# seungju-k1m/Distributed_RL

Hardware: AMD Instinct MI355X
Metric: learner frames/sec (whole node), Ape-X DQN Atari CNN (higher is better)
Workload: dtype bf16; 1 GPU; model=ape_x net (ape_x.json), global_batch=512, seq_len=4, parallelism=dp1, actors=0, replay=gpu sum-tree PER, graph=True

## Files before the change

distributed_rl_amd/algos/ape_x.py:

```python

from __future__ import annotations

import time
from collections import deque
from typing import Any, Dict, List, Optional

import numpy as np
import torch

from .. import ops
from ..config import Config
from ..models import BaseAgent
from ..replay import make_apex_schema, make_per
from .common import LearnerBase

PUBLISH_EVERY = 50
ACTOR_PULL_EVERY = 100


class ApexLearner(LearnerBase):
    ALG = "APE_X"

    def __init__(self, cfg: Config, device: Optional[str] = None, rank: int = 0,
                 world_size: int = 1, transport=None,
                 batch_size: Optional[int] = None,
                 replay_capacity: Optional[int] = None,
                 replay_device: Optional[str] = None,
                 replay_state_dtype: Optional[torch.dtype] = None,
                 replay=None, enable_tb: bool = True, run_root: str = "."):
        super().__init__(cfg, device, rank, world_size, run_root=run_root,
                         enable_tb=enable_tb)
        self.batch_size = batch_size or cfg.batch_size
        self.model = self.build_model()
        self.mp = None
        if self.device.type == "cuda":
            from ..parallel.precision import MixedPrecisionTrainer

            self.model.to(memory_format=torch.channels_last)
            order = self._dueling_param_order()
            self.mp = MixedPrecisionTrainer(self.model, param_order=order)
            self.net = self.mp.compute
            import copy as _copy

            self.target = _copy.deepcopy(self.mp.compute)
            for p in self.target.parameters():
                p.requires_grad_(False)
            from ..parallel.precision import _to_flat, _view_like

            tnamed = dict(self.target.named_parameters())
            tp = [tnamed[n] for n in self.mp._name_order]
            self.flat_tparam = torch.empty(
                sum(p.numel() for p in tp), dtype=torch.bfloat16,
                device=self.device,
            )
            off = 0
            with torch.no_grad():
                for p in tp:
                    n = p.numel()
                    self.flat_tparam[off : off + n].copy_(_to_flat(p))
                    p.data = _view_like(self.flat_tparam[off : off + n], p)
                    off += n
            self._build_fast_forward(order)
        else:
            self.net = self.model
            self.target = self.build_model()
            self.target.updateParameter(self.model, 1.0)
            for p in self.target.parameters():
                p.requires_grad_(False)
        self.optim = self.build_optim(self.model)
        cap = replay_capacity or cfg.replay_memory_len
        rdev = replay_device or (
            str(self.device) if self.device.type == "cuda" else "cpu"
        )
        self._nhwc = self.device.type == "cuda"
        self.state_dtype = replay_state_dtype or torch.uint8
        if replay is not None:
            self.replay = replay
            self._nhwc = False
        else:
            schema = (
                make_apex_schema(frame_shape=(84, 84, 4),
                                 state_dtype=self.state_dtype)
                if self._nhwc else make_apex_schema(state_dtype=self.state_dtype)
            )
            self.replay = make_per(cap, schema, device=rdev)
        self.transport = transport
        self.gamma = cfg.gamma
        self.n_step = cfg.unroll_step
        self.alpha = cfg.alpha
        self.beta = cfg.beta
        self.reducer = None
        self._ingest_stream = (
            torch.cuda.Stream(self.device) if self.device.type == "cuda" else None
        )
        self._staging = None

    def _dueling_param_order(self) -> List[str]:
        d = getattr(self.model, "_dueling", {})
        if len(d) != 1:
            return []
        (a_node, v_node), = d.values()
        if a_node not in self.model.nodes or v_node not in self.model.nodes:
            return []
        a_mod = self.model.nodes[a_node]
        v_mod = self.model.nodes[v_node]
        try:
            ok = (a_mod.body[0].in_features == v_mod.body[0].in_features
                  and a_mod.body[0].out_features == v_mod.body[0].out_features
                  and len(a_mod.body) == 4)
        except (AttributeError, IndexError, TypeError):
            ok = False
        if not ok:
            return []
        self._fast_nodes = (a_node, v_node)
        return [
            f"nodes.{a_node}.body.0.weight", f"nodes.{v_node}.body.0.weight",
            f"nodes.{a_node}.body.0.bias", f"nodes.{v_node}.body.0.bias",
        ]

    def _build_fast_forward(self, order: List[str]):
        self._fast_fwd = None
        self._fast_heads = None
        if not order:
            return
        import torch.nn.functional as F

        a_node, v_node = self._fast_nodes
        a_mod = self.net.nodes[a_node]
        hidden = a_mod.body[0].out_features
        in_f = a_mod.body[0].in_features
        w1 = self.mp.flat_view(order[:2]).view(2 * hidden, in_f
                                               ).detach().requires_grad_(True)
        w1.grad = self.mp.flat_view(order[:2], "grad").view_as(w1)
        b1 = self.mp.flat_view(order[2:]).detach().requires_grad_(True)
        b1.grad = self.mp.flat_view(order[2:], "grad").view_as(b1)
        a_head = self.net.nodes[a_node].body[2]
        v_head = self.net.nodes[v_node].body[2]
        cnn_node = next(
            n for n, c in self.cfg.model_info.items()
            if str(c.get("netCat", "")).upper() == "CNN2D"
        )
        cnn = self.net.nodes[cnn_node]

        import os as _os

        own_lin = (ops.linear_relu_supported(in_f, 2 * hidden)
                   and _os.environ.get("DRL_OWN_LINEAR", "0") == "1")

        def hidden_of(feat):
            if own_lin and feat.dtype == torch.bfloat16:
                return ops.fused_linear_relu(feat, w1, b1)
            return F.relu(F.linear(feat.to(w1.dtype), w1, b1))

        def fast_fwd(x):
            h = hidden_of(cnn(x))
            adv = a_head(h[:, :hidden])
            val = v_head(h[:, hidden:])
            return ops.dueling_head(adv.float(), val.float())

        self._fast_fwd = fast_fwd

        def fast_heads(x):
            h = hidden_of(cnn(x))
            return a_head(h[:, :hidden]), v_head(h[:, hidden:])

        self._fast_heads = fast_heads

        def fast_hidden(x):
            return hidden_of(cnn(x))

        self._fast_hidden = fast_hidden
        self._direct_list = [w1, b1] + list(self.mp.groups[0].c_params[4:])
        self._head_params = (a_head.weight, a_head.bias, v_head.weight,
                             v_head.bias)
        self._use_q_loss = ops.has_dueling_q_loss(hidden, self.cfg.action_size)
        t_cnn = self.target.nodes[cnn_node]
        ta_head = self.target.nodes[a_node].body[2]
        tv_head = self.target.nodes[v_node].body[2]
        w1t = self.flat_tparam[: 2 * hidden * in_f].view(2 * hidden, in_f)
        b1t = self.flat_tparam[2 * hidden * in_f : 2 * hidden * (in_f + 1)]

        def t_hidden_of(feat):
            if own_lin and feat.dtype == torch.bfloat16:
                return ops.fused_linear_relu(feat, w1t, b1t)
            return F.relu(F.linear(feat.to(w1t.dtype), w1t, b1t))

        def target_heads(x):
            h = t_hidden_of(t_cnn(x))
            return ta_head(h[:, :hidden]), tv_head(h[:, hidden:])

        self._target_heads = target_heads

        def target_hidden(x):
            return t_hidden_of(t_cnn(x))

        self._target_hidden = target_hidden
        self._thead_params = (ta_head.weight, ta_head.bias, tv_head.weight,
                              tv_head.bias)

    def _online_q(self, x):
        if getattr(self, "_fast_fwd", None) is not None:
            return self._fast_fwd(x)
        return self.net.forward([x])[0]

    _STAGE_ROWS = 4096

    def _staging_buffers(self):
        if self._staging is None:
            from ..replay import make_apex_schema

            wire = make_apex_schema()
            self._wire_names = list(wire)
            self._staging = {
                name: torch.empty((self._STAGE_ROWS, *shape), dtype=dtype
                                  ).pin_memory()
                for name, (shape, dtype) in wire.items()
            }
            self._staging["__prio__"] = torch.empty(
                self._STAGE_ROWS, dtype=torch.float32).pin_memory()
            self._stage_evt = torch.cuda.Event()
            self._stage_busy = False
        return self._staging

    def ingest(self) -> int:
        if self.transport is None:
            return 0
        if self._ingest_stream is not None and \
                hasattr(self.transport, "drain_views"):
            return self._ingest_views()
        got = self.transport.drain()
        if got is None:
            return 0
        cols_np, prio_np = got
        n = len(prio_np)
        if self._ingest_stream is None:
            cols = {k: torch.from_numpy(np.ascontiguousarray(v))
                    for k, v in cols_np.items()}
            self.replay.push(cols, torch.from_numpy(
                np.ascontiguousarray(prio_np)))
            self.ingested_total += n
            return n
        stage = self._staging_buffers()
        done = 0
        while done < n:
            k = min(self._STAGE_ROWS, n - done)
            if self._stage_busy:
                self._stage_evt.synchronize()
            for name, arr in cols_np.items():
                stage[name][:k].numpy()[:] = arr[done : done + k]
            stage["__prio__"][:k].numpy()[:] = prio_np[done : done + k]
            with torch.cuda.stream(self._ingest_stream):
                dev_cols = {
                    name: stage[name][:k].to(self.device, non_blocking=True)
                    for name in cols_np
                }
                if self._nhwc:
                    for kk in ("state", "next_state"):
                        dev_cols[kk] = dev_cols[kk].permute(0, 2, 3, 1
                                                            ).contiguous()
                if self.state_dtype != torch.uint8:
                    for kk in ("state", "next_state"):
                        dev_cols[kk] = dev_cols[kk].to(self.state_dtype) / 255.0
                prio_dev = stage["__prio__"][:k].to(self.device,
                                                    non_blocking=True)
            self._ingest_stream.wait_stream(
                torch.cuda.current_stream(self.device))
            with torch.cuda.stream(self._ingest_stream):
                self.replay.push(dev_cols, prio_dev)
            self._stage_evt.record(self._ingest_stream)
            self._stage_busy = True
            torch.cuda.current_stream(self.device).wait_stream(
                self._ingest_stream)
            done += k
        self.ingested_total += n
        return n

    def _ingest_views(self) -> int:
        stage = self._staging_buffers()
        np_dtype = self.transport.record_dtype
# ... 46 lines not shown
        for views, n, advance in self.transport.drain_views(
                max_per_ring=self._STAGE_ROWS):
            if stop_evt is not None and stop_evt.is_set():
                break
            for v in views:
                nrows = v.shape[0]
                i = 0
                while i < nrows:
                    if cursor == 0 and self._stage_busy:
                        self._stage_evt.synchronize()
                        self._stage_busy = False
                    k = min(self._STAGE_ROWS - cursor, nrows - i)
                    if has_pack:
                        src = torch.from_numpy(
                            np.ascontiguousarray(v[i : i + k]).reshape(-1))
                        ext.pack_rows(src, rec_size, offs, sizes, dsts, cursor)
                    else:
                        sl = v[i : i + k].reshape(-1).view(np_dtype)
                        for name in names:
                            stage[name][cursor : cursor + k].numpy()[:] = \
                                sl[name]
                        stage["__prio__"][cursor : cursor + k].numpy()[:] = \
                            sl["priority"]
                    cursor += k
                    i += k
                    total += k
                    self.ingested_total += k
                    if cursor == self._STAGE_ROWS:
                        flush()
            advance(n)
        flush()
        return total

    def push_experience(self, cols: Dict[str, torch.Tensor], prio: torch.Tensor):
        cols = dict(cols)
        for k in ("state", "next_state"):
            v = cols[k]
            if self._nhwc:
                v = v.permute(0, 2, 3, 1)
            if self.state_dtype != torch.uint8 and v.dtype == torch.uint8:
                v = v.to(self.state_dtype) / 255.0
            cols[k] = v.contiguous()
        self.replay.push(cols, prio)

    def train_step(self, data, idx, weights) -> Dict[str, torch.Tensor]:
        stats, prio = self._fwd_bwd(data, weights)
        if self.mp is not None:
            self.mp.allreduce_grads()
            self._optimize_mp()
        else:
            if self.reducer is not None:
                self.reducer.all_reduce()
            self.optim.step()
        self.replay.update(idx, prio)
        return stats

    def _fwd_bwd(self, data, weights):
        cuda = self.device.type == "cuda"
        if cuda:
            def to_cl(t):
                if t.shape[-1] == 4:
                    return t.to(self.device, non_blocking=True).permute(0, 3, 1, 2)
                return t.to(self.device, non_blocking=True).contiguous(
                    memory_format=torch.channels_last
                )

            s = to_cl(data["state"])
            sp = to_cl(data["next_state"])
            if s.dtype == torch.float16:
                s = s.to(torch.bfloat16)
                sp = sp.to(torch.bfloat16)
        elif data["state"].dtype == torch.uint8:
            s = ops.dequant_frames(data["state"], torch.float32)
            sp = ops.dequant_frames(data["next_state"], torch.float32)
        else:
            s = data["state"].float()
            sp = data["next_state"].float()
        actions = data["action"].to(self.device).long()
        rewards = data["reward"].to(self.device)
        dones = data["done"].to(self.device)
        weights = weights.to(self.device)

        if cuda and getattr(self, "_use_q_loss", False):
            h_s = self._fast_hidden(s)
            with torch.no_grad():
                h_on = self._fast_hidden(sp)
                h_tg = self._target_hidden(sp)
            wa, ba, wv, bv = self._head_params
            wat, bat, wvt, bvt = self._thead_params
            loss, prio, qmean = ops.dueling_q_head_loss(
                h_s, wa, ba, wv, bv, h_on, h_tg, wat, bat, wvt, bvt,
                actions, rewards, dones, weights, self.gamma, self.n_step,
                self.alpha,
            )
        elif cuda and getattr(self, "_fast_heads", None) is not None:
            adv_s, val_s = self._fast_heads(s)
            with torch.no_grad():
                adv_on, val_on = self._fast_heads(sp)
                adv_tg, val_tg = self._target_heads(sp)
            loss, prio, qmean = ops.dueling_nstep_dqn_loss(
                adv_s, val_s, adv_on, val_on, adv_tg, val_tg, actions,
                rewards, dones, weights, self.gamma, self.n_step, self.alpha,
            )
        else:
            q_s = self._online_q(s) if cuda else self.net.forward([s])[0]
            with torch.no_grad():
                q_sp_on = (self._online_q(sp) if cuda
                           else self.net.forward([sp])[0])
                q_sp_tg = self.target.forward([sp])[0]
            loss, prio, qmean = ops.nstep_dqn_loss(
                q_s, q_sp_on, q_sp_tg, actions, rewards,
                dones, weights, self.gamma, self.n_step, self.alpha,
                with_value_stat=True,
            )
        if self.mp is not None:
            self.mp.direct_grads(loss, getattr(self, "_direct_list", None))
        else:
            self.optim.zero_grad(set_to_none=False)
            loss.backward()
        return {"loss": loss.detach(), "value": qmean}, prio

    def _optimize_mp(self):
        self.mp.upcast_grads()
        self.optim.step()
        self.mp.sync_compute_params()

    def sync_target(self):
        if self.mp is not None:
            self.flat_tparam.copy_(self.mp.flat_cparam)
        else:
            self.target.updateParameter(self.model, 1.0)

    def _inner_step(self) -> Dict[str, torch.Tensor]:
        data, idx, w = self.replay.sample(self.batch_size, self.beta)
        return self.train_step(data, idx, w)

    def _cadence(self):
        self.step_count += 1
        if self.step_count % self.cfg.target_frequency == 0:
            self.sync_target()
            self.publish_weights(include_target=True)
        elif self.step_count % PUBLISH_EVERY == 0:
            self.publish_weights()

    def step(self) -> Dict[str, torch.Tensor]:
        stats = self.maybe_profile_first_step(self._inner_step)
        self._cadence()
        return stats

    def make_graphed_step(self, warmup_iters: int = 3):
        assert self.device.type == "cuda", "graph capture needs a GPU"
        for g in self.optim.param_groups:
            g["capturable"] = True
        split = self.mp is not None and self.mp.world > 1
        side = torch.cuda.Stream(self.device)
        side.wait_stream(torch.cuda.current_stream(self.device))
        with torch.cuda.stream(side):
            for _ in range(warmup_iters):
                self._inner_step()
        torch.cuda.current_stream(self.device).wait_stream(side)

        if not split:
            graph = torch.cuda.CUDAGraph()
            with torch.cuda.graph(graph):
                static_out = self._inner_step()
            self._graph = graph

            def stepper():
                graph.replay()
                self._cadence()
                return static_out

            return stepper

        mp = self.mp
        idx_save = torch.empty(self.batch_size, dtype=torch.int64,
                               device=self.device)
        g_s = torch.cuda.CUDAGraph()
        with torch.cuda.graph(g_s):
            s_data, s_idx, s_w = self.replay.sample(self.batch_size, self.beta)
        g_fb = torch.cuda.CUDAGraph()
        with torch.cuda.graph(g_fb, pool=g_s.pool()):
            static_out, prio = self._fwd_bwd(s_data, s_w)
            idx_save.copy_(s_idx)
        g_upd = torch.cuda.CUDAGraph()
        with torch.cuda.graph(g_upd, pool=g_s.pool()):
            self.replay.update(idx_save, prio)
        g_opt = torch.cuda.CUDAGraph()
        with torch.cuda.graph(g_opt, pool=g_s.pool()):
            self._optimize_mp()
        self._graph = (g_s, g_fb, g_upd, g_opt)
        comm = torch.cuda.Stream(self.device)
        g_s.replay()

        def stepper():
            cur = torch.cuda.current_stream(self.device)
            g_fb.replay()
            comm.wait_stream(cur)
            with torch.cuda.stream(comm):
                mp.allreduce_grads()
            g_upd.replay()
            g_s.replay()
            cur.wait_stream(comm)
            g_opt.replay()
            self._cadence()
# ... 366 lines not shown
```

distributed_rl_amd/models/base_agent.py:

```python

from __future__ import annotations

from typing import Any, Dict, List, Optional, Sequence, Tuple

import torch
import torch.nn as nn

_ACTS = {
    "relu": nn.ReLU,
    "leakyrelu": nn.LeakyReLU,
    "tanh": nn.Tanh,
    "sigmoid": nn.Sigmoid,
    "elu": nn.ELU,
    "linear": nn.Identity,
    "identity": nn.Identity,
}


def _act(name: str) -> nn.Module:
    return _ACTS[name.lower()]()


class CNN2D(nn.Module):

    def __init__(self, cfg: Dict[str, Any]):
        super().__init__()
        in_ch = int(cfg["iSize"])
        n_layer = int(cfg["nLayer"])
        f_size = list(cfg["fSize"])
        n_unit = list(cfg["nUnit"])
        stride = list(cfg.get("stride", [1] * len(n_unit)))
        padding = list(cfg.get("padding", [0] * len(n_unit)))
        acts = list(cfg.get("act", ["relu"] * len(n_unit)))
        bn = list(cfg.get("BN", [False] * n_layer))
        self.flatten = bool(cfg.get("linear", False)) or (f_size and f_size[-1] == -1)

        layers: List[nn.Module] = []
        n_conv = len(n_unit)
        ch = in_ch
        self._convs: List[nn.Conv2d] = []
        for i in range(n_conv):
            conv = nn.Conv2d(ch, n_unit[i], kernel_size=f_size[i],
                             stride=stride[i], padding=padding[i])
            self._convs.append(conv)
            layers.append(conv)
            if i < len(bn) and bn[i]:
                layers.append(nn.BatchNorm2d(n_unit[i]))
            layers.append(_act(acts[i]))
            ch = n_unit[i]
        self.body = nn.Sequential(*layers)
        self._fusable_static = (
            all(a.lower() == "relu" for a in acts[:n_conv])
            and not any(bn[:n_conv])
            and all(p == 0 for p in padding[:n_conv])
        )
        self._fused_checked: dict = {}

    def _fused_ok(self, x: torch.Tensor) -> bool:
        if not (self._fusable_static and x.is_cuda):
            return False
        if x.dtype not in (torch.uint8, torch.bfloat16):
            return False
        key = (tuple(x.shape[1:]), x.dtype)
        hit = self._fused_checked.get(key)
        if hit is not None:
            return hit
        from .. import ops as _ops

        ok = self._convs[0].weight.dtype == torch.bfloat16 and x.is_contiguous(
            memory_format=torch.channels_last
        )
        if ok:
            C, H, W = x.shape[1:]
            u8 = x.dtype == torch.uint8
            for conv in self._convs:
                COUT, _, KH, KW = conv.weight.shape
                S = conv.stride[0]
                if not _ops.conv_supported(H, W, C, KH, KW, S, COUT, u8):
                    ok = False
                    break
                H = (H - KH) // S + 1
                W = (W - KW) // S + 1
                C = COUT
                u8 = False
        self._fused_checked[key] = ok
        return ok

    def forward(self, x: torch.Tensor) -> torch.Tensor:
        if self._fused_ok(x):
            from .. import ops as _ops

            y = x
            last = len(self._convs) - 1
            for i, conv in enumerate(self._convs):
                if i == last and self.flatten and _ops.conv_chw_supported(
                        y.shape[2], y.shape[3], y.shape[1],
                        conv.weight.shape[2], conv.weight.shape[3],
                        conv.stride[0], conv.weight.shape[0]):
                    return _ops.fused_conv_relu(y, conv.weight, conv.bias,
                                                conv.stride[0], chw_out=True)
                y = _ops.fused_conv_relu(y, conv.weight, conv.bias,
                                         conv.stride[0])
        else:
            y = self.body(x)
        if self.flatten:
            y = torch.flatten(y, 1)
        return y


class MLP(nn.Module):
    def __init__(self, cfg: Dict[str, Any]):
        super().__init__()
        in_f = int(cfg["iSize"])
        f_size = list(cfg["fSize"])
        acts = list(cfg.get("act", ["relu"] * len(f_size)))
        bn = list(cfg.get("BN", [False] * len(f_size)))
        layers: List[nn.Module] = []
        f = in_f
        for i, out_f in enumerate(f_size):
            layers.append(nn.Linear(f, out_f))
            if i < len(bn) and bn[i]:
                layers.append(nn.BatchNorm1d(out_f))
            layers.append(_act(acts[i]))
            f = out_f
        self.body = nn.Sequential(*layers)

    def forward(self, x: torch.Tensor) -> torch.Tensor:
        return self.body(x)


class ViewV2(nn.Module):

    def forward(self, x: torch.Tensor, shape_hint: torch.Tensor) -> torch.Tensor:
        shape = [int(v) for v in shape_hint.flatten().tolist()]
        return x.reshape(shape)


class LSTMNET(nn.Module):

    def __init__(self, cfg: Dict[str, Any]):
        super().__init__()
        self.hidden_size = int(cfg["hiddenSize"])
        self.input_size = int(cfg["iSize"])
        self.num_layers = int(cfg.get("nLayer", 1))
        self.flatten_mode = bool(cfg.get("FlattenMode", True))
        self.return_hidden = bool(cfg.get("return_hidden", False))
        self.lstm = nn.LSTM(self.input_size, self.hidden_size, self.num_layers)
        self._state: Optional[Tuple[torch.Tensor, torch.Tensor]] = None

    def get_cell_state(self):
        return self._state

    def set_cell_state(self, state) -> None:
        self._state = state

    def zero_cell_state(self, batch: int = 1) -> None:
        p = next(self.lstm.parameters())
        z = torch.zeros(
            self.num_layers, batch, self.hidden_size, device=p.device, dtype=p.dtype
        )
        self._state = (z, z.clone())

    def detach_cell_state(self) -> None:
        if self._state is not None:
            self._state = (self._state[0].detach(), self._state[1].detach())

    def forward(self, x: torch.Tensor) -> torch.Tensor:
        p = next(self.lstm.parameters())
        import os as _os

        bf16_in = (
            x.dtype == torch.bfloat16 and x.is_cuda and self.num_layers == 1
            and _os.environ.get("DRL_LSTM_BF16_IN", "1") == "1"
        )
        if x.dtype != p.dtype and not bf16_in:
            x = x.to(p.dtype)
        if x.dim() == 2:
            x = x.unsqueeze(0)
        seq, batch, _ = x.shape
        if self._state is None or self._state[0].shape[1] != batch:
            self.zero_cell_state(batch)
        st = self._state
        if st[0].dtype != p.dtype or st[0].device != x.device:
            st = (st[0].to(x.device, p.dtype), st[1].to(x.device, p.dtype))
        if x.is_cuda and self.num_layers == 1:
            from .manual_lstm import manual_lstm_seq

            out, new_state = manual_lstm_seq(x, st, self.lstm)
        else:
            out, new_state = self.lstm(x, st)
# ... 292 lines not shown
```

distributed_rl_amd/ops/__init__.py:

```python

from __future__ import annotations

import os
from typing import Optional

import torch

from . import torch_ref

_EXT = None
_EXT_TRIED = False


def hip_ext(required: bool = True):
    global _EXT, _EXT_TRIED
    if _EXT is None and not _EXT_TRIED:
        _EXT_TRIED = True
        from . import build as _build

        _EXT = _build.load_prebuilt()
        if _EXT is None and torch.cuda.is_available():
            try:
                _EXT = _build.build()
            except Exception as e:
# ... 2 lines not shown
                        "gfx950 HIP extension missing and build failed: %s" % e
                    )
    if _EXT is None and required and not _allow_eager():
        raise RuntimeError(
            "device tensor reached a fused op but the _drl_hip extension is "
            "not built; run `python -m distributed_rl_amd.ops.build` "
            "(or set DRL_ALLOW_EAGER=1 to debug with eager torch)"
        )
    return _EXT


def _allow_eager() -> bool:
    return os.environ.get("DRL_ALLOW_EAGER", "0") == "1"


def _use_hip(t: torch.Tensor) -> bool:
    if not t.is_cuda:
        return False
    ext = hip_ext(required=not _allow_eager())
    return ext is not None




def dequant_frames(x_u8: torch.Tensor, dtype: torch.dtype = torch.bfloat16) -> torch.Tensor:
    if _use_hip(x_u8):
        out = torch.empty(x_u8.shape, dtype=dtype, device=x_u8.device)
        hip_ext().dequant(x_u8.contiguous(), out)
        return out
    return torch_ref.dequant_frames(x_u8, dtype)


def dequant_frames_nhwc(x_u8: torch.Tensor) -> torch.Tensor:
    if _use_hip(x_u8):
        out = torch.empty(
            x_u8.shape, dtype=torch.bfloat16, device=x_u8.device,
            memory_format=torch.channels_last,
        )
        hip_ext().dequant_nhwc(x_u8.contiguous(), out)
        return out
    return torch_ref.dequant_frames(x_u8, torch.float32).to(
        memory_format=torch.channels_last
    )




def conv_supported(H, W, C, KH, KW, S, COUT, u8: bool) -> bool:
    ext = hip_ext(required=False)
    if ext is None:
        return False
    return bool(ext.conv_fwd_supported(H, W, C, KH, KW, S, COUT, u8))


class _FusedConvFn(torch.autograd.Function):
    @staticmethod
    def forward(ctx, x, weight, bias, stride, chw_out=False):
        ext = hip_ext()
        N, C, H, W = x.shape
        COUT, _, KH, KW = weight.shape
        P = (H - KH) // stride + 1
        Q = (W - KW) // stride + 1
        b = bias if bias is not None else torch.empty(0, device=x.device)
        if chw_out:
            out = torch.empty(N, COUT * P * Q, dtype=torch.bfloat16,
                              device=x.device)
            ext.conv_fwd_chw(x, weight, b, out, stride)
        else:
            out = torch.empty(
                N, COUT, P, Q, dtype=torch.bfloat16, device=x.device,
                memory_format=torch.channels_last,
            )
            ext.conv_fwd(x, weight, b, out, stride)
        ctx.save_for_backward(x, weight, out)
        ctx.stride = stride
        ctx.has_bias = bias is not None
        ctx.chw = chw_out
        ctx.pq = (P, Q)
        return out

    @staticmethod
    def backward(ctx, gout):
        x, weight, out = ctx.saved_tensors
        stride = ctx.stride
        COUT = weight.shape[0]
        if ctx.chw:
            P, Q = ctx.pq
            N = gout.shape[0]
            masked = torch.empty(N, COUT, P, Q, dtype=torch.bfloat16,
                                 device=gout.device,
                                 memory_format=torch.channels_last)
            hip_ext().relu_mask_bwd_chw(gout.contiguous(), out, masked,
                                        COUT, P * Q)
            gout = masked
        else:
            if not gout.is_contiguous(memory_format=torch.channels_last):
                gout = gout.contiguous(memory_format=torch.channels_last)
            masked = torch.empty_like(gout)
            hip_ext().relu_mask_bwd(gout, out, masked)
            gout = masked
        need_x = ctx.needs_input_grad[0]
        need_w = ctx.needs_input_grad[1]
        need_b = ctx.has_bias and ctx.needs_input_grad[2]
        COUT, C, KH, KW = weight.shape
        ext = hip_ext()
        use_own_wrw = need_w and bool(
            ext.conv_wrw_supported(x.shape[2], x.shape[3], C, KH, KW, stride,
                                   COUT, x.dtype == torch.uint8)
        )
        gw = gb = None
        if use_own_wrw:
            K = KH * KW * C
            flat_ws = torch.empty(COUT * (K + 1), dtype=torch.float32,
                                  device=x.device)
            ws = flat_ws[: COUT * K].view(COUT, K)
            gb_ws = (flat_ws[COUT * K :] if need_b
                     else torch.empty(0, device=x.device))
            ext.conv_wrw(x, gout, ws, gb_ws, stride)
            gw = ws.view(COUT, KH, KW, C).permute(0, 3, 1, 2).to(torch.bfloat16)
            if need_b:
                gb = gb_ws.to(torch.bfloat16)
        gi = None
        use_own_dgrad = (
            os.environ.get("DRL_OWN_DGRAD", "0") == "1"
            and need_x and x.dtype == torch.bfloat16
            and hasattr(ext, "conv_dgrad_supported")
            and bool(ext.conv_dgrad_supported(x.shape[2], x.shape[3], C, KH,
                                              KW, stride, COUT))
        )
        if use_own_dgrad:
            gi = torch.empty_like(x)
            w_t = torch.empty(weight.numel(), dtype=torch.bfloat16,
                              device=x.device)
            ext.conv_dgrad(gout, weight, w_t, gi, stride)
        if (need_x and not use_own_dgrad) or (need_w and not use_own_wrw):
            if x.dtype == torch.uint8:
                xf = dequant_frames(x.permute(0, 2, 3, 1), torch.bfloat16)
                xf = xf.permute(0, 3, 1, 2)
            else:
                xf = x
            gi2, gw2, gb2 = torch.ops.aten.convolution_backward(
                gout, xf, weight,
                [COUT] if ctx.has_bias else None,
                [stride, stride], [0, 0], [1, 1], False, [0, 0], 1,
                [need_x and not use_own_dgrad, need_w and not use_own_wrw,
                 need_b and not use_own_wrw],
            )
            if gi is None:
                gi = gi2
            if gw is None:
                gw, gb = gw2, gb2
        return (gi if need_x else None), gw, gb, None, None


def fused_conv_relu(x, weight, bias, stride: int, chw_out: bool = False):
    return _FusedConvFn.apply(x, weight, bias, stride, chw_out)




def conv3x3_supported(H, W, C, COUT) -> bool:
    ext = hip_ext(required=False)
    return ext is not None and hasattr(ext, "conv3x3p1_supported") and \
        bool(ext.conv3x3p1_supported(H, W, C, COUT))


class _FusedConv3x3Fn(torch.autograd.Function):
    @staticmethod
    def forward(ctx, x, weight, bias, residual, relu_in, relu_out):
        ext = hip_ext()
        N, _, H, W = x.shape
        COUT = weight.shape[0]
        empty = torch.empty(0, device=x.device, dtype=torch.bfloat16)
        out = torch.empty(
            N, COUT, H, W, dtype=torch.bfloat16, device=x.device,
            memory_format=torch.channels_last,
        )
        ext.conv3x3p1_fwd(x, weight, bias if bias is not None else empty,
                          residual if residual is not None else empty, out,
                          relu_in, relu_out)
        ctx.save_for_backward(x, weight, out if relu_out else None)
        ctx.has_bias = bias is not None
        ctx.relu_in = relu_in
        ctx.relu_out = relu_out
        return out

    @staticmethod
    def backward(ctx, gout):
        x, weight, out = ctx.saved_tensors
        ext = hip_ext()
        COUT = weight.shape[0]
        if not gout.is_contiguous(memory_format=torch.channels_last):
            gout = gout.contiguous(memory_format=torch.channels_last)
        if ctx.relu_out:
            masked = torch.empty_like(gout)
            ext.relu_mask_bwd(gout, out, masked)
            gout = masked
        need_x = ctx.needs_input_grad[0]
        need_w = ctx.needs_input_grad[1]
        need_b = ctx.has_bias and ctx.needs_input_grad[2]
        gres = gout if ctx.needs_input_grad[3] else None
        gx = gw = gb = None
        if need_x or need_w or need_b:
            gx, gw, gb = torch.ops.aten.convolution_backward(
                gout, torch.relu(x) if ctx.relu_in else x, weight,
                [COUT] if ctx.has_bias else None,
                [1, 1], [1, 1], [1, 1], False, [0, 0], 1,
                [need_x, need_w, need_b],
            )
            if need_x and ctx.relu_in:
                if not gx.is_contiguous(memory_format=torch.channels_last):
                    gx = gx.contiguous(memory_format=torch.channels_last)
                masked = torch.empty_like(gx)
                ext.relu_mask_bwd(gx, x, masked)
                gx = masked
        return (gx if need_x else None), gw, gb, gres, None, None


def fused_conv3x3(x, weight, bias, *, relu_in: bool = False,
                  relu_out: bool = False, residual=None):
    if _use_hip(x):
        return _FusedConv3x3Fn.apply(x, weight, bias, residual, bool(relu_in),
                                     bool(relu_out))
    return torch_ref.conv3x3_res(x, weight, bias, relu_in, relu_out, residual)


def conv_chw_supported(H, W, C, KH, KW, S, COUT) -> bool:
    ext = hip_ext(required=False)
    return ext is not None and hasattr(ext, "conv_fwd_chw_supported") and \
        bool(ext.conv_fwd_chw_supported(H, W, C, KH, KW, S, COUT))


def linear_relu_supported(K, N) -> bool:
    ext = hip_ext(required=False)
    return ext is not None and hasattr(ext, "linear_relu_supported") and \
        bool(ext.linear_relu_supported(K, N))


class _LinearReluFn(torch.autograd.Function):
# ... 104 lines not shown
                   with_value_stat: bool = False):
    if _use_hip(q_s):
        loss, prio, qmean = _DQNLossFn.apply(
            q_s, q_sp_on, q_sp_tg, actions.long(),
            rewards.float(), dones.float(), weights.float(),
            gamma ** n_step, alpha,
        )
        return (loss, prio, qmean) if with_value_stat else (loss, prio)
    loss, prio = torch_ref.nstep_dqn_loss(
        q_s.float(), q_sp_on.float(), q_sp_tg.float(), actions, rewards.float(),
        dones.float(), weights.float(), gamma, n_step, alpha
    )
    if with_value_stat:
        return loss, prio, q_s.detach().float().max(1).values.mean()
    return loss, prio




class _DuelingDQNLossFn(torch.autograd.Function):
    @staticmethod
    def forward(ctx, adv_s, val_s, adv_on, val_on, adv_tg, val_tg, actions,
                rewards, dones, weights, gamma_n, alpha):
        ext = hip_ext()
        B, A = adv_s.shape
        dev = adv_s.device
        acc2 = torch.zeros(2, dtype=torch.float32, device=dev)
        prio = torch.empty(B, dtype=torch.float32, device=dev)
        coef = torch.empty(B, dtype=torch.float32, device=dev)
        ext.dueling_dqn_loss_fwd(
            adv_s.contiguous(), val_s.reshape(B).contiguous(),
            adv_on.contiguous(), val_on.reshape(B).contiguous(),
            adv_tg.contiguous(), val_tg.reshape(B).contiguous(),
            actions.contiguous(), rewards.contiguous(), dones.contiguous(),
            weights.contiguous(), float(gamma_n), float(alpha),
            acc2[0:1], prio, coef, acc2[1:2],
        )
        ctx.save_for_backward(coef, actions)
        ctx.shape = (B, A)
        ctx.in_dtype = adv_s.dtype
        loss_out, qmean = acc2[0], acc2[1]
        ctx.mark_non_differentiable(prio, qmean)
        return loss_out, prio, qmean

    @staticmethod
    def backward(ctx, gout, _gprio, _gqm):
        coef, actions = ctx.saved_tensors
        B, A = ctx.shape
        g_adv = torch.empty(B, A, dtype=ctx.in_dtype, device=coef.device)
        g_val = torch.empty(B, 1, dtype=ctx.in_dtype, device=coef.device)
        hip_ext().dueling_dqn_loss_bwd(coef, actions,
                                       gout.reshape(1).contiguous(), g_adv,
                                       g_val)
        return (g_adv, g_val) + (None,) * 10


def dueling_nstep_dqn_loss(adv_s, val_s, adv_on, val_on, adv_tg, val_tg,
                           actions, rewards, dones, weights, gamma: float,
                           n_step: int, alpha: float):
    if _use_hip(adv_s):
        return _DuelingDQNLossFn.apply(
            adv_s, val_s, adv_on, val_on, adv_tg, val_tg, actions.long(),
            rewards.float(), dones.float(), weights.float(),
            gamma ** n_step, alpha,
        )
    q_s = dueling_head(adv_s.float(), val_s.float())
    q_on = dueling_head(adv_on.float(), val_on.float())
    q_tg = dueling_head(adv_tg.float(), val_tg.float())
    return nstep_dqn_loss(q_s, q_on, q_tg, actions, rewards, dones, weights,
                          gamma, n_step, alpha, with_value_stat=True)




def has_dueling_q_loss(hidden: int, actions: int) -> bool:
    ext = hip_ext(required=False)
    return (ext is not None and hasattr(ext, "dueling_q_loss_fwd")
            and hidden == 512 and actions == 6)


class _DuelingQLossFn(torch.autograd.Function):
    @staticmethod
    def forward(ctx, h_s, wa, ba, wv, bv, h_on, h_tg, wa_t, ba_t, wv_t, bv_t,
                actions, rewards, dones, weights, gamma_n, alpha):
        ext = hip_ext()
        B = h_s.shape[0]
        dev = h_s.device
        acc2 = torch.zeros(2, dtype=torch.float32, device=dev)
        prio = torch.empty(B, dtype=torch.float32, device=dev)
        coef = torch.empty(B, dtype=torch.float32, device=dev)
        ext.dueling_q_loss_fwd(
            h_s.contiguous(), h_on.contiguous(), h_tg.contiguous(),
            wa.contiguous(), ba.contiguous(), wv.reshape(-1).contiguous(),
            bv.contiguous(), wa_t.contiguous(), ba_t.contiguous(),
            wv_t.reshape(-1).contiguous(), bv_t.contiguous(),
            actions.contiguous(), rewards.contiguous(), dones.contiguous(),
            weights.contiguous(), float(gamma_n), float(alpha),
            acc2[0:1], prio, coef, acc2[1:2],
        )
        ctx.save_for_backward(coef, actions, wa, wv, h_s)
        loss_out, qmean = acc2[0], acc2[1]
        ctx.mark_non_differentiable(prio, qmean)
        return loss_out, prio, qmean

    @staticmethod
    def backward(ctx, gout, _gprio, _gqm):
        coef, actions, wa, wv, h_s = ctx.saved_tensors
        ext = hip_ext()
        B = h_s.shape[0]
        dev = h_s.device
        dh = torch.empty(B, 1024, dtype=torch.bfloat16, device=dev)
        dwa = torch.empty(6, 512, dtype=torch.bfloat16, device=dev)
        dba = torch.empty(6, dtype=torch.bfloat16, device=dev)
        dwv = torch.empty(1, 512, dtype=torch.bfloat16, device=dev)
        dbv = torch.empty(1, dtype=torch.bfloat16, device=dev)
        ext.dueling_q_loss_bwd(coef, actions, gout.reshape(1).contiguous(),
                               wa.contiguous(), wv.reshape(-1).contiguous(),
                               h_s.contiguous(), dh, dwa, dba, dwv, dbv)
        return (dh, dwa, dba, dwv, dbv) + (None,) * 12


def has_r2d2_seq_loss() -> bool:
    ext = hip_ext(required=False)
    return ext is not None and hasattr(ext, "r2d2_loss_fwd")


class _R2D2SeqLossFn(torch.autograd.Function):
    @staticmethod
    def forward(ctx, q_train, q_tgt, actions, rewards, done, weights,
                burn_in, n_step, gamma, alpha, eta, use_rescaling):
        ext = hip_ext()
        T, B, A = q_tgt.shape
        W = T - 1 - burn_in
        dev = q_tgt.device
        td = torch.empty(W, B, dtype=torch.float32, device=dev)
        stats = torch.zeros(3, dtype=torch.float32, device=dev)
        ext.r2d2_loss_fwd(q_train, q_tgt, actions, rewards, done, weights,
                          burn_in, n_step, float(gamma), bool(use_rescaling),
                          td, stats)
        prio = torch.empty(B, dtype=torch.float32, device=dev)
        ext.r2d2_prio(td, float(alpha), float(eta), prio)
        ctx.save_for_backward(td, actions, weights)
        ctx.meta = (T, burn_in, tuple(q_train.shape))
        loss_out, value, td_abs = stats[0], stats[1], stats[2]
        ctx.mark_non_differentiable(prio, value, td_abs)
        return loss_out, prio, value, td_abs

    @staticmethod
    def backward(ctx, gout, _gp, _gv, _gt):
        td, actions, weights = ctx.saved_tensors
        T, m, qshape = ctx.meta
        dq = torch.empty(qshape, dtype=torch.float32, device=td.device)
        hip_ext().r2d2_loss_bwd(td, actions, weights,
                                gout.reshape(1).contiguous(), T, m, dq)
        return (dq,) + (None,) * 11


def r2d2_sequence_loss(q_train, q_tgt, actions, rewards, done, weights,
                       burn_in: int, n_step: int, gamma: float, alpha: float,
                       eta: float, use_rescaling: bool):
    return _R2D2SeqLossFn.apply(
        q_train.contiguous(), q_tgt.contiguous(),
        actions.to(torch.int32).contiguous(), rewards.float().contiguous(),
        done.float().contiguous(), weights.float().contiguous(),
        burn_in, n_step, gamma, alpha, eta, use_rescaling,
    )


def dueling_q_head_loss(h_s, wa, ba, wv, bv, h_on, h_tg, wa_t, ba_t, wv_t,
                        bv_t, actions, rewards, dones, weights, gamma: float,
                        n_step: int, alpha: float):
    if _use_hip(h_s):
        return _DuelingQLossFn.apply(
            h_s, wa, ba, wv, bv, h_on, h_tg, wa_t, ba_t, wv_t, bv_t,
            actions.long(), rewards.float(), dones.float(), weights.float(),
            gamma ** n_step, alpha,
        )
    import torch.nn.functional as F

    def heads(h, wa_, ba_, wv_, bv_):
        return (F.linear(h[:, :512].float(), wa_.float(), ba_.float()),
                F.linear(h[:, 512:].float(), wv_.float(), bv_.float()))

    adv_s, val_s = heads(h_s, wa, ba, wv, bv)
    adv_on, val_on = heads(h_on, wa, ba, wv, bv)
    adv_tg, val_tg = heads(h_tg, wa_t, ba_t, wv_t, bv_t)
    return dueling_nstep_dqn_loss(adv_s, val_s, adv_on, val_on, adv_tg,
                                  val_tg, actions, rewards, dones, weights,
                                  gamma, n_step, alpha)




def value_rescale(x: torch.Tensor, eps: float = 1e-3) -> torch.Tensor:
    if _use_hip(x) and not x.requires_grad:
        y = torch.empty_like(x, dtype=torch.float32)
        hip_ext().value_rescale(x.float().contiguous(), y, eps)
        return y
    return torch_ref.value_rescale(x, eps)


def inv_value_rescale(x: torch.Tensor, eps: float = 1e-3) -> torch.Tensor:
    if _use_hip(x) and not x.requires_grad:
        y = torch.empty_like(x, dtype=torch.float32)
        hip_ext().inv_value_rescale(x.float().contiguous(), y, eps)
        return y
    return torch_ref.inv_value_rescale(x, eps)


def sequence_priority(td_abs: torch.Tensor, alpha: float, eta: float = 0.9) -> torch.Tensor:
    if _use_hip(td_abs):
        T, B = td_abs.shape
        out = torch.empty(B, dtype=torch.float32, device=td_abs.device)
        hip_ext().seq_priority(td_abs.float().contiguous(), eta, alpha, out)
        return out
    return torch_ref.sequence_priority(td_abs, alpha, eta)




def vtrace(behavior_log_prob, target_log_prob, rewards, values, bootstrap_value,
           not_done, gamma, rho_bar=1.0, c_bar=1.0, lam=1.0):
    if _use_hip(rewards):
        T, B = rewards.shape
        dev = rewards.device
        vs = torch.empty(T, B, dtype=torch.float32, device=dev)
        pg_adv = torch.empty_like(vs)
        rho_c = torch.empty_like(vs)
        hip_ext().vtrace(
            behavior_log_prob.float().contiguous(),
            target_log_prob.float().contiguous(), rewards.float().contiguous(),
            values.float().contiguous(), bootstrap_value.float().contiguous(),
            not_done.float().contiguous(), gamma, rho_bar, c_bar, lam,
            vs, pg_adv, rho_c,
        )
        return vs, pg_adv, rho_c
    return torch_ref.vtrace(
        behavior_log_prob, target_log_prob, rewards, values, bootstrap_value,
        not_done, gamma, rho_bar, c_bar, lam
    )


def vtrace_bt(mu_probs, target_log_prob, rewards, values, bootstrap_value,
              not_done, gamma, rho_bar=1.0, c_bar=1.0, lam=1.0):
    if _use_hip(rewards):
        B, T = rewards.shape
        dev = rewards.device
        vs = torch.empty(B, T, dtype=torch.float32, device=dev)
        pg_adv = torch.empty_like(vs)
        hip_ext().vtrace_bt(
            mu_probs.float().contiguous(), target_log_prob.float().contiguous(),
            rewards.float().contiguous(), values.float().contiguous(),
            bootstrap_value.float().contiguous(), not_done.float().contiguous(),
            gamma, rho_bar, c_bar, lam, vs, pg_adv,
        )
        return vs, pg_adv
    vs_T, pg_T, _ = torch_ref.vtrace(
        mu_probs.log().t().contiguous(), target_log_prob.t().contiguous(),
        rewards.t().contiguous(), values.t().contiguous(), bootstrap_value,
        not_done, gamma, rho_bar, c_bar, lam
    )
# ... 116 lines not shown
```

distributed_rl_amd/ops/hip/conv_mfma.hip:

```cpp

#include <hip/hip_runtime.h>
#include <hip/hip_bf16.h>
#include <torch/extension.h>
#include <ATen/cuda/CUDAContext.h>

namespace {

using bf16x8 = __attribute__((ext_vector_type(8))) __bf16;
using f32x4 = __attribute__((ext_vector_type(4))) float;

constexpr int kPad = 32;

template <int H, int W, int C, int KH, int KW, int S, int COUT, bool U8IN>
struct ConvGeom {
  static constexpr int P = (H - KH) / S + 1;
  static constexpr int Q = (W - KW) / S + 1;
  static constexpr int K = KH * KW * C;
  static constexpr int KCHUNKS = K / 32;
  static_assert(K % 32 == 0, "K must be a multiple of 32");
  static_assert((KW * C) % 32 == 0, "patch row must tile by 32");
  static constexpr int ROWC = KW * C;
  static constexpr int LDS_ROW = K + kPad;
  static constexpr int LDS_ELEMS = COUT * LDS_ROW;
};

template <int H, int W, int C, int KH, int KW, int S, int COUT, bool U8IN,
          int WAVES, int RPW, bool CHW_OUT = false>
__global__ __launch_bounds__(WAVES * 64) void conv_fwd_kernel(
    const void* __restrict__ in_v,
    const __bf16* __restrict__ weight,
    const __bf16* __restrict__ bias,
    __bf16* __restrict__ out,
    int batch) {
  using G = ConvGeom<H, W, C, KH, KW, S, COUT, U8IN>;
  extern __shared__ __attribute__((aligned(16))) char smem[];
  __bf16* wlds = reinterpret_cast<__bf16*>(smem);

  const int tid = threadIdx.x;
  const int lane = tid & 63;
  const int wave = tid >> 6;

  constexpr int WELEMS = COUT * G::K;
  for (int base = tid * 8; base < WELEMS; base += WAVES * 64 * 8) {
    int co = base / G::K;
    int k = base - co * G::K;
    bf16x8 v = *reinterpret_cast<const bf16x8*>(weight + co * G::K + k);
    *reinterpret_cast<bf16x8*>(wlds + co * G::LDS_ROW + k) = v;
  }
  __syncthreads();

  const int M = batch * G::P * G::Q;
  const int row0 = (blockIdx.x * WAVES + wave) * RPW;
  if (row0 >= M) return;
  constexpr int RFRAG = RPW / 16;
  constexpr int NFRAG = COUT / 16;
  int64_t in_row0[RFRAG];
#pragma unroll
  for (int rf = 0; rf < RFRAG; ++rf) {
    int arow = row0 + rf * 16 + (lane & 15);
    if (arow >= M) arow = M - 1;
    const int n = arow / (G::P * G::Q);
    const int rem = arow - n * (G::P * G::Q);
    const int p = rem / G::Q;
    const int q = rem - p * G::Q;
    in_row0[rf] = ((int64_t)n * H + p * S) * (W * C) + q * S * C;
  }
  const int kpart = (lane >> 4) * 8;

  f32x4 acc[RFRAG][NFRAG];
#pragma unroll
  for (int rf = 0; rf < RFRAG; ++rf)
#pragma unroll
    for (int f = 0; f < NFRAG; ++f) acc[rf][f] = {0.f, 0.f, 0.f, 0.f};

#pragma unroll
  for (int kc = 0; kc < G::KCHUNKS; ++kc) {
    const int kelem = kc * 32 + kpart;
    const int dy = kelem / G::ROWC;
    const int dx = kelem - dy * G::ROWC;
    const int64_t koff = (int64_t)dy * (W * C) + dx;
    bf16x8 a[RFRAG];
#pragma unroll
    for (int rf = 0; rf < RFRAG; ++rf) {
      const int64_t goff = in_row0[rf] + koff;
      if constexpr (U8IN) {
        const uint8_t* src = reinterpret_cast<const uint8_t*>(in_v) + goff;
        uint2 raw = *reinterpret_cast<const uint2*>(src);
        const float inv255 = 1.0f / 255.0f;
#pragma unroll
        for (int j = 0; j < 8; ++j) {
          unsigned byte =
              (j < 4 ? raw.x >> (8 * j) : raw.y >> (8 * (j - 4))) & 0xFF;
          a[rf][j] = (__bf16)(byte * inv255);
        }
      } else {
        a[rf] = *reinterpret_cast<const bf16x8*>(
            reinterpret_cast<const __bf16*>(in_v) + goff);
      }
    }
#pragma unroll
    for (int f = 0; f < NFRAG; ++f) {
      const int col = f * 16 + (lane & 15);
      bf16x8 b = *reinterpret_cast<const bf16x8*>(
          wlds + col * G::LDS_ROW + kc * 32 + kpart);
#pragma unroll
      for (int rf = 0; rf < RFRAG; ++rf)
        acc[rf][f] =
            __builtin_amdgcn_mfma_f32_16x16x32_bf16(a[rf], b, acc[rf][f], 0, 0, 0);
    }
  }

  const int crow_base = (lane >> 4) * 4;
#pragma unroll
  for (int rf = 0; rf < RFRAG; ++rf)
#pragma unroll
    for (int f = 0; f < NFRAG; ++f) {
      const int col = f * 16 + (lane & 15);
      const float bv = bias ? (float)bias[col] : 0.0f;
#pragma unroll
      for (int r = 0; r < 4; ++r) {
        const int orow = row0 + rf * 16 + crow_base + r;
        if (orow < M) {
          float v = acc[rf][f][r] + bv;
          v = v > 0.0f ? v : 0.0f;
          if constexpr (CHW_OUT) {
            const int n = orow / (G::P * G::Q);
            const int pq = orow - n * (G::P * G::Q);
            out[((int64_t)n * COUT + col) * (G::P * G::Q) + pq] = (__bf16)v;
          } else {
            out[(int64_t)orow * COUT + col] = (__bf16)v;
          }
        }
      }
    }
}

struct ConvLaunch {
  int H, W, C, KH, KW, S, COUT;
  bool u8;
  void (*fn)(const void*, const __bf16*, const __bf16*, __bf16*, int);
  int lds_bytes;
  int waves, rpw;
};

template <int H, int W, int C, int KH, int KW, int S, int COUT, bool U8,
          int WAVES = 4, int RPW = 16, bool CHW = false>
ConvLaunch make_launch() {
  using G = ConvGeom<H, W, C, KH, KW, S, COUT, U8>;
  return ConvLaunch{H, W, C, KH, KW, S, COUT, U8,
                    conv_fwd_kernel<H, W, C, KH, KW, S, COUT, U8, WAVES, RPW,
                                    CHW>,
                    (int)(G::LDS_ELEMS * sizeof(__bf16)), WAVES, RPW};
}

static const ConvLaunch kChwLaunches[] = {
    make_launch<9, 9, 64, 3, 3, 1, 64, false, 8, 16, true>(),
    make_launch<20, 20, 16, 4, 4, 2, 32, false, 8, 16, true>(),
};

static const ConvLaunch kLaunches[] = {
    make_launch<84, 84, 4, 8, 8, 4, 32, true, 8, 32>(),
    make_launch<84, 84, 4, 8, 8, 4, 32, false, 8, 32>(),
    make_launch<20, 20, 32, 4, 4, 2, 64, false, 8, 16>(),
    make_launch<9, 9, 64, 3, 3, 1, 64, false, 8, 16>(),
    make_launch<84, 84, 4, 8, 8, 4, 16, true, 8, 16>(),
    make_launch<84, 84, 4, 8, 8, 4, 16, false, 8, 16>(),
    make_launch<20, 20, 16, 4, 4, 2, 32, false, 8, 16>(),
};

static const ConvLaunch kVariants[] = {
    make_launch<84, 84, 4, 8, 8, 4, 32, true, 4, 16>(),
    make_launch<84, 84, 4, 8, 8, 4, 32, true, 8, 16>(),
    make_launch<84, 84, 4, 8, 8, 4, 32, true, 4, 32>(),
    make_launch<84, 84, 4, 8, 8, 4, 32, true, 8, 32>(),
    make_launch<20, 20, 32, 4, 4, 2, 64, false, 4, 16>(),
    make_launch<20, 20, 32, 4, 4, 2, 64, false, 8, 16>(),
    make_launch<20, 20, 32, 4, 4, 2, 64, false, 4, 32>(),
    make_launch<20, 20, 32, 4, 4, 2, 64, false, 8, 32>(),
    make_launch<9, 9, 64, 3, 3, 1, 64, false, 4, 16>(),
    make_launch<9, 9, 64, 3, 3, 1, 64, false, 8, 16>(),
    make_launch<9, 9, 64, 3, 3, 1, 64, false, 4, 32>(),
    make_launch<9, 9, 64, 3, 3, 1, 64, false, 8, 32>(),
};

__global__ void mfma_probe_kernel(const __bf16* __restrict__ A,
                                  const __bf16* __restrict__ B,
                                  float* __restrict__ C) {
  int lane = threadIdx.x & 63;
  bf16x8 a, b;
  int kpart = (lane >> 4) * 8;
#pragma unroll
  for (int j = 0; j < 8; ++j) {
    a[j] = A[(lane & 15) * 32 + kpart + j];
    b[j] = B[(kpart + j) * 16 + (lane & 15)];
  }
  f32x4 acc = {0.f, 0.f, 0.f, 0.f};
  acc = __builtin_amdgcn_mfma_f32_16x16x32_bf16(a, b, acc, 0, 0, 0);
#pragma unroll
  for (int r = 0; r < 4; ++r)
    C[((lane >> 4) * 4 + r) * 16 + (lane & 15)] = acc[r];
}

}

void mfma_probe(torch::Tensor A, torch::Tensor B, torch::Tensor C) {
  hipLaunchKernelGGL(mfma_probe_kernel, dim3(1), dim3(64), 0,
                     (hipStream_t)at::cuda::getCurrentCUDAStream().stream(),
                     (const __bf16*)A.data_ptr(), (const __bf16*)B.data_ptr(),
                     C.data_ptr<float>());
}

bool conv_fwd_supported(int64_t H, int64_t W, int64_t C, int64_t KH, int64_t KW,
                        int64_t S, int64_t COUT, bool u8) {
  for (const auto& l : kLaunches)
    if (l.H == H && l.W == W && l.C == C && l.KH == KH && l.KW == KW &&
        l.S == S && l.COUT == COUT && l.u8 == u8)
      return true;
  return false;
}

void conv_fwd(torch::Tensor in, torch::Tensor weight, torch::Tensor bias,
              torch::Tensor out, int64_t stride) {
  TORCH_CHECK(in.is_cuda() && out.is_cuda());
  TORCH_CHECK(in.is_contiguous(at::MemoryFormat::ChannelsLast),
              "conv_fwd input must be channels_last");
  TORCH_CHECK(out.is_contiguous(at::MemoryFormat::ChannelsLast));
  TORCH_CHECK(weight.is_contiguous(at::MemoryFormat::ChannelsLast));
  const int N = (int)in.size(0), C = (int)in.size(1), H = (int)in.size(2),
            W = (int)in.size(3);
  const int COUT = (int)weight.size(0), KH = (int)weight.size(2),
            KW = (int)weight.size(3);
  const bool u8 = in.scalar_type() == torch::kUInt8;
  if (!u8) TORCH_CHECK(in.scalar_type() == torch::kBFloat16);
  TORCH_CHECK(weight.scalar_type() == torch::kBFloat16);
  TORCH_CHECK(out.scalar_type() == torch::kBFloat16);
  const ConvLaunch* L = nullptr;
  for (const auto& l : kLaunches)
    if (l.H == H && l.W == W && l.C == C && l.KH == KH && l.KW == KW &&
        l.S == (int)stride && l.COUT == COUT && l.u8 == u8) {
      L = &l;
      break;
    }
  TORCH_CHECK(L, "no fused conv kernel for this geometry: ", H, "x", W, "x", C,
              " k", KH, "x", KW, " s", stride, " -> ", COUT, " u8=", u8);
  const int P = (H - KH) / (int)stride + 1, Q = (W - KW) / (int)stride + 1;
  const int M = N * P * Q;
  const int rows_per_block = L->waves * L->rpw;
  const int blocks = (M + rows_per_block - 1) / rows_per_block;
  const __bf16* bias_ptr = nullptr;
  if (bias.defined() && bias.numel() > 0) {
    TORCH_CHECK(bias.scalar_type() == torch::kBFloat16);
    bias_ptr = (const __bf16*)bias.data_ptr();
  }
  hipLaunchKernelGGL(L->fn, dim3(blocks), dim3(L->waves * 64), L->lds_bytes,
                     (hipStream_t)at::cuda::getCurrentCUDAStream().stream(),
                     (const void*)in.data_ptr(),
                     (const __bf16*)weight.data_ptr(), bias_ptr,
                     (__bf16*)out.data_ptr(), N);
}

bool conv_fwd_variant(torch::Tensor in, torch::Tensor weight,
                      torch::Tensor bias, torch::Tensor out, int64_t stride,
                      int64_t variant) {
  const int N = (int)in.size(0), C = (int)in.size(1), H = (int)in.size(2),
            W = (int)in.size(3);
  const int COUT = (int)weight.size(0), KH = (int)weight.size(2),
            KW = (int)weight.size(3);
  const bool u8 = in.scalar_type() == torch::kUInt8;
  if (variant < 0 || variant >= (int64_t)(sizeof(kVariants) / sizeof(ConvLaunch)))
    return false;
  const ConvLaunch* L = &kVariants[variant];
  if (!(L->H == H && L->W == W && L->C == C && L->KH == KH && L->KW == KW &&
        L->S == (int)stride && L->COUT == COUT && L->u8 == u8))
    return false;
  const int P = (H - KH) / (int)stride + 1, Q = (W - KW) / (int)stride + 1;
  const int M = N * P * Q;
  const int rows_per_block = L->waves * L->rpw;
  const int blocks = (M + rows_per_block - 1) / rows_per_block;
  const __bf16* bias_ptr = nullptr;
  if (bias.defined() && bias.numel() > 0)
    bias_ptr = (const __bf16*)bias.data_ptr();
  hipLaunchKernelGGL(L->fn, dim3(blocks), dim3(L->waves * 64), L->lds_bytes,
                     (hipStream_t)at::cuda::getCurrentCUDAStream().stream(),
                     (const void*)in.data_ptr(),
                     (const __bf16*)weight.data_ptr(), bias_ptr,
                     (__bf16*)out.data_ptr(), N);
  return true;
}

void conv_wrw(torch::Tensor in, torch::Tensor gout, torch::Tensor gw_ws,
              torch::Tensor gb_ws, int64_t stride);
bool conv_wrw_supported(int64_t H, int64_t W, int64_t C, int64_t KH,
                        int64_t KW, int64_t S, int64_t COUT, bool u8);
void conv_dgrad(torch::Tensor gout, torch::Tensor weight, torch::Tensor w_t,
                torch::Tensor dx, int64_t stride);
bool conv_dgrad_supported(int64_t H, int64_t W, int64_t C, int64_t KH,
                          int64_t KW, int64_t S, int64_t COUT);
void conv_fwd_chw(torch::Tensor in, torch::Tensor weight, torch::Tensor bias,
                  torch::Tensor out2d, int64_t stride);
bool conv_fwd_chw_supported(int64_t H, int64_t W, int64_t C, int64_t KH,
                            int64_t KW, int64_t S, int64_t COUT);
void relu_mask_bwd_chw(torch::Tensor gout2d, torch::Tensor out2d,
                       torch::Tensor dst_nhwc, int64_t C, int64_t PQ);
void linear_relu(torch::Tensor x, torch::Tensor w, torch::Tensor b,
                 torch::Tensor out);
bool linear_relu_supported(int64_t K, int64_t N);
void tr16_probe(torch::Tensor out, int64_t mode);
void conv3x3p1_fwd(torch::Tensor in, torch::Tensor weight, torch::Tensor bias,
                   torch::Tensor residual, torch::Tensor out, bool relu_in,
                   bool relu_out);
bool conv3x3p1_supported(int64_t H, int64_t W, int64_t C, int64_t COUT);

void register_conv(pybind11::module_& m) {
  m.def("conv_fwd", &conv_fwd,
        "fused NHWC bf16 MFMA conv fwd (+dequant on u8 input, bias, ReLU)");
  m.def("conv_fwd_supported", &conv_fwd_supported);
  m.def("mfma_probe", &mfma_probe, "16x16x32 bf16 MFMA fragment-map probe");
  m.def("conv_fwd_variant", &conv_fwd_variant, "tuning-variant conv fwd");
  m.def("conv_wrw", &conv_wrw, "MFMA conv weight-grad (fp32 workspace)");
  m.def("conv_wrw_supported", &conv_wrw_supported);
  m.def("conv_dgrad", &conv_dgrad,
        "MFMA conv data-grad (masked-tap gather, pre-transposed weights)");
  m.def("conv_dgrad_supported", &conv_dgrad_supported);
  m.def("conv_fwd_chw", &conv_fwd_chw,
        "conv fwd with flatten fused into the epilogue (2-D CHW out)");
  m.def("conv_fwd_chw_supported", &conv_fwd_chw_supported);
  m.def("relu_mask_bwd_chw", &relu_mask_bwd_chw,
        "relu-mask + CHW->NHWC transpose (backward of the fused flatten)");
  m.def("linear_relu", &linear_relu,
        "fused Linear+bias+ReLU fwd (own MFMA GEMM, LDS-staged W)");
  m.def("linear_relu_supported", &linear_relu_supported);
  m.def("tr16_probe", &tr16_probe);
  m.def("conv3x3p1_fwd", &conv3x3p1_fwd,
        "MFMA 3x3 s1 pad-1 NHWC bf16 conv fwd (+relu_in, bias, residual, "
        "relu_out)");
  m.def("conv3x3p1_supported", &conv3x3p1_supported);
}


namespace {

constexpr int kPadM = 8;
constexpr int kPlanePad = 64;

typedef __bf16 v4bf_w __attribute__((ext_vector_type(4)));

template <int STRIDE>
__device__ __forceinline__ bf16x8 tr_frag(const __bf16* tile, int lane,
                                          int colblk) {
  const int g = lane >> 4, r = lane & 15;
  const __bf16* base =
      tile + (g * 8 + (r >> 2)) * STRIDE + colblk * 16 + 4 * (r & 3);
  auto* p0 = (__attribute__((address_space(3))) v4bf_w*)base;
  auto* p1 = (__attribute__((address_space(3))) v4bf_w*)(base + 4 * STRIDE);
  v4bf_w lo = __builtin_amdgcn_ds_read_tr16_b64_v4bf16(p0);
  v4bf_w hi = __builtin_amdgcn_ds_read_tr16_b64_v4bf16(p1);
  bf16x8 out;
#pragma unroll
  for (int j = 0; j < 4; ++j) { out[j] = lo[j]; out[j + 4] = hi[j]; }
  return out;
}

template <int H, int W, int C, int KH, int KW, int S, int COUT, bool U8IN>
__global__ __launch_bounds__(256) void conv_wrw_kernel(
    const void* __restrict__ in_v,
    const __bf16* __restrict__ gout,
    float* __restrict__ gw_part,
    int batch, int mblocks) {
  using G = ConvGeom<H, W, C, KH, KW, S, COUT, U8IN>;
  extern __shared__ __attribute__((aligned(16))) char smem[];
  constexpr int ASTRIDE = 64 + kPadM;
  constexpr int GSTRIDE = COUT + kPadM;
  __bf16* a_t = reinterpret_cast<__bf16*>(smem);
  __bf16* g_t = a_t + 32 * ASTRIDE;

  const int ktile = blockIdx.x;
  const int mb = blockIdx.y;
  const int tid = threadIdx.x;
  const int lane = tid & 63;
  const int wave = tid >> 6;
  const int M = batch * G::P * G::Q;
  const int n_chunks = (M + 31) / 32;

  constexpr int CBLK = COUT / 16;
  f32x4 acc[CBLK];
#pragma unroll
  for (int cb = 0; cb < CBLK; ++cb) acc[cb] = {0.f, 0.f, 0.f, 0.f};

  static_assert(G::ROWC % 16 == 0, "16-elem staging piece crosses a row");
  const int sm = tid >> 2;
  const int sk16 = (tid & 3) * 16;

  for (int mc = mb; mc < n_chunks; mc += mblocks) {
    const int m0 = mc * 32;
    if (tid < 128) {
      const int m = m0 + sm;
      const int mcl = m < M ? m : M - 1;
      const int n = mcl / (G::P * G::Q);
      const int rem = mcl - n * (G::P * G::Q);
      const int p = rem / G::Q;
      const int q = rem - p * G::Q;
      const int kelem = ktile * 64 + sk16;
      const int dy = kelem / G::ROWC;
      const int dx = kelem - dy * G::ROWC;
      const int64_t goff =
          ((int64_t)n * H + p * S + dy) * (W * C) + q * S * C + dx;
      bf16x8 v0, v1;
      if constexpr (U8IN) {
        const uint8_t* src = reinterpret_cast<const uint8_t*>(in_v) + goff;
        uint4 raw = *reinterpret_cast<const uint4*>(src);
        const float inv255 = 1.0f / 255.0f;
        const unsigned rw[4] = {raw.x, raw.y, raw.z, raw.w};
#pragma unroll
        for (int j = 0; j < 8; ++j) {
          v0[j] = (__bf16)(((rw[j >> 2] >> (8 * (j & 3))) & 0xFF) * inv255);
          v1[j] = (__bf16)(((rw[2 + (j >> 2)] >> (8 * (j & 3))) & 0xFF)
                           * inv255);
        }
      } else {
        const __bf16* src = reinterpret_cast<const __bf16*>(in_v) + goff;
        v0 = *reinterpret_cast<const bf16x8*>(src);
        v1 = *reinterpret_cast<const bf16x8*>(src + 8);
      }
      if (m >= M) {
#pragma unroll
        for (int j = 0; j < 8; ++j) {
          v0[j] = (__bf16)0.0f;
          v1[j] = (__bf16)0.0f;
        }
      }
      *reinterpret_cast<bf16x8*>(a_t + sm * ASTRIDE + sk16) = v0;
      *reinterpret_cast<bf16x8*>(a_t + sm * ASTRIDE + sk16 + 8) = v1;
    } else {
      constexpr int PIECES = COUT / 8;
      for (int piece = tid - 128; piece < 32 * PIECES; piece += 128) {
        const int m = m0 + piece / PIECES;
        const int c0 = (piece % PIECES) * 8;
        bf16x8 v;
        if (m < M) {
          v = *reinterpret_cast<const bf16x8*>(gout + (int64_t)m * COUT + c0);
        } else {
#pragma unroll
          for (int j = 0; j < 8; ++j) v[j] = (__bf16)0.0f;
        }
        *reinterpret_cast<bf16x8*>(g_t + (piece / PIECES) * GSTRIDE + c0) = v;
      }
    }
    __syncthreads();
    bf16x8 bfrag = tr_frag<ASTRIDE>(a_t, lane, wave);
#pragma unroll
    for (int cb = 0; cb < CBLK; ++cb) {
      bf16x8 afrag = tr_frag<GSTRIDE>(g_t, lane, cb);
      acc[cb] = __builtin_amdgcn_mfma_f32_16x16x32_bf16(afrag, bfrag, acc[cb],
                                                        0, 0, 0);
    }
    __syncthreads();
  }

  float* plane = gw_part + (int64_t)mb * (COUT * G::K + kPlanePad);
  const int kout = ktile * 64 + wave * 16 + (lane & 15);
#pragma unroll
  for (int cb = 0; cb < CBLK; ++cb)
#pragma unroll
    for (int r = 0; r < 4; ++r) {
      const int cout = cb * 16 + (lane >> 4) * 4 + r;
      plane[(int64_t)cout * G::K + kout] = acc[cb][r];
    }
}

__global__ __launch_bounds__(256) void wrw_reduce_kernel(
    const float* __restrict__ part, int planes, int n_elem,
    float* __restrict__ out, const float* __restrict__ b_part, int b_planes,
    int cout, float* __restrict__ b_out) {
  __shared__ __attribute__((aligned(16))) float sh4_raw[256 * 4];
  float* sh = sh4_raw;
  const int tid = threadIdx.x;
  const int e_blocks = (n_elem + 63) / 64;
  if ((int)blockIdx.x < e_blocks) {
    const int e4 = blockIdx.x * 64 + (tid & 15) * 4;
    const int g = tid >> 4;
    float4 s = {0.0f, 0.0f, 0.0f, 0.0f};
    const float4 zero = {0.0f, 0.0f, 0.0f, 0.0f};
    for (int p = g; p < planes; p += 64) {
      float4 v[4];
#pragma unroll
      for (int u = 0; u < 4; ++u) {
        const int pu = p + 16 * u;
        v[u] = pu < planes ? *reinterpret_cast<const float4*>(
                                 part + (int64_t)pu * (n_elem + kPlanePad) + e4)
                           : zero;
      }
#pragma unroll
      for (int u = 0; u < 4; ++u) {
        s.x += v[u].x; s.y += v[u].y; s.z += v[u].z; s.w += v[u].w;
      }
    }
    float4* sh4 = reinterpret_cast<float4*>(sh4_raw);
    sh4[tid] = s;
    __syncthreads();
    if (tid < 16) {
      float4 t = sh4[tid];
      for (int k = 1; k < 16; ++k) {
        const float4 v = sh4[k * 16 + tid];
        t.x += v.x; t.y += v.y; t.z += v.z; t.w += v.w;
      }
      *reinterpret_cast<float4*>(out + e4) = t;
    }
  } else {
    const int G = 256 / cout;
    const int c = tid % cout, g = tid / cout;
    float s = 0.0f;
    for (int p = g; p < b_planes; p += G) s += b_part[p * cout + c];
    sh[tid] = s;
    __syncthreads();
    if (tid < cout) {
      float t = 0.0f;
      for (int k = 0; k < G; ++k) t += sh[k * cout + tid];
      b_out[tid] = t;
    }
  }
}

struct WrwLaunch {
  int H, W, C, KH, KW, S, COUT;
  bool u8;
  void (*fn)(const void*, const __bf16*, float*, int, int);
  int lds_bytes;
  int ktiles;
};

template <int H, int W, int C, int KH, int KW, int S, int COUT, bool U8>
WrwLaunch make_wrw() {
  using G = ConvGeom<H, W, C, KH, KW, S, COUT, U8>;
  static_assert(G::K % 64 == 0, "wrw needs K % 64 == 0");
  return WrwLaunch{H, W, C, KH, KW, S, COUT, U8,
                   conv_wrw_kernel<H, W, C, KH, KW, S, COUT, U8>,
                   (int)(32 * (64 + kPadM + COUT + kPadM) * sizeof(__bf16)),
                   G::K / 64};
}

static const WrwLaunch kWrwLaunches[] = {
    make_wrw<84, 84, 4, 8, 8, 4, 32, true>(),
    make_wrw<84, 84, 4, 8, 8, 4, 32, false>(),
    make_wrw<20, 20, 32, 4, 4, 2, 64, false>(),
    make_wrw<9, 9, 64, 3, 3, 1, 64, false>(),
    make_wrw<84, 84, 4, 8, 8, 4, 16, true>(),
    make_wrw<84, 84, 4, 8, 8, 4, 16, false>(),
    make_wrw<20, 20, 16, 4, 4, 2, 32, false>(),
};

template <int COUT>
__global__ __launch_bounds__(256) void colsum_bf16_kernel(
    const __bf16* __restrict__ x, int64_t M, float* __restrict__ out) {
  typedef __bf16 bf8 __attribute__((ext_vector_type(8)));
  __shared__ float sh[256 * 8];
  const int tid = threadIdx.x;
  const int64_t nchunk = M * COUT / 8;
  int64_t i = (int64_t)blockIdx.x * blockDim.x + tid;
  const int64_t stride = (int64_t)gridDim.x * blockDim.x;
  float acc[8] = {0, 0, 0, 0, 0, 0, 0, 0};
  const bf8* __restrict__ x8 = (const bf8*)x;
  for (; i < nchunk; i += stride) {
    bf8 v = x8[i];
#pragma unroll
    for (int j = 0; j < 8; ++j) acc[j] += (float)v[j];
  }
#pragma unroll
  for (int j = 0; j < 8; ++j) sh[tid * 8 + j] = acc[j];
  __syncthreads();
  if (tid < COUT) {
    float s = 0.0f;
    for (int t = tid >> 3; t < 256; t += COUT / 8) s += sh[t * 8 + (tid & 7)];
    out[(int64_t)blockIdx.x * COUT + tid] = s;
  }
}

}

bool conv_wrw_supported(int64_t H, int64_t W, int64_t C, int64_t KH, int64_t KW,
                        int64_t S, int64_t COUT, bool u8) {
  for (const auto& l : kWrwLaunches)
    if (l.H == H && l.W == W && l.C == C && l.KH == KH && l.KW == KW &&
        l.S == S && l.COUT == COUT && l.u8 == u8)
      return true;
  return false;
}

void conv_wrw(torch::Tensor in, torch::Tensor gout, torch::Tensor gw_ws,
              torch::Tensor gb_ws, int64_t stride) {
  TORCH_CHECK(in.is_contiguous(at::MemoryFormat::ChannelsLast));
  TORCH_CHECK(gout.is_contiguous(at::MemoryFormat::ChannelsLast));
  TORCH_CHECK(gw_ws.scalar_type() == torch::kFloat32 && gw_ws.is_contiguous());
  const int N = (int)in.size(0), C = (int)in.size(1), H = (int)in.size(2),
            W = (int)in.size(3);
  const int COUT = (int)gout.size(1);
  const bool u8 = in.scalar_type() == torch::kUInt8;
  const WrwLaunch* L = nullptr;
  for (const auto& l : kWrwLaunches) {
    int KHl = l.KH, KWl = l.KW;
    if (l.H == H && l.W == W && l.C == C && l.S == (int)stride &&
        l.COUT == COUT && l.u8 == u8 &&
        (H - KHl) / (int)stride + 1 == (int)gout.size(2) &&
        (W - KWl) / (int)stride + 1 == (int)gout.size(3)) {
      L = &l;
      break;
    }
  }
  TORCH_CHECK(L, "no wrw kernel for this geometry");
  const int P = (int)gout.size(2), Q = (int)gout.size(3);
  const int M = N * P * Q;
  const int n_chunks = (M + 31) / 32;
  int mb = (n_chunks > 8192 ? 2048 : 512) / L->ktiles;
  if (mb > n_chunks) mb = n_chunks;
  if (mb < 1) mb = 1;
  auto st = (hipStream_t)at::cuda::getCurrentCUDAStream().stream();
  const int n_elem = (int)gw_ws.numel();
  TORCH_CHECK(n_elem == COUT * L->ktiles * 64, "gw_ws shape mismatch");
  auto part = torch::empty({(int64_t)mb, (int64_t)n_elem + kPlanePad},
                           gw_ws.options());
  hipLaunchKernelGGL(L->fn, dim3(L->ktiles, mb), dim3(256), L->lds_bytes, st,
                     (const void*)in.data_ptr(), (const __bf16*)gout.data_ptr(),
                     part.data_ptr<float>(), N, mb);
  const bool bias = gb_ws.defined() && gb_ws.numel() > 0;
  constexpr int kColsumBlocks = 256;
  torch::Tensor b_part;
  if (bias) {
    TORCH_CHECK(gb_ws.numel() == COUT && gb_ws.scalar_type() == torch::kFloat32);
    b_part = torch::empty({(int64_t)kColsumBlocks, (int64_t)COUT},
                          gw_ws.options());
    const int64_t Mrows = (int64_t)N * P * Q;
    switch (COUT) {
      case 16:
        hipLaunchKernelGGL(colsum_bf16_kernel<16>, dim3(kColsumBlocks),
                           dim3(256), 0, st, (const __bf16*)gout.data_ptr(),
                           Mrows, b_part.data_ptr<float>());
        break;
      case 32:
        hipLaunchKernelGGL(colsum_bf16_kernel<32>, dim3(kColsumBlocks),
                           dim3(256), 0, st, (const __bf16*)gout.data_ptr(),
                           Mrows, b_part.data_ptr<float>());
        break;
      case 64:
        hipLaunchKernelGGL(colsum_bf16_kernel<64>, dim3(kColsumBlocks),
                           dim3(256), 0, st, (const __bf16*)gout.data_ptr(),
                           Mrows, b_part.data_ptr<float>());
        break;
      default:
        TORCH_CHECK(false, "no colsum instantiation for COUT=", COUT);
    }
  }
  const int e_blocks = (n_elem + 63) / 64;
  hipLaunchKernelGGL(wrw_reduce_kernel, dim3(e_blocks + (bias ? 1 : 0)),
                     dim3(256), 0, st, (const float*)part.data_ptr<float>(), mb,
                     n_elem, gw_ws.data_ptr<float>(),
                     bias ? (const float*)b_part.data_ptr<float>() : nullptr,
                     kColsumBlocks, COUT, bias ? gb_ws.data_ptr<float>() : nullptr);
}

namespace {
typedef __bf16 v4bf __attribute__((ext_vector_type(4)));
__global__ void tr16_probe_kernel(float* out, int mode) {
  __shared__ __bf16 lds[512];
  int lane = threadIdx.x & 63;
  for (int i = threadIdx.x; i < 512; i += 64) lds[i] = (__bf16)(float)i;
  __syncthreads();
  int off;
  switch (mode) {
    case 0: off = 0; break;
    case 1: off = lane * 4; break;
    case 2: off = (lane >> 4) * 64; break;
    default: off = (lane & 15) * 4; break;
  }
  auto* p = (__attribute__((address_space(3))) v4bf*)(lds + off);
  v4bf v = __builtin_amdgcn_ds_read_tr16_b64_v4bf16(p);
#pragma unroll
  for (int j = 0; j < 4; ++j) out[lane * 4 + j] = (float)v[j];
}
}

void tr16_probe(torch::Tensor out, int64_t mode) {
  hipLaunchKernelGGL(tr16_probe_kernel, dim3(1), dim3(64), 0,
                     (hipStream_t)at::cuda::getCurrentCUDAStream().stream(),
                     out.data_ptr<float>(), (int)mode);
}

namespace {

template <int H, int W, int C, int KH, int KW, int S, int COUT, int WAVES,
          int RPW>
__global__ __launch_bounds__(WAVES * 64) void conv_dgrad_kernel(
    const __bf16* __restrict__ gout,
    const __bf16* __restrict__ w_t,
    __bf16* __restrict__ dx,
    int batch) {
  constexpr int P = (H - KH) / S + 1;
  constexpr int Q = (W - KW) / S + 1;
  constexpr int K = KH * KW * COUT;
  constexpr int KCHUNKS = K / 32;
  constexpr int CPT = COUT / 32;
  static_assert(COUT % 32 == 0, "chunks must not straddle taps");
  constexpr int RFRAG = RPW / 16;
  constexpr int NFRAG = C / 16;

  const int tid = threadIdx.x;
  const int lane = tid & 63;
  const int wave = tid >> 6;
  const int M = batch * H * W;
  const int row0 = (blockIdx.x * WAVES + wave) * RPW;
  if (row0 >= M) return;

  int a_n[RFRAG], a_y[RFRAG], a_x[RFRAG];
#pragma unroll
  for (int rf = 0; rf < RFRAG; ++rf) {
    int arow = row0 + rf * 16 + (lane & 15);
    if (arow >= M) arow = M - 1;
    a_n[rf] = arow / (H * W);
    const int rem = arow - a_n[rf] * (H * W);
    a_y[rf] = rem / W;
    a_x[rf] = rem - a_y[rf] * W;
  }
  const int kpart = (lane >> 4) * 8;

  f32x4 acc[RFRAG][NFRAG];
#pragma unroll
  for (int rf = 0; rf < RFRAG; ++rf)
#pragma unroll
    for (int f = 0; f < NFRAG; ++f) acc[rf][f] = {0.f, 0.f, 0.f, 0.f};

#pragma unroll
  for (int kc = 0; kc < KCHUNKS; ++kc) {
    const int tap = kc / CPT;
    const int kh = tap / KW;
    const int kw = tap - kh * KW;
    const int co = (kc - tap * CPT) * 32 + kpart;
    bf16x8 a[RFRAG];
#pragma unroll
    for (int rf = 0; rf < RFRAG; ++rf) {
      const int py = a_y[rf] - kh;
      const int qx = a_x[rf] - kw;
// ... 64 lines not shown
    make_dgrad<20, 20, 32, 4, 4, 2, 64>(),
    make_dgrad<9, 9, 64, 3, 3, 1, 64>(),
    make_dgrad<20, 20, 16, 4, 4, 2, 32>(),
};
}

bool conv_dgrad_supported(int64_t H, int64_t W, int64_t C, int64_t KH,
                          int64_t KW, int64_t S, int64_t COUT) {
  for (const auto& l : kDgrad)
    if (l.H == H && l.W == W && l.C == C && l.KH == KH && l.KW == KW &&
        l.S == S && l.COUT == COUT)
      return true;
  return false;
}

void conv_dgrad(torch::Tensor gout, torch::Tensor weight, torch::Tensor w_t,
                torch::Tensor dx, int64_t stride) {
  TORCH_CHECK(gout.is_contiguous(at::MemoryFormat::ChannelsLast));
  TORCH_CHECK(dx.is_contiguous(at::MemoryFormat::ChannelsLast));
  TORCH_CHECK(weight.is_contiguous(at::MemoryFormat::ChannelsLast));
  const int N = (int)dx.size(0), C = (int)dx.size(1), H = (int)dx.size(2),
            W = (int)dx.size(3);
  const int COUT = (int)weight.size(0), KH = (int)weight.size(2),
            KW = (int)weight.size(3);
  const DgradLaunch* L = nullptr;
  for (const auto& l : kDgrad)
    if (l.H == H && l.W == W && l.C == C && l.KH == KH && l.KW == KW &&
        l.S == (int)stride && l.COUT == COUT) {
      L = &l;
      break;
    }
  TORCH_CHECK(L, "no dgrad kernel for this geometry");
  auto stream = (hipStream_t)at::cuda::getCurrentCUDAStream().stream();
  const int total = KH * KW * C * COUT;
  hipLaunchKernelGGL(conv_w_transpose_kernel, dim3((total + 255) / 256),
                     dim3(256), 0, stream, (const __bf16*)weight.data_ptr(),
                     (__bf16*)w_t.data_ptr(), KH * KW, C, COUT);
  const int M = N * H * W;
  const int rows_per_block = L->waves * L->rpw;
  const int blocks = (M + rows_per_block - 1) / rows_per_block;
  hipLaunchKernelGGL(L->fn, dim3(blocks), dim3(L->waves * 64), 0, stream,
                     (const __bf16*)gout.data_ptr(),
                     (const __bf16*)w_t.data_ptr(), (__bf16*)dx.data_ptr(), N);
}

bool conv_fwd_chw_supported(int64_t H, int64_t W, int64_t C, int64_t KH,
                            int64_t KW, int64_t S, int64_t COUT) {
  for (const auto& l : kChwLaunches)
    if (l.H == H && l.W == W && l.C == C && l.KH == KH && l.KW == KW &&
        l.S == S && l.COUT == COUT)
      return true;
  return false;
}

void conv_fwd_chw(torch::Tensor in, torch::Tensor weight, torch::Tensor bias,
                  torch::Tensor out2d, int64_t stride) {
  TORCH_CHECK(in.is_contiguous(at::MemoryFormat::ChannelsLast));
  TORCH_CHECK(weight.is_contiguous(at::MemoryFormat::ChannelsLast));
  TORCH_CHECK(out2d.is_contiguous() && out2d.dim() == 2);
  const int N = (int)in.size(0), C = (int)in.size(1), H = (int)in.size(2),
            W = (int)in.size(3);
  const int COUT = (int)weight.size(0), KH = (int)weight.size(2),
            KW = (int)weight.size(3);
  const ConvLaunch* L = nullptr;
  for (const auto& l : kChwLaunches)
    if (l.H == H && l.W == W && l.C == C && l.KH == KH && l.KW == KW &&
        l.S == (int)stride && l.COUT == COUT) {
      L = &l;
      break;
    }
  TORCH_CHECK(L, "no CHW-out conv kernel for this geometry");
  const int P = (H - KH) / (int)stride + 1, Q = (W - KW) / (int)stride + 1;
  const int M = N * P * Q;
  const int rows_per_block = L->waves * L->rpw;
  const int blocks = (M + rows_per_block - 1) / rows_per_block;
  const __bf16* bias_ptr = nullptr;
  if (bias.defined() && bias.numel() > 0)
    bias_ptr = (const __bf16*)bias.data_ptr();
  hipLaunchKernelGGL(L->fn, dim3(blocks), dim3(L->waves * 64), L->lds_bytes,
                     (hipStream_t)at::cuda::getCurrentCUDAStream().stream(),
                     (const void*)in.data_ptr(),
                     (const __bf16*)weight.data_ptr(), bias_ptr,
                     (__bf16*)out2d.data_ptr(), N);
}

namespace {
__global__ void relu_mask_bwd_chw_kernel(const __bf16* __restrict__ gout,
                                         const __bf16* __restrict__ outv,
                                         __bf16* __restrict__ dst, int64_t N,
                                         int C, int PQ) {
  int64_t i = (int64_t)blockIdx.x * blockDim.x + threadIdx.x;
  const int64_t total = N * (int64_t)C * PQ;
  const int64_t stride = (int64_t)gridDim.x * blockDim.x;
  for (; i < total; i += stride) {
    const int c = (int)(i % C);
    const int64_t t = i / C;
    const int pq = (int)(t % PQ);
    const int64_t n = t / PQ;
    const int64_t src = ((int64_t)n * C + c) * PQ + pq;
    dst[i] = ((float)outv[src] > 0.0f) ? gout[src] : (__bf16)0.0f;
  }
}
}

void relu_mask_bwd_chw(torch::Tensor gout2d, torch::Tensor out2d,
                       torch::Tensor dst_nhwc, int64_t C, int64_t PQ) {
  const int64_t N = gout2d.size(0);
  const int64_t total = N * C * PQ;
  int blocks = (int)std::min<int64_t>((total + 255) / 256, 2048);
  hipLaunchKernelGGL(relu_mask_bwd_chw_kernel, dim3(blocks), dim3(256), 0,
                     (hipStream_t)at::cuda::getCurrentCUDAStream().stream(),
                     (const __bf16*)gout2d.data_ptr(),
                     (const __bf16*)out2d.data_ptr(),
                     (__bf16*)dst_nhwc.data_ptr(), N, (int)C, (int)PQ);
}

namespace {

template <int K, int N, int NT >
__global__ __launch_bounds__(256) void linear_relu_kernel(
    const __bf16* __restrict__ x,
    const __bf16* __restrict__ w,
    const __bf16* __restrict__ b,
    __bf16* __restrict__ out,
    int M) {
  constexpr int KB = 64;
  constexpr int LROW = KB + 32;
  __shared__ __bf16 wlds[NT][LROW];
  const int tid = threadIdx.x;
  const int lane = tid & 63;
  const int wave = tid >> 6;
  const int row0 = blockIdx.x * 32 + (wave >> 1) * 16;
  const int col0 = blockIdx.y * NT + (wave & 1) * (NT / 2);
  constexpr int NFRAG = NT / 2 / 16;
  const int arow = row0 + (lane & 15);
  const int arow_c = arow < M ? arow : (M > 0 ? M - 1 : 0);
  const int kpart = (lane >> 4) * 8;

  f32x4 acc[NFRAG];
#pragma unroll
  for (int f = 0; f < NFRAG; ++f) acc[f] = {0.f, 0.f, 0.f, 0.f};

  constexpr int PIECES = NT * KB / (256 * 8);
  bf16x8 wpre[PIECES];
#pragma unroll
  for (int pc = 0; pc < PIECES; ++pc) {
    const int base = (tid + pc * 256) * 8;
    const int r = base / KB;
    wpre[pc] = *reinterpret_cast<const bf16x8*>(
        w + (int64_t)(blockIdx.y * NT + r) * K + (base - r * KB));
  }
  bf16x8 a_cur[2], a_nxt[2];
#pragma unroll
  for (int kc = 0; kc < 2; ++kc)
    a_cur[kc] = *reinterpret_cast<const bf16x8*>(
        x + (int64_t)arow_c * K + kc * 32 + kpart);
  for (int k0 = 0; k0 < K; k0 += KB) {
    __syncthreads();
#pragma unroll
    for (int pc = 0; pc < PIECES; ++pc) {
      const int base = (tid + pc * 256) * 8;
      const int r = base / KB;
      *reinterpret_cast<bf16x8*>(&wlds[r][base - r * KB]) = wpre[pc];
    }
    __syncthreads();
    if (k0 + KB < K) {
// ... 309 lines not shown
```

distributed_rl_amd/ops/hip/drl_kernels.hip:

```cpp

#include <hip/hip_runtime.h>
#include <hip/hip_bf16.h>
#include <torch/extension.h>
#include <ATen/cuda/CUDAContext.h>

#define DRL_CHECK_CUDA(x) TORCH_CHECK(x.is_cuda(), #x " must be a device tensor")
#define DRL_CHECK_CONTIG(x) TORCH_CHECK(x.is_contiguous(), #x " must be contiguous")

namespace {

constexpr int kBlock = 256;

__host__ __device__ inline int64_t ceil_div(int64_t a, int64_t b) { return (a + b - 1) / b; }

inline int grid_for(int64_t work, int per_thread = 1) {
  int64_t blocks = ceil_div(work, (int64_t)kBlock * per_thread);
  if (blocks > 2048) blocks = 2048;
  if (blocks < 1) blocks = 1;
  return (int)blocks;
}


__global__ void dequant_u8_bf16_kernel(const uchar4* __restrict__ in,
                                       ushort2* __restrict__ out,
// ... 516 lines not shown
                     (float)eps);
}

void seq_priority(torch::Tensor td_abs, double eta, double alpha,
                  torch::Tensor out) {
  int T = (int)td_abs.size(0), B = (int)td_abs.size(1);
  hipLaunchKernelGGL(seq_priority_kernel, dim3(ceil_div(B, kBlock)), dim3(kBlock), 0,
                     cur_stream(), td_abs.data_ptr<float>(), T, B, (float)eta,
                     (float)alpha, out.data_ptr<float>());
}

void vtrace(torch::Tensor b_logp, torch::Tensor t_logp, torch::Tensor rew,
            torch::Tensor values, torch::Tensor boot, torch::Tensor not_done,
            double gamma, double rho_bar, double c_bar, double lam,
            torch::Tensor vs, torch::Tensor pg_adv, torch::Tensor rho_out) {
  int T = (int)rew.size(0), B = (int)rew.size(1);
  hipLaunchKernelGGL(vtrace_kernel, dim3(ceil_div(B, kBlock)), dim3(kBlock), 0,
                     cur_stream(), b_logp.data_ptr<float>(),
                     t_logp.data_ptr<float>(), rew.data_ptr<float>(),
                     values.data_ptr<float>(), boot.data_ptr<float>(),
                     not_done.data_ptr<float>(), T, B, (float)gamma,
                     (float)rho_bar, (float)c_bar, (float)lam,
                     vs.data_ptr<float>(), pg_adv.data_ptr<float>(),
                     rho_out.data_ptr<float>());
}

void vtrace_bt(torch::Tensor mu, torch::Tensor t_logp, torch::Tensor rew,
               torch::Tensor values, torch::Tensor boot, torch::Tensor not_done,
               double gamma, double rho_bar, double c_bar, double lam,
               torch::Tensor vs, torch::Tensor pg_adv) {
  int B = (int)rew.size(0), T = (int)rew.size(1);
  for (auto* t : {&mu, &t_logp, &values, &vs, &pg_adv}) {
    DRL_CHECK_CONTIG((*t));
    TORCH_CHECK(t->numel() == (int64_t)B * T, "vtrace_bt shape mismatch");
  }
  TORCH_CHECK(boot.numel() == B && not_done.numel() == B);
  hipLaunchKernelGGL(vtrace_bt_kernel, dim3(ceil_div(B, kBlock)), dim3(kBlock),
                     0, cur_stream(), mu.data_ptr<float>(),
                     t_logp.data_ptr<float>(), rew.data_ptr<float>(),
                     values.data_ptr<float>(), boot.data_ptr<float>(),
                     not_done.data_ptr<float>(), T, B, (float)gamma,
                     (float)rho_bar, (float)c_bar, (float)lam,
                     vs.data_ptr<float>(), pg_adv.data_ptr<float>());
}

void grad_clip(torch::Tensor flat, double max_norm, torch::Tensor sqsum_buf) {
  int64_t n = flat.numel();
  hipLaunchKernelGGL(sq_sum_kernel, dim3(grid_for(n, 8)), dim3(kBlock), 0,
                     cur_stream(), flat.data_ptr<float>(), n,
                     sqsum_buf.data_ptr<float>());
  hipLaunchKernelGGL(clip_scale_kernel, dim3(grid_for(n, 4)), dim3(kBlock), 0,
                     cur_stream(), flat.data_ptr<float>(), n,
                     sqsum_buf.data_ptr<float>(), (float)max_norm);
}

void register_conv(pybind11::module_& m);
void relu_mask_bwd(torch::Tensor gout, torch::Tensor out, torch::Tensor dst);
void dueling_fwd(torch::Tensor adv, torch::Tensor val, torch::Tensor out);
void dueling_bwd(torch::Tensor g, torch::Tensor gadv, torch::Tensor gval);
void lstm_cell_fwd(torch::Tensor gates, torch::Tensor c_prev,
                   torch::Tensor h_out, torch::Tensor c_out,
                   torch::Tensor acts, torch::Tensor tanhc);
void lstm_cell_bwd(torch::Tensor dh, torch::Tensor gout_t, torch::Tensor dc_in,
                   torch::Tensor acts, torch::Tensor tanhc,
                   torch::Tensor c_prev, torch::Tensor dgates,
                   torch::Tensor dc_prev);
void policy_loss_fwd(torch::Tensor logits, torch::Tensor act, torch::Tensor adv,
                     double er, torch::Tensor obj_out, torch::Tensor ent_out,
                     torch::Tensor logpa_out, torch::Tensor pi_save,
                     torch::Tensor H_save);
void policy_loss_bwd(torch::Tensor pi_save, torch::Tensor H_save,
                     torch::Tensor act, torch::Tensor adv, torch::Tensor gout,
                     double er, double gsign, torch::Tensor dlogits);
void impala_loss_fwd(torch::Tensor logpa, torch::Tensor adv,
                     torch::Tensor mean_H, torch::Tensor v, torch::Tensor vs,
                     double er, torch::Tensor loss_out, torch::Tensor obj_out,
                     torch::Tensor critic_out);
void impala_out_bwd(torch::Tensor pi_save, torch::Tensor H_save,
                    torch::Tensor act, torch::Tensor adv, torch::Tensor v,
                    torch::Tensor vs, torch::Tensor gloss, int64_t B,
                    int64_t T, int64_t A, double er, torch::Tensor dout);
void rmsprop_step(torch::Tensor p, torch::Tensor g, torch::Tensor sq,
                  torch::Tensor ga, torch::Tensor mom, double lr, double alpha,
                  double eps, double wd, double mu, bool centered, bool has_mom);
void adam_step(torch::Tensor p, torch::Tensor g, torch::Tensor m,
               torch::Tensor v, torch::Tensor step, double lr, double b1,
               double b2, double eps, double wd);
bool lstm_step_fused(torch::Tensor xp_t, torch::Tensor h_in, torch::Tensor c_in,
                     torch::Tensor w_hh, torch::Tensor h_out,
                     torch::Tensor c_out, torch::Tensor acts,
                     torch::Tensor tanhc);
bool lstm_seq_persistent(torch::Tensor xp, torch::Tensor hs, torch::Tensor cs,
                         torch::Tensor w_hh, torch::Tensor acts,
                         torch::Tensor tanhc, torch::Tensor ctr);
bool lstm_step_fwd_bf16(torch::Tensor xp_t, torch::Tensor h_bf,
                        torch::Tensor c_in, torch::Tensor w_bf,
                        torch::Tensor h_out, torch::Tensor c_out,
                        torch::Tensor h_bf_out, torch::Tensor acts_t,
                        torch::Tensor tanhc_t);
bool lstm_step_bwd_bf16(torch::Tensor dg_prev, torch::Tensor dh_init,
                        torch::Tensor gout_t, torch::Tensor dc_in,
                        torch::Tensor w_t_bf, torch::Tensor acts_t,
                        torch::Tensor tanhc_t, torch::Tensor c_prev,
                        torch::Tensor dgates_t, torch::Tensor dg_bf_t,
                        torch::Tensor dc_out);
void dueling_dqn_loss_fwd(torch::Tensor adv_s, torch::Tensor val_s,
                          torch::Tensor adv_on, torch::Tensor val_on,
                          torch::Tensor adv_tg, torch::Tensor val_tg,
                          torch::Tensor act, torch::Tensor rew,
                          torch::Tensor done, torch::Tensor w, double gamma_n,
                          double alpha, torch::Tensor loss_out,
                          torch::Tensor prio_out, torch::Tensor grad_coef,
                          torch::Tensor qmax_out);
void dueling_dqn_loss_bwd(torch::Tensor grad_coef, torch::Tensor act,
                          torch::Tensor gout, torch::Tensor g_adv,
                          torch::Tensor g_val);
void pack_rows(torch::Tensor src, int64_t rec_size, std::vector<int64_t> offs,
               std::vector<int64_t> sizes, std::vector<torch::Tensor> dsts,
               int64_t dst_row);
bool lstm_seq_fwd_bf16(torch::Tensor xp, torch::Tensor c0, torch::Tensor w_bf,
                       torch::Tensor hs, torch::Tensor cs, torch::Tensor h_bfs,
                       torch::Tensor acts, torch::Tensor tanhc,
                       torch::Tensor ctr);
bool lstm_seq_bwd_bf16(torch::Tensor dh_init, torch::Tensor gout,
                       torch::Tensor dc_T, torch::Tensor w_t_bf,
                       torch::Tensor acts, torch::Tensor tanhc,
                       torch::Tensor cs, torch::Tensor dgates,
                       torch::Tensor dgates_bf, torch::Tensor dc0_out,
                       torch::Tensor ctr);
void dueling_q_loss_fwd(torch::Tensor h_s, torch::Tensor h_on,
                        torch::Tensor h_tg, torch::Tensor wa, torch::Tensor ba,
                        torch::Tensor wv, torch::Tensor bv, torch::Tensor wa_t,
                        torch::Tensor ba_t, torch::Tensor wv_t,
                        torch::Tensor bv_t, torch::Tensor act,
                        torch::Tensor rew, torch::Tensor done, torch::Tensor w,
                        double gamma_n, double alpha, torch::Tensor loss_out,
                        torch::Tensor prio_out, torch::Tensor grad_coef,
                        torch::Tensor qmax_out);
void dueling_q_loss_bwd(torch::Tensor grad_coef, torch::Tensor act,
                        torch::Tensor gout, torch::Tensor wa, torch::Tensor wv,
                        torch::Tensor h_s, torch::Tensor dh, torch::Tensor dwa,
                        torch::Tensor dba, torch::Tensor dwv,
                        torch::Tensor dbv);
void r2d2_loss_fwd(torch::Tensor q_train, torch::Tensor q_tgt,
                   torch::Tensor act, torch::Tensor rew, torch::Tensor done,
                   torch::Tensor w, int64_t m, int64_t n_step, double gamma,
                   bool rescale, torch::Tensor td_out, torch::Tensor stats);
void r2d2_prio(torch::Tensor td, double alpha, double eta, torch::Tensor prio);
void r2d2_loss_bwd(torch::Tensor td, torch::Tensor act, torch::Tensor w,
                   torch::Tensor gout, int64_t T, int64_t m, torch::Tensor dq);
void seq_transpose_rows(torch::Tensor src, torch::Tensor dst);
void gather_rows(torch::Tensor idx, std::vector<torch::Tensor> srcs,
                 std::vector<torch::Tensor> dsts);
void lstm_diag(torch::Tensor h_bfs, torch::Tensor w_bf, torch::Tensor sink,
               torch::Tensor ctr, int64_t B, int64_t T, int64_t mode);

PYBIND11_MODULE(TORCH_EXTENSION_NAME, m) {
  register_conv(m);
  m.def("dequant", &dequant, "u8 -> bf16/f32 /255 (K1)");
  m.def("dequant_nhwc", &dequant_nhwc, "u8 NCHW -> bf16 NHWC /255 (K1)");
  m.def("sumtree_update", &sumtree_update, "sum-tree leaf update + ordered subtree/top rebuild (K10); calls on one "
        "tree must be stream-ordered");
  m.def("sumtree_sample", &sumtree_sample, "stratified sum-tree descent (K10)");
  m.def("leaf_min_pos", &leaf_min_pos, "min positive leaf priority (K10)");
  m.def("per_weights", &per_weights, "PER IS weights (K10)");
  m.def("bump_seed", &bump_seed, "advance device RNG seed (graph-safe)");
  m.def("dqn_loss_fwd", &dqn_loss_fwd, "fused n-step double-DQN loss fwd (K4)");
  m.def("dqn_loss_bwd", &dqn_loss_bwd, "fused n-step double-DQN loss bwd (K4)");
  m.def("value_rescale", &value_rescale, "R2D2 h(x) (K6)");
  m.def("inv_value_rescale", &inv_value_rescale, "R2D2 h^-1(x) (K6)");
  m.def("seq_priority", &seq_priority, "R2D2 eta-mix sequence priority (K7)");
  m.def("vtrace", &vtrace, "IMPALA V-trace reversed scan (K8)");
  m.def("vtrace_bt", &vtrace_bt,
        "V-trace on (B,T) row-major tensors, mu probs raw (K8, no transposes)");
  m.def("grad_clip", &grad_clip, "fused global grad-norm clip (K11)");
  m.def("relu_mask_bwd", &relu_mask_bwd, "dst = gout * (out > 0), bf16");
  m.def("dueling_fwd", &dueling_fwd, "fused (A+V)-mean(A) (K3)");
  m.def("dueling_bwd", &dueling_bwd, "dueling epilogue backward (K3)");
  m.def("lstm_cell_fwd", &lstm_cell_fwd, "fused LSTM cell forward (K5)");
  m.def("lstm_cell_bwd", &lstm_cell_bwd, "fused LSTM cell backward (K5)");
  m.def("policy_loss_fwd", &policy_loss_fwd, "fused IMPALA policy obj fwd (K9)");
  m.def("policy_loss_bwd", &policy_loss_bwd, "fused IMPALA policy obj bwd (K9)");
  m.def("impala_loss_fwd", &impala_loss_fwd,
        "fused IMPALA total loss: pg objective + entropy + critic MSE (K9)");
  m.def("impala_out_bwd", &impala_out_bwd,
        "IMPALA whole-head backward: d loss/d out in one launch (K9)");
  m.def("rmsprop_step", &rmsprop_step, "fused flat centered RMSprop (K12)");
  m.def("adam_step", &adam_step, "fused flat Adam (K12)");
  m.def("lstm_step_fused", &lstm_step_fused,
        "one-kernel LSTM timestep: fp32-MFMA hh GEMM + cell (K5)");
  m.def("lstm_seq_persistent", &lstm_seq_persistent,
        "whole-sequence persistent LSTM: grid-resident, agent-scope step "
        "barriers (K5)");
  m.def("lstm_step_fwd_bf16", &lstm_step_fwd_bf16,
        "one-kernel LSTM timestep fwd: bf16-MFMA hh GEMM + cell (K5 v2)");
  m.def("lstm_step_bwd_bf16", &lstm_step_bwd_bf16,
        "one-kernel LSTM timestep bwd: bf16-MFMA dh GEMM + cell-bwd (K5 v2)");
  m.def("dueling_dqn_loss_fwd", &dueling_dqn_loss_fwd,
        "whole-head dueling + n-step double-DQN loss fwd (K3+K4 fused)");
  m.def("dueling_dqn_loss_bwd", &dueling_dqn_loss_bwd,
        "whole-head dueling loss bwd: closed-form (g_adv, g_val) (K3+K4)");
  m.def("pack_rows", &pack_rows,
        "AoS records -> SoA pinned staging, GIL-free multithreaded (C2)",
        pybind11::call_guard<pybind11::gil_scoped_release>());
  m.def("lstm_seq_fwd_bf16", &lstm_seq_fwd_bf16,
        "persistent whole-sequence LSTM fwd, bf16-MFMA hh + grid barriers "
        "(K5 v3)");
  m.def("lstm_seq_bwd_bf16", &lstm_seq_bwd_bf16,
        "persistent whole-sequence LSTM bwd, bf16-MFMA dh + grid barriers "
        "(K5 v3)");
  m.def("dueling_q_loss_fwd", &dueling_q_loss_fwd,
        "heads+dueling+n-step-DQN loss in one kernel (K3+K4+heads)");
  m.def("dueling_q_loss_bwd", &dueling_q_loss_bwd,
        "closed-form dh + head weight/bias grads (2 kernels)");
  m.def("r2d2_loss_fwd", &r2d2_loss_fwd,
        "R2D2 n-step targets + rescale + IS loss, one kernel (K4/K6 seq)");
  m.def("r2d2_prio", &r2d2_prio, "eta-mix sequence priority (K7)");
  m.def("r2d2_loss_bwd", &r2d2_loss_bwd,
        "R2D2 loss backward: closed-form dq_train scatter");
  m.def("seq_transpose_rows", &seq_transpose_rows,
        "(B,T,row) -> (T,B,row) whole-row block copy");
  m.def("gather_rows", &gather_rows,
        "fused multi-column replay row gather (one launch per sample)");
  m.def("lstm_diag", &lstm_diag,
        "persistent-step cost decomposition (barrier/stage/mfma)");
}
namespace {
__global__ void relu_mask_bwd_kernel(const ushort4* __restrict__ out,
                                     const ushort4* __restrict__ gout,
                                     ushort4* __restrict__ dst, int64_t n4) {
  int64_t stride = (int64_t)gridDim.x * blockDim.x;
  for (int64_t i = (int64_t)blockIdx.x * blockDim.x + threadIdx.x; i < n4;
       i += stride) {
    ushort4 o = out[i];
    ushort4 g = gout[i];
    g.x = (o.x & 0x8000 || o.x == 0) ? 0 : g.x;
    g.y = (o.y & 0x8000 || o.y == 0) ? 0 : g.y;
    g.z = (o.z & 0x8000 || o.z == 0) ? 0 : g.z;
    g.w = (o.w & 0x8000 || o.w == 0) ? 0 : g.w;
    dst[i] = g;
  }
}
}

void relu_mask_bwd(torch::Tensor gout, torch::Tensor out, torch::Tensor dst) {
  TORCH_CHECK(gout.scalar_type() == torch::kBFloat16 &&
              out.scalar_type() == torch::kBFloat16);
  int64_t n = gout.numel();
  TORCH_CHECK(n % 4 == 0);
  hipLaunchKernelGGL(relu_mask_bwd_kernel, dim3(grid_for(n / 4)), dim3(kBlock),
                     0, cur_stream(), (const ushort4*)out.data_ptr(),
                     (const ushort4*)gout.data_ptr(), (ushort4*)dst.data_ptr(),
                     n / 4);
}

namespace {
__global__ void dueling_fwd_kernel(const float* __restrict__ adv,
                                   const float* __restrict__ val, int B, int A,
                                   float* __restrict__ out) {
  int i = blockIdx.x * blockDim.x + threadIdx.x;
  if (i >= B) return;
  const float* a = adv + (int64_t)i * A;
  float mean = 0.0f;
  for (int j = 0; j < A; ++j) mean += a[j];
  mean /= A;
  float v = val[i];
  float* o = out + (int64_t)i * A;
  for (int j = 0; j < A; ++j) o[j] = a[j] + v - mean;
}

// ... 226 lines not shown
  const float n_inv = 1.0f / (float)((int64_t)B * T);
  for (; k < total; k += stride) {
    int64_t r = k / (A + 1);
    int j = (int)(k - r * (A + 1));
    int b = (int)(r / (T + 1));
    int t = (int)(r - (int64_t)b * (T + 1));
    float g = 0.0f;
    if (t < T) {
      int64_t i = (int64_t)b * T + t;
      if (j < A) {
        float p = pi_save[i * A + j];
        float lp = __logf(fmaxf(p, 1e-30f));
        float d = adv[i] * (((int)act[i] == j ? 1.0f : 0.0f) - p)
                  - er * p * (lp + H_save[i]);
        g = -gloss[0] * d * n_inv;
      } else {
        g = gloss[0] * (v[i] - vs[i]) * n_inv;
      }
    }
    dout[k] = g;
  }
}
}

void policy_loss_fwd(torch::Tensor logits, torch::Tensor act, torch::Tensor adv,
                     double er, torch::Tensor obj_out, torch::Tensor ent_out,
                     torch::Tensor logpa_out, torch::Tensor pi_save,
                     torch::Tensor H_save) {
  int N = (int)logits.size(0), A = (int)logits.size(1);
  hipLaunchKernelGGL(policy_loss_fwd_kernel, dim3(ceil_div(N, kBlock)),
                     dim3(kBlock), 0, cur_stream(), logits.data_ptr<float>(),
                     act.data_ptr<int64_t>(), adv.data_ptr<float>(), N, A,
                     (float)er, obj_out.data_ptr<float>(),
                     ent_out.data_ptr<float>(), logpa_out.data_ptr<float>(),
                     pi_save.data_ptr<float>(), H_save.data_ptr<float>());
}

void policy_loss_bwd(torch::Tensor pi_save, torch::Tensor H_save,
                     torch::Tensor act, torch::Tensor adv, torch::Tensor gout,
                     double er, double gsign, torch::Tensor dlogits) {
  int N = (int)pi_save.size(0), A = (int)pi_save.size(1);
  hipLaunchKernelGGL(policy_loss_bwd_kernel,
                     dim3(ceil_div((int64_t)N * A, kBlock)), dim3(kBlock), 0,
                     cur_stream(), pi_save.data_ptr<float>(),
                     H_save.data_ptr<float>(), act.data_ptr<int64_t>(),
                     adv.data_ptr<float>(), gout.data_ptr<float>(), N, A,
                     (float)er, (float)gsign, dlogits.data_ptr<float>());
}

void impala_loss_fwd(torch::Tensor logpa, torch::Tensor adv,
                     torch::Tensor mean_H, torch::Tensor v, torch::Tensor vs,
                     double er, torch::Tensor loss_out, torch::Tensor obj_out,
                     torch::Tensor critic_out) {
  int64_t n = logpa.numel();
  TORCH_CHECK(adv.numel() == n && v.numel() == n && vs.numel() == n,
              "impala_loss_fwd length mismatch");
  for (auto* t : {&logpa, &adv, &v, &vs}) DRL_CHECK_CONTIG((*t));
  hipLaunchKernelGGL(impala_loss_fwd_kernel, dim3(1), dim3(kBlock), 0,
                     cur_stream(), logpa.data_ptr<float>(),
                     adv.data_ptr<float>(), mean_H.data_ptr<float>(),
                     v.data_ptr<float>(), vs.data_ptr<float>(), n, (float)er,
                     loss_out.data_ptr<float>(), obj_out.data_ptr<float>(),
                     critic_out.data_ptr<float>());
}

void impala_out_bwd(torch::Tensor pi_save, torch::Tensor H_save,
                    torch::Tensor act, torch::Tensor adv, torch::Tensor v,
                    torch::Tensor vs, torch::Tensor gloss, int64_t B,
                    int64_t T, int64_t A, double er, torch::Tensor dout) {
  int64_t total = B * (T + 1) * (A + 1);
  TORCH_CHECK(dout.numel() == total && dout.is_contiguous(),
              "impala_out_bwd dout shape mismatch");
  TORCH_CHECK(pi_save.numel() == B * T * A && v.numel() == B * T &&
              vs.numel() == B * T && act.numel() == B * T);
  hipLaunchKernelGGL(impala_out_bwd_kernel, dim3(grid_for(total, 2)),
                     dim3(kBlock), 0, cur_stream(), pi_save.data_ptr<float>(),
                     H_save.data_ptr<float>(), act.data_ptr<int64_t>(),
                     adv.data_ptr<float>(), v.data_ptr<float>(),
                     vs.data_ptr<float>(), gloss.data_ptr<float>(), (int)B,
                     (int)T, (int)A, (float)er, dout.data_ptr<float>());
}

namespace {
__global__ void rmsprop_step_kernel(
    float* __restrict__ p, const float* __restrict__ g,
    float* __restrict__ sq, float* __restrict__ ga, float* __restrict__ mom,
    int64_t n, float lr, float alpha, float eps, float wd, float mu,
    bool centered, bool has_mom) {
  int64_t stride = (int64_t)gridDim.x * blockDim.x;
  for (int64_t i = (int64_t)blockIdx.x * blockDim.x + threadIdx.x; i < n;
       i += stride) {
    float grad = g[i] + wd * p[i];
    float s = alpha * sq[i] + (1.0f - alpha) * grad * grad;
    sq[i] = s;
    float avg;
    if (centered) {
      float a = alpha * ga[i] + (1.0f - alpha) * grad;
      ga[i] = a;
      avg = sqrtf(fmaxf(s - a * a, 0.0f)) + eps;
    } else {
      avg = sqrtf(s) + eps;
    }
    float upd = grad / avg;
    if (has_mom) {
      float m = mu * mom[i] + upd;
      mom[i] = m;
      upd = m;
    }
    p[i] -= lr * upd;
  }
}

__global__ void adam_bump_kernel(float* step) {
  if (threadIdx.x == 0 && blockIdx.x == 0) step[0] += 1.0f;
}

__global__ void adam_step_kernel(
    float* __restrict__ p, const float* __restrict__ g,
    float* __restrict__ m, float* __restrict__ v,
    const float* __restrict__ step, int64_t n, float lr, float b1, float b2,
    float eps, float wd) {
  float t = step[0];
  float bc1 = 1.0f - __powf(b1, t);
  float bc2 = 1.0f - __powf(b2, t);
  int64_t stride = (int64_t)gridDim.x * blockDim.x;
  for (int64_t i = (int64_t)blockIdx.x * blockDim.x + threadIdx.x; i < n;
       i += stride) {
    float grad = g[i] + wd * p[i];
    float mi = b1 * m[i] + (1.0f - b1) * grad;
    float vi = b2 * v[i] + (1.0f - b2) * grad * grad;
    m[i] = mi;
    v[i] = vi;
    p[i] -= lr * (mi / bc1) / (sqrtf(vi / bc2) + eps);
  }
}
}

void rmsprop_step(torch::Tensor p, torch::Tensor g, torch::Tensor sq,
                  torch::Tensor ga, torch::Tensor mom, double lr, double alpha,
                  double eps, double wd, double mu, bool centered,
                  bool has_mom) {
  int64_t n = p.numel();
  hipLaunchKernelGGL(rmsprop_step_kernel, dim3(grid_for(n, 4)), dim3(kBlock), 0,
                     cur_stream(), p.data_ptr<float>(), g.data_ptr<float>(),
                     sq.data_ptr<float>(),
                     centered ? ga.data_ptr<float>() : sq.data_ptr<float>(),
                     has_mom ? mom.data_ptr<float>() : sq.data_ptr<float>(),
                     n, (float)lr, (float)alpha, (float)eps, (float)wd,
                     (float)mu, centered, has_mom);
}

void adam_step(torch::Tensor p, torch::Tensor g, torch::Tensor m,
               torch::Tensor v, torch::Tensor step, double lr, double b1,
               double b2, double eps, double wd) {
  int64_t n = p.numel();
  hipLaunchKernelGGL(adam_bump_kernel, dim3(1), dim3(64), 0, cur_stream(),
                     step.data_ptr<float>());
  hipLaunchKernelGGL(adam_step_kernel, dim3(grid_for(n, 4)), dim3(kBlock), 0,
                     cur_stream(), p.data_ptr<float>(), g.data_ptr<float>(),
                     m.data_ptr<float>(), v.data_ptr<float>(),
                     step.data_ptr<float>(), n, (float)lr, (float)b1,
                     (float)b2, (float)eps, (float)wd);
}

namespace {
constexpr int kLstmMaxB = 32;
using f32x4 = __attribute__((ext_vector_type(4))) float;

template <int H>
__global__ __launch_bounds__(256) void lstm_step_fused_kernel(
    const float* __restrict__ xp_t,
    const float* __restrict__ h_in,
    const float* __restrict__ c_in,
    const float* __restrict__ w_hh,
    float* __restrict__ h_out, float* __restrict__ c_out,
    float* __restrict__ acts,
    float* __restrict__ tanhc,
    int B) {
  constexpr int PAD = 4;
  extern __shared__ __attribute__((aligned(16))) char smem[];
  float* h_lds = reinterpret_cast<float*>(smem);
  float* gbuf = h_lds + 32 * (H + PAD);

  const int tid = threadIdx.x;
  const int lane = tid & 63;
  const int wave = tid >> 6;
  const int s16 = blockIdx.x * 16;

  for (int i = tid * 4; i < 32 * H; i += 256 * 4) {
    int row = i / H;
    int k = i - row * H;
    float4 v = {0.f, 0.f, 0.f, 0.f};
    if (row < B) v = *reinterpret_cast<const float4*>(h_in + row * H + k);
    *reinterpret_cast<float4*>(h_lds + row * (H + PAD) + k) = v;
  }
  __syncthreads();

  const int col = wave * H + s16 + (lane & 15);
  f32x4 acc[2] = {{0.f, 0.f, 0.f, 0.f}, {0.f, 0.f, 0.f, 0.f}};
  const int ksub = (lane >> 4) * 4;
  const float* wrow = w_hh + (int64_t)col * H;
#pragma unroll 4
  for (int kb = 0; kb < H; kb += 16) {
    float4 b4 = *reinterpret_cast<const float4*>(wrow + kb + ksub);
    float4 a0 = *reinterpret_cast<const float4*>(
        h_lds + (lane & 15) * (H + PAD) + kb + ksub);
    float4 a1 = *reinterpret_cast<const float4*>(
        h_lds + (16 + (lane & 15)) * (H + PAD) + kb + ksub);
#pragma unroll
    for (int j = 0; j < 4; ++j) {
      acc[0] = __builtin_amdgcn_mfma_f32_16x16x4f32(a0[j], b4[j], acc[0], 0, 0, 0);
      acc[1] = __builtin_amdgcn_mfma_f32_16x16x4f32(a1[j], b4[j], acc[1], 0, 0, 0);
    }
  }
  const int crow = (lane >> 4) * 4;
#pragma unroll
  for (int rf = 0; rf < 2; ++rf)
#pragma unroll
    for (int r = 0; r < 4; ++r) {
      int row = rf * 16 + crow + r;
      int rclamp = row < B ? row : 0;
      float v = acc[rf][r] + xp_t[(int64_t)rclamp * 4 * H + col];
      gbuf[(wave * 32 + row) * 16 + (lane & 15)] = v;
    }
  __syncthreads();

  for (int e = tid; e < 32 * 16; e += 256) {
    int row = e / 16;
    int hc = e - row * 16;
    if (row >= B) continue;
    float gi = gbuf[(0 * 32 + row) * 16 + hc];
    float gf = gbuf[(1 * 32 + row) * 16 + hc];
// ... 752 lines not shown
      if (row < B) {
        const int64_t base =
            (int64_t)t * B * 4 * H + (int64_t)row * 4 * H + g_ * H + n0;
        float4 lo = *reinterpret_cast<const float4*>(&partial[g_][row][half]);
        float4 hi =
            *reinterpret_cast<const float4*>(&partial[g_][row][half + 4]);
        *reinterpret_cast<float4*>(dgates + base + half) = lo;
        *reinterpret_cast<float4*>(dgates + base + half + 4) = hi;
        bf16x8_k5 bv;
        bv[0] = (__bf16)lo.x; bv[1] = (__bf16)lo.y;
        bv[2] = (__bf16)lo.z; bv[3] = (__bf16)lo.w;
        bv[4] = (__bf16)hi.x; bv[5] = (__bf16)hi.y;
        bv[6] = (__bf16)hi.z; bv[7] = (__bf16)hi.w;
        *reinterpret_cast<bf16x8_k5*>(dgates_bf + base + half) = bv;
      }
    }
    __syncthreads();
    if (tid == 0) {
      __builtin_amdgcn_fence(__ATOMIC_RELEASE, "agent");
      asm volatile("s_waitcnt vmcnt(0)" ::: "memory");
      __hip_atomic_fetch_add((gu32_t*)ctr, 1u, DRL_RLX_AGENT);
      const unsigned target = nblocks * (unsigned)(it + 1);
      unsigned spins = 0;
      while (__hip_atomic_load((gu32_t*)ctr, DRL_RLX_AGENT) < target) {
        __builtin_amdgcn_s_sleep(4);
        if (++spins > 5000000u) break;
      }
      __builtin_amdgcn_fence(__ATOMIC_ACQUIRE, "agent");
    }
    __syncthreads();
  }
#pragma unroll
  for (int u = 0; u < 2; ++u) {
    int e = tid + u * 256;
    int row = e >> 4, hc = e & 15;
    if (row < B) dc0_out[(int64_t)row * H + n0 + hc] = dc_reg[u];
  }
}
}

bool lstm_seq_fwd_bf16(torch::Tensor xp, torch::Tensor c0, torch::Tensor w_bf,
                       torch::Tensor hs, torch::Tensor cs, torch::Tensor h_bfs,
                       torch::Tensor acts, torch::Tensor tanhc,
                       torch::Tensor ctr) {
  int T = (int)xp.size(0), B = (int)xp.size(1), H = (int)c0.size(1);
  if (B > kLstmMaxB || H != 512) return false;
  constexpr int HH = 512;
  hipLaunchKernelGGL(lstm_seq_fwd_bf16_kernel<HH>, dim3(HH / 16), dim3(256), 0,
                     cur_stream(), xp.data_ptr<float>(), c0.data_ptr<float>(),
                     (const __bf16*)w_bf.data_ptr(), hs.data_ptr<float>(),
                     cs.data_ptr<float>(), (__bf16*)h_bfs.data_ptr(),
                     acts.data_ptr<float>(), tanhc.data_ptr<float>(),
                     (unsigned int*)ctr.data_ptr(), B, T);
  return true;
}

bool lstm_seq_bwd_bf16(torch::Tensor dh_init, torch::Tensor gout,
                       torch::Tensor dc_T, torch::Tensor w_t_bf,
                       torch::Tensor acts, torch::Tensor tanhc,
                       torch::Tensor cs, torch::Tensor dgates,
                       torch::Tensor dgates_bf, torch::Tensor dc0_out,
                       torch::Tensor ctr) {
  int T = (int)gout.size(0), B = (int)gout.size(1), H = (int)gout.size(2);
  if (B > kLstmMaxB || H != 512) return false;
  constexpr int HH = 512;
  hipLaunchKernelGGL(lstm_seq_bwd_bf16_kernel<HH>, dim3(HH / 16), dim3(256), 0,
                     cur_stream(), dh_init.data_ptr<float>(),
                     gout.data_ptr<float>(), dc_T.data_ptr<float>(),
                     (const __bf16*)w_t_bf.data_ptr(), acts.data_ptr<float>(),
                     tanhc.data_ptr<float>(), cs.data_ptr<float>(),
                     dgates.data_ptr<float>(), (__bf16*)dgates_bf.data_ptr(),
                     dc0_out.data_ptr<float>(),
                     (unsigned int*)ctr.data_ptr(), B, T);
  return true;
}

namespace {

__device__ __forceinline__ float wave_sum(float v) {
  for (int off = 32; off > 0; off >>= 1) v += __shfl_down(v, off, 64);
  return v;
}

template <int HH, int A>
__global__ __launch_bounds__(256) void dueling_q_loss_fwd_kernel(
    const __bf16* __restrict__ h_s,
    const __bf16* __restrict__ h_on,
    const __bf16* __restrict__ h_tg,
    const __bf16* __restrict__ wa, const __bf16* __restrict__ ba,
    const __bf16* __restrict__ wv, const __bf16* __restrict__ bv,
    const __bf16* __restrict__ wa_t, const __bf16* __restrict__ ba_t,
    const __bf16* __restrict__ wv_t, const __bf16* __restrict__ bv_t,
    const int64_t* __restrict__ act, const float* __restrict__ rew,
    const float* __restrict__ done, const float* __restrict__ w, int B,
    float gamma_n, float alpha, float* __restrict__ loss_out,
    float* __restrict__ prio_out, float* __restrict__ grad_coef,
    float* __restrict__ qmax_out) {
  const int lane = threadIdx.x & 63;
  const int b = blockIdx.x * 4 + (threadIdx.x >> 6);
  if (b >= B) return;
  const int k8 = lane * 8;

  float ha_s[8], hv_s[8], ha_on[8], hv_on[8], ha_tg[8], hv_tg[8];
#pragma unroll
  for (int j = 0; j < 8; ++j) {
    ha_s[j] = (float)h_s[(int64_t)b * 2 * HH + k8 + j];
    hv_s[j] = (float)h_s[(int64_t)b * 2 * HH + HH + k8 + j];
    ha_on[j] = (float)h_on[(int64_t)b * 2 * HH + k8 + j];
    hv_on[j] = (float)h_on[(int64_t)b * 2 * HH + HH + k8 + j];
    ha_tg[j] = (float)h_tg[(int64_t)b * 2 * HH + k8 + j];
    hv_tg[j] = (float)h_tg[(int64_t)b * 2 * HH + HH + k8 + j];
  }
  float q_s[A], q_on[A], q_tg[A];
#pragma unroll
  for (int j = 0; j < A; ++j) {
    float pa_s = 0.f, pa_on = 0.f, pa_tg = 0.f;
#pragma unroll
    for (int u = 0; u < 8; ++u) {
      const float wav = (float)wa[(int64_t)j * HH + k8 + u];
      const float wat = (float)wa_t[(int64_t)j * HH + k8 + u];
      pa_s += ha_s[u] * wav;
      pa_on += ha_on[u] * wav;
      pa_tg += ha_tg[u] * wat;
    }
    q_s[j] = wave_sum(pa_s);
    q_on[j] = wave_sum(pa_on);
    q_tg[j] = wave_sum(pa_tg);
  }
  float pv_s = 0.f, pv_on = 0.f, pv_tg = 0.f;
#pragma unroll
  for (int u = 0; u < 8; ++u) {
    const float wvv = (float)wv[k8 + u];
    const float wvt = (float)wv_t[k8 + u];
    pv_s += hv_s[u] * wvv;
    pv_on += hv_on[u] * wvv;
    pv_tg += hv_tg[u] * wvt;
  }
  const float v_s = wave_sum(pv_s);
  const float v_tg = wave_sum(pv_tg);
  wave_sum(pv_on);

  if (lane == 0) {
    float mean_s = 0.f, mean_tg = 0.f, best = -1e30f;
    int a_star = 0;
#pragma unroll
    for (int j = 0; j < A; ++j) {
      const float adv_on = q_on[j] + (float)ba[j];
      if (adv_on > best) { best = adv_on; a_star = j; }
      q_s[j] += (float)ba[j];
      q_tg[j] += (float)ba_t[j];
      mean_s += q_s[j];
      mean_tg += q_tg[j];
    }
    mean_s /= A;
    mean_tg /= A;
    const float vs_full = v_s + (float)bv[0];
    const float vt_full = v_tg + (float)bv_t[0];
    const float q_tgt = q_tg[a_star] - mean_tg + vt_full;
    const float target = rew[b] + gamma_n * q_tgt * (1.0f - done[b]);
    float smax = q_s[0];
#pragma unroll
    for (int j = 1; j < A; ++j) smax = fmaxf(smax, q_s[j]);
    const float q = q_s[act[b]] - mean_s + vs_full;
    const float raw = target - q;
    const float td = fminf(1.0f, fmaxf(-1.0f, raw));
    prio_out[b] = __powf(fabsf(td) + 1e-7f, alpha);
    const float in_range = (raw > -1.0f && raw < 1.0f) ? 1.0f : 0.0f;
    const float invB = 1.0f / B;
    grad_coef[b] = w[b] * td * in_range * invB;
    atomicAdd(loss_out, 0.5f * w[b] * td * td * invB);
    atomicAdd(qmax_out, (smax - mean_s + vs_full) * invB);
  }
}

template <int HH, int A>
__global__ void dueling_q_loss_bwd_dh_kernel(
    const float* __restrict__ grad_coef, const int64_t* __restrict__ act,
    const float* __restrict__ gout, const __bf16* __restrict__ wa,
    const __bf16* __restrict__ wv, int B, __bf16* __restrict__ dh) {
  const int i = blockIdx.x * blockDim.x + threadIdx.x;
  if (i >= B * 2 * HH) return;
  const int b = i / (2 * HH);
  const int k = i - b * 2 * HH;
  const float c = -grad_coef[b] * gout[0];
  float v;
  if (k < HH) {
    float m = 0.f;
#pragma unroll
    for (int j = 0; j < A; ++j) m += (float)wa[(int64_t)j * HH + k];
    v = c * ((float)wa[(int64_t)act[b] * HH + k] - m / A);
  } else {
    v = c * (float)wv[k - HH];
  }
  dh[i] = (__bf16)v;
}

template <int HH, int A, int BS>
__global__ __launch_bounds__(256) void dueling_q_loss_bwd_dw_kernel(
    const float* __restrict__ grad_coef, const int64_t* __restrict__ act,
    const float* __restrict__ gout, const __bf16* __restrict__ h_s, int B,
    float* __restrict__ ws) {
  const int j = blockIdx.x;
  const int sl = blockIdx.y;
  const int tid = threadIdx.x;
  const float g = gout[0];
  float accw[HH / 256];
#pragma unroll
  for (int u = 0; u < HH / 256; ++u) accw[u] = 0.f;
  float accb = 0.f;
  for (int b = sl; b < B; b += BS) {
    const float c = -grad_coef[b] * g;
    float alpha_jb;
    int64_t hoff;
    if (j < A) {
      alpha_jb = c * (((int)act[b] == j ? 1.0f : 0.0f) - 1.0f / A);
      hoff = (int64_t)b * 2 * HH;
    } else {
      alpha_jb = c;
      hoff = (int64_t)b * 2 * HH + HH;
    }
    accb += alpha_jb;
#pragma unroll
    for (int u = 0; u < HH / 256; ++u) {
      const int k = u * 256 + tid;
      accw[u] += alpha_jb * (float)h_s[hoff + k];
    }
  }
  float* row = ws + ((int64_t)sl * (A + 1) + j) * (HH + 1);
#pragma unroll
  for (int u = 0; u < HH / 256; ++u) row[u * 256 + tid] = accw[u];
  if (tid == 0) row[HH] = accb;
}

template <int HH, int A, int BS>
__global__ void dueling_q_loss_bwd_dw_fold_kernel(
    const float* __restrict__ ws, __bf16* __restrict__ dwa,
    __bf16* __restrict__ dba, __bf16* __restrict__ dwv,
    __bf16* __restrict__ dbv) {
  const int i = blockIdx.x * blockDim.x + threadIdx.x;
  constexpr int ROW = HH + 1;
  if (i >= (A + 1) * ROW) return;
  const int j = i / ROW;
  const int k = i - j * ROW;
  float v = 0.f;
#pragma unroll
  for (int s = 0; s < BS; ++s) v += ws[((int64_t)s * (A + 1) + j) * ROW + k];
  if (k < HH) {
    if (j < A)
      dwa[(int64_t)j * HH + k] = (__bf16)v;
    else
      dwv[k] = (__bf16)v;
  } else {
    if (j < A)
      dba[j] = (__bf16)v;
    else
      dbv[0] = (__bf16)v;
  }
}
}

void dueling_q_loss_fwd(torch::Tensor h_s, torch::Tensor h_on,
                        torch::Tensor h_tg, torch::Tensor wa, torch::Tensor ba,
                        torch::Tensor wv, torch::Tensor bv, torch::Tensor wa_t,
                        torch::Tensor ba_t, torch::Tensor wv_t,
                        torch::Tensor bv_t, torch::Tensor act,
                        torch::Tensor rew, torch::Tensor done, torch::Tensor w,
                        double gamma_n, double alpha, torch::Tensor loss_out,
                        torch::Tensor prio_out, torch::Tensor grad_coef,
                        torch::Tensor qmax_out) {
  int B = (int)h_s.size(0);
  TORCH_CHECK(h_s.size(1) == 1024 && wa.size(0) == 6, "geometry: HH=512 A=6");
  hipLaunchKernelGGL((dueling_q_loss_fwd_kernel<512, 6>),
                     dim3((B + 3) / 4), dim3(256), 0, cur_stream(),
                     (const __bf16*)h_s.data_ptr(),
                     (const __bf16*)h_on.data_ptr(),
                     (const __bf16*)h_tg.data_ptr(),
                     (const __bf16*)wa.data_ptr(), (const __bf16*)ba.data_ptr(),
                     (const __bf16*)wv.data_ptr(), (const __bf16*)bv.data_ptr(),
                     (const __bf16*)wa_t.data_ptr(),
                     (const __bf16*)ba_t.data_ptr(),
                     (const __bf16*)wv_t.data_ptr(),
                     (const __bf16*)bv_t.data_ptr(), act.data_ptr<int64_t>(),
                     rew.data_ptr<float>(), done.data_ptr<float>(),
                     w.data_ptr<float>(), B, (float)gamma_n, (float)alpha,
                     loss_out.data_ptr<float>(), prio_out.data_ptr<float>(),
                     grad_coef.data_ptr<float>(), qmax_out.data_ptr<float>());
}

void dueling_q_loss_bwd(torch::Tensor grad_coef, torch::Tensor act,
                        torch::Tensor gout, torch::Tensor wa, torch::Tensor wv,
                        torch::Tensor h_s, torch::Tensor dh, torch::Tensor dwa,
                        torch::Tensor dba, torch::Tensor dwv,
                        torch::Tensor dbv) {
  int B = (int)h_s.size(0);
  hipLaunchKernelGGL((dueling_q_loss_bwd_dh_kernel<512, 6>),
                     dim3(ceil_div((int64_t)B * 1024, kBlock)), dim3(kBlock),
                     0, cur_stream(), grad_coef.data_ptr<float>(),
                     act.data_ptr<int64_t>(), gout.data_ptr<float>(),
                     (const __bf16*)wa.data_ptr(), (const __bf16*)wv.data_ptr(),
                     B, (__bf16*)dh.data_ptr());
  constexpr int BS = 32;
  auto ws = torch::empty({BS * 7 * 513}, torch::dtype(torch::kFloat32)
                                             .device(h_s.device()));
  hipLaunchKernelGGL((dueling_q_loss_bwd_dw_kernel<512, 6, BS>),
                     dim3(7, BS), dim3(256), 0, cur_stream(),
                     grad_coef.data_ptr<float>(), act.data_ptr<int64_t>(),
                     gout.data_ptr<float>(), (const __bf16*)h_s.data_ptr(), B,
                     ws.data_ptr<float>());
  hipLaunchKernelGGL((dueling_q_loss_bwd_dw_fold_kernel<512, 6, BS>),
                     dim3(ceil_div(7 * 513, kBlock)), dim3(kBlock), 0,
                     cur_stream(), ws.data_ptr<float>(),
                     (__bf16*)dwa.data_ptr(), (__bf16*)dba.data_ptr(),
                     (__bf16*)dwv.data_ptr(), (__bf16*)dbv.data_ptr());
}

namespace {

__device__ __forceinline__ float vrescale(float x) {
  const float s = x >= 0.0f ? 1.0f : -1.0f;
  return s * (sqrtf(fabsf(x) + 1.0f) - 1.0f) + 1e-3f * x;
}

__device__ __forceinline__ float inv_vrescale(float x) {
  const float s = x >= 0.0f ? 1.0f : -1.0f;
  const float e = 1e-3f;
  const float t = 1.0f + 4.0f * e * (fabsf(x) + 1.0f + e);
  const float r = (sqrtf(t) - 1.0f) / (2.0f * e);
  return s * (r * r - 1.0f);
}

__global__ void r2d2_loss_fwd_kernel(
    const float* __restrict__ q_train,
    const float* __restrict__ q_tgt,
    const int* __restrict__ act,
    const float* __restrict__ rew,
    const float* __restrict__ done,
    const float* __restrict__ w,
    int T, int B, int A, int m, int n_step, float gamma, int rescale,
    float* __restrict__ td_out,
    float* __restrict__ stats)
{
  const int W = T - 1 - m;
  const int i = blockIdx.x * blockDim.x + threadIdx.x;
  float lc = 0.f, qc = 0.f, tc = 0.f;
  if (i < W * B) {
    const int ti = i / B;
    const int b = i - ti * B;
    const int t = m + ti;
    const int n = min(n_step, T - 1 - t);
    float ret = 0.f, g = 1.0f;
    for (int k = 0; k < n; ++k) {
      ret += g * rew[(int64_t)(t + k) * B + b];
      g *= gamma;
    }
    const int tn = t + n;
    const float* q_on_row = (tn >= m)
        ? q_train + ((int64_t)(tn - m) * B + b) * A
        : q_tgt + ((int64_t)tn * B + b) * A;
    int a_star = 0;
    float best = q_on_row[0];
    for (int a = 1; a < A; ++a)
      if (q_on_row[a] > best) { best = q_on_row[a]; a_star = a; }
    float q_boot = q_tgt[((int64_t)tn * B + b) * A + a_star];
    if (rescale) q_boot = inv_vrescale(q_boot);
    if (tn == T - 1) q_boot *= (1.0f - done[b]);
    float G = ret + g * q_boot;
    if (rescale) G = vrescale(G);
    const float q_taken =
        q_train[((int64_t)ti * B + b) * A + act[(int64_t)t * B + b]];
    const float td = G - q_taken;
    td_out[(int64_t)ti * B + b] = td;
    const float inv = 1.0f / (B * W);
    lc = 0.5f * w[b] * td * td * inv;
    qc = q_taken * inv;
    tc = fabsf(td) * inv;
  }
  for (int off = 32; off > 0; off >>= 1) {
    lc += __shfl_down(lc, off, 64);
    qc += __shfl_down(qc, off, 64);
    tc += __shfl_down(tc, off, 64);
  }
  if ((threadIdx.x & 63) == 0 && (lc != 0.f || qc != 0.f || tc != 0.f)) {
    atomicAdd(&stats[0], lc);
    atomicAdd(&stats[1], qc);
    atomicAdd(&stats[2], tc);
  }
}
// ... 238 lines not shown
```

distributed_rl_amd/parallel/flat_optim.py:

```python

from __future__ import annotations

from typing import Any, Dict, List

import torch

from ..ops import hip_ext


class _FlatOptimBase:
    def __init__(self):
        self.param_groups: List[Dict[str, Any]] = [{}]

    def zero_grad(self, set_to_none: bool = False):
        for g in self.grads:
            g.zero_()


class FlatRMSprop(_FlatOptimBase):
    def __init__(self, params_flat, grads_flat, lr=1e-2, alpha=0.99, eps=1e-8,
                 weight_decay=0.0, momentum=0.0, centered=False):
        super().__init__()
        self.params = list(params_flat)
        self.grads = list(grads_flat)
        self.lr, self.alpha, self.eps = float(lr), float(alpha), float(eps)
        self.wd, self.mu = float(weight_decay), float(momentum)
        self.centered = bool(centered)
        self.sq = [torch.zeros_like(p) for p in self.params]
        self.ga = [torch.zeros_like(p) if centered else torch.empty(0)
                   for p in self.params]
        self.mom = [torch.zeros_like(p) if momentum > 0 else torch.empty(0)
                    for p in self.params]

    def step(self):
        ext = hip_ext()
        for p, g, sq, ga, mom in zip(self.params, self.grads, self.sq,
                                     self.ga, self.mom):
            ext.rmsprop_step(p, g, sq, ga, mom, self.lr, self.alpha, self.eps,
                             self.wd, self.mu, self.centered, self.mu > 0)

    def state_dict(self):
        return {"kind": "flat_rmsprop", "sq": self.sq, "ga": self.ga,
                "mom": self.mom}

    def load_state_dict(self, sd):
        for dst, src in zip(self.sq, sd["sq"]):
            dst.copy_(src.to(dst.device))
        for dst, src in zip(self.ga, sd["ga"]):
            if dst.numel():
                dst.copy_(src.to(dst.device))
        for dst, src in zip(self.mom, sd["mom"]):
            if dst.numel():
                dst.copy_(src.to(dst.device))


class FlatAdam(_FlatOptimBase):
    def __init__(self, params_flat, grads_flat, lr=1e-3, betas=(0.9, 0.999),
                 eps=1e-8, weight_decay=0.0):
        super().__init__()
        self.params = list(params_flat)
        self.grads = list(grads_flat)
        self.lr, self.eps = float(lr), float(eps)
        self.b1, self.b2 = float(betas[0]), float(betas[1])
        self.wd = float(weight_decay)
        self.m = [torch.zeros_like(p) for p in self.params]
        self.v = [torch.zeros_like(p) for p in self.params]
        dev = self.params[0].device
        self.t = [torch.zeros(1, device=dev) for _ in self.params]

    def step(self):
        ext = hip_ext()
        for p, g, m, v, t in zip(self.params, self.grads, self.m, self.v,
                                 self.t):
            ext.adam_step(p, g, m, v, t, self.lr, self.b1, self.b2, self.eps,
                          self.wd)

    def state_dict(self):
        return {"kind": "flat_adam", "m": self.m, "v": self.v, "t": self.t}

    def load_state_dict(self, sd):
        for name in ("m", "v", "t"):
            for dst, src in zip(getattr(self, name), sd[name]):
                dst.copy_(src.to(dst.device))


def make_flat_optimizer(optim_info: Dict[str, Any], mp):
    name = str(optim_info.get("name", "")).lower()
    params = [g.flat_mparam for g in mp.groups]
    grads = [g.flat_mgrad for g in mp.groups]
    if name == "rmsprop":
        return FlatRMSprop(
            params, grads, lr=float(optim_info.get("lr", 1e-3)),
            alpha=float(optim_info.get("alpha", 0.99)),
            eps=float(optim_info.get("eps", 1e-8)),
            weight_decay=float(optim_info.get("decay", 0.0)),
            momentum=float(optim_info.get("momentum", 0.0)),
            centered=bool(optim_info.get("centered", False)),
        )
    if name == "adam":
        return FlatAdam(
            params, grads, lr=float(optim_info.get("lr", 1e-3)),
            eps=float(optim_info.get("eps", 1e-8)),
            weight_decay=float(optim_info.get("decay", 0.0)),
        )
    return None
```

distributed_rl_amd/parallel/precision.py:

```python

from __future__ import annotations

import copy
from typing import Callable, Optional

import torch
import torch.distributed as dist


def _is_cl(p: torch.Tensor) -> bool:
    return p.dim() == 4 and p.is_contiguous(memory_format=torch.channels_last) \
        and not p.is_contiguous()


def _to_flat(p: torch.Tensor) -> torch.Tensor:
    if _is_cl(p):
        return p.permute(0, 2, 3, 1).reshape(-1)
    return p.reshape(-1)


def _view_like(flat_slice: torch.Tensor, p: torch.Tensor) -> torch.Tensor:
    if _is_cl(p):
        N, C, H, W = p.shape
        return flat_slice.view(N, H, W, C).permute(0, 3, 1, 2)
# ... 76 lines not shown
                assert end - start == sum(offs[n][1] for n in names), (
                    f"params {names} are not adjacent in the flat buffer"
                )
                buf = g.flat_cparam if of == "param" else g.flat_cgrad
                return buf[start:end]
        raise KeyError(f"params {names} not found in one group")

    @property
    def flat_cparam(self):
        assert len(self.groups) == 1
        return self.groups[0].flat_cparam

    @property
    def flat_cgrad(self):
        assert len(self.groups) == 1
        return self.groups[0].flat_cgrad

    @property
    def flat_mgrad(self):
        assert len(self.groups) == 1
        return self.groups[0].flat_mgrad

    @property
    def flat_mparam(self):
        assert len(self.groups) == 1
        return self.groups[0].flat_mparam

    def all_mgrads(self):
        return [g.flat_mgrad for g in self.groups]

    def zero_grads(self):
        for g in self.groups:
            g.flat_cgrad.zero_()

    def direct_grads(self, loss, params_override=None):
        if params_override is not None:
            assert len(self.groups) == 1
            grads = torch.autograd.grad(loss, params_override)
            flats = []
            for p, gr in zip(params_override, grads):
                if gr.dim() == 4 and _is_cl(p) and not _is_cl(gr):
                    gr = gr.contiguous(memory_format=torch.channels_last)
                flats.append(_to_flat(gr))
            torch.cat(flats, out=self.groups[0].flat_cgrad)
            return
        params = [cp for g in self.groups for cp in g.c_params]
        grads = torch.autograd.grad(loss, params)
        i = 0
        for g in self.groups:
            n = len(g.c_params)
            flats = []
            for cp, gr in zip(g.c_params, grads[i : i + n]):
                if gr.dim() == 4 and _is_cl(cp) and not _is_cl(gr):
                    gr = gr.contiguous(memory_format=torch.channels_last)
                flats.append(_to_flat(gr))
            i += n
            torch.cat(flats, out=g.flat_cgrad)

    def allreduce_grads(self):
        if self.world > 1:
            for g in self.groups:
                dist.all_reduce(g.flat_cgrad, group=self.pg)

    def allreduce_grads_async(self):
        if self.world > 1:
            return [dist.all_reduce(g.flat_cgrad, group=self.pg, async_op=True)
                    for g in self.groups]
        return []

    def upcast_grads(self):
        for g in self.groups:
            g.flat_mgrad.copy_(g.flat_cgrad)
            if self.world > 1:
                g.flat_mgrad.mul_(1.0 / self.world)

    def reduce_and_upcast(self):
        self.allreduce_grads()
        self.upcast_grads()

    def sync_compute_params(self):
        for g in self.groups:
            g.flat_cparam.copy_(g.flat_mparam)

    def broadcast_master(self):
        if self.world > 1:
            for g in self.groups:
                dist.broadcast(g.flat_mparam, src=0, group=self.pg)
            self.sync_compute_params()
```

Measured before the change: 908,300 frames/s.

## Group three conv towers, fuse ReLU into Q-loss, fuse optimizer tail

Runs the online-state, online-next-state and target-next-state CNN forwards as one grouped conv launch per layer instead of three separate passes. Moves the hidden-layer ReLU into the dueling Q-loss kernels, which now take pre-activations and mask gradients themselves. Fuses grad upcast, the RMSprop step and the bf16 parameter copy-back into a single kernel reading bf16 grads. Conv weight-gradient output now goes straight to bf16 without a float workspace. These cut kernel launches and memory passes, at the cost of more custom code paths, all enabled by default through environment flags.

```diff
diff --git a/distributed_rl_amd/algos/ape_x.py b/distributed_rl_amd/algos/ape_x.py
--- a/distributed_rl_amd/algos/ape_x.py
+++ b/distributed_rl_amd/algos/ape_x.py
@@ -1,6 +1,7 @@
 
 from __future__ import annotations
 
+import os as _os
 import time
 from collections import deque
 from typing import Any, Dict, List, Optional
@@ -11,6 +12,7 @@
 from .. import ops
 from ..config import Config
 from ..models import BaseAgent
+from ..models.base_agent import CNN2D
 from ..replay import make_apex_schema, make_per
 from .common import LearnerBase
 
@@ -142,8 +144,6 @@
         )
         cnn = self.net.nodes[cnn_node]
 
-        import os as _os
-
         own_lin = (ops.linear_relu_supported(in_f, 2 * hidden)
                    and _os.environ.get("DRL_OWN_LINEAR", "0") == "1")
 
@@ -170,6 +170,14 @@
             return hidden_of(cnn(x))
 
         self._fast_hidden = fast_hidden
+        self._cnn = cnn
+        self._own_lin = own_lin
+
+        def pre_hidden_of(feat):
+            return F.linear(feat.to(w1.dtype), w1, b1)
+
+        self._pre_hidden_of = pre_hidden_of
+        self._hidden_of = hidden_of
         self._direct_list = [w1, b1] + list(self.mp.groups[0].c_params[4:])
         self._head_params = (a_head.weight, a_head.bias, v_head.weight,
                              v_head.bias)
@@ -195,6 +203,10 @@
             return t_hidden_of(t_cnn(x))
 
         self._target_hidden = target_hidden
+        self._t_cnn = t_cnn
+        self._t_hidden_of = t_hidden_of
+        self._t_pre_hidden_of = (
+            lambda feat: F.linear(feat.to(w1t.dtype), w1t, b1t))
         self._thead_params = (ta_head.weight, ta_head.bias, tv_head.weight,
                               tv_head.bias)
 
@@ -407,16 +419,29 @@
         weights = weights.to(self.device)
 
         if cuda and getattr(self, "_use_q_loss", False):
-            h_s = self._fast_hidden(s)
+            pre = (_os.environ.get("DRL_PREACT_LOSS", "1") == "1"
+                   and not self._own_lin)
+            if _os.environ.get("DRL_GROUPED_CONV", "1") == "1":
+                f_s, f_on, f_tg = CNN2D.forward_grouped(
+                    [(s, self._cnn, True), (sp, self._cnn, False),
+                     (sp, self._t_cnn, False)])
+            else:
+                f_s = self._cnn(s)
+                with torch.no_grad():
+                    f_on = self._cnn(sp)
+                    f_tg = self._t_cnn(sp)
+            hid = self._pre_hidden_of if pre else self._hidden_of
+            t_hid = self._t_pre_hidden_of if pre else self._t_hidden_of
+            h_s = hid(f_s)
             with torch.no_grad():
-                h_on = self._fast_hidden(sp)
-                h_tg = self._target_hidden(sp)
+                h_on = hid(f_on)
+                h_tg = t_hid(f_tg)
             wa, ba, wv, bv = self._head_params
             wat, bat, wvt, bvt = self._thead_params
             loss, prio, qmean = ops.dueling_q_head_loss(
                 h_s, wa, ba, wv, bv, h_on, h_tg, wat, bat, wvt, bvt,
                 actions, rewards, dones, weights, self.gamma, self.n_step,
-                self.alpha,
+                self.alpha, pre_act=pre,
             )
         elif cuda and getattr(self, "_fast_heads", None) is not None:
             adv_s, val_s = self._fast_heads(s)
@@ -446,6 +471,9 @@
         return {"loss": loss.detach(), "value": qmean}, prio
 
     def _optimize_mp(self):
+        if (_os.environ.get("DRL_FUSED_OPT_TAIL", "1") == "1"
+                and self.mp.fused_step(self.optim)):
+            return
         self.mp.upcast_grads()
         self.optim.step()
         self.mp.sync_compute_params()
diff --git a/distributed_rl_amd/models/base_agent.py b/distributed_rl_amd/models/base_agent.py
--- a/distributed_rl_amd/models/base_agent.py
+++ b/distributed_rl_amd/models/base_agent.py
@@ -106,6 +106,81 @@
         if self.flatten:
             y = torch.flatten(y, 1)
         return y
+
+    def _grouped_ok(self, x: torch.Tensor) -> bool:
+        if not self._fused_ok(x):
+            return False
+        key = ("grouped", tuple(x.shape[1:]), x.dtype)
+        hit = self._fused_checked.get(key)
+        if hit is not None:
+            return hit
+        from .. import ops as _ops
+
+        ok = True
+        C, H, W = x.shape[1:]
+        u8 = x.dtype == torch.uint8
+        last = len(self._convs) - 1
+        for i, conv in enumerate(self._convs):
+            COUT, _, KH, KW = conv.weight.shape
+            S = conv.stride[0]
+            chw = (i == last and self.flatten
+                   and _ops.conv_chw_supported(H, W, C, KH, KW, S, COUT))
+            if not _ops.conv_grouped_supported(H, W, C, KH, KW, S, COUT, u8,
+                                               chw):
+                ok = False
+                break
+            H = (H - KH) // S + 1
+            W = (W - KW) // S + 1
+            C = COUT
+            u8 = False
+        self._fused_checked[key] = ok
+        return ok
+
+    @staticmethod
+    def forward_grouped(jobs) -> List[torch.Tensor]:
+        from .. import ops as _ops
+
+        xs = [j[0] for j in jobs]
+        mods = [j[1] for j in jobs]
+        m0 = mods[0]
+        same = all(
+            m.flatten == m0.flatten and len(m._convs) == len(m0._convs)
+            and all(a.weight.shape == b.weight.shape and a.stride == b.stride
+                    and (a.bias is None) == (b.bias is None)
+                    for a, b in zip(m._convs, m0._convs))
+            for m in mods)
+        if not (same and 1 <= len(jobs) <= 4
+                and all(x.shape == xs[0].shape and x.dtype == xs[0].dtype
+                        for x in xs)
+                and all(m._grouped_ok(x) for x, m in zip(xs, mods))):
+            outs = []
+            for x, m, needs_grad in jobs:
+                with torch.set_grad_enabled(needs_grad
+                                            and torch.is_grad_enabled()):
+                    outs.append(m(x))
+            return outs
+
+        def par(t, needs_grad):
+            return t if needs_grad or t is None else t.detach()
+
+        ys = [x if g else x.detach() for x, _, g in jobs]
+        last = len(m0._convs) - 1
+        for i in range(len(m0._convs)):
+            convs = [m._convs[i] for m in mods]
+            c0 = convs[0]
+            chw = (i == last and m0.flatten and _ops.conv_chw_supported(
+                ys[0].shape[2], ys[0].shape[3], ys[0].shape[1],
+                c0.weight.shape[2], c0.weight.shape[3], c0.stride[0],
+                c0.weight.shape[0]))
+            ys = list(_ops.fused_conv_relu_grouped(
+                ys, [par(c.weight, j[2]) for c, j in zip(convs, jobs)],
+                [par(c.bias, j[2]) for c, j in zip(convs, jobs)],
+                c0.stride[0], chw_out=chw))
+            if chw:
+                return ys
+        if m0.flatten:
+            ys = [torch.flatten(y, 1) for y in ys]
+        return ys
 
 
 class MLP(nn.Module):
diff --git a/distributed_rl_amd/ops/__init__.py b/distributed_rl_amd/ops/__init__.py
--- a/distributed_rl_amd/ops/__init__.py
+++ b/distributed_rl_amd/ops/__init__.py
@@ -108,79 +108,178 @@
     @staticmethod
     def backward(ctx, gout):
         x, weight, out = ctx.saved_tensors
-        stride = ctx.stride
-        COUT = weight.shape[0]
-        if ctx.chw:
-            P, Q = ctx.pq
-            N = gout.shape[0]
-            masked = torch.empty(N, COUT, P, Q, dtype=torch.bfloat16,
-                                 device=gout.device,
-                                 memory_format=torch.channels_last)
-            hip_ext().relu_mask_bwd_chw(gout.contiguous(), out, masked,
-                                        COUT, P * Q)
-            gout = masked
-        else:
-            if not gout.is_contiguous(memory_format=torch.channels_last):
-                gout = gout.contiguous(memory_format=torch.channels_last)
-            masked = torch.empty_like(gout)
-            hip_ext().relu_mask_bwd(gout, out, masked)
-            gout = masked
         need_x = ctx.needs_input_grad[0]
         need_w = ctx.needs_input_grad[1]
         need_b = ctx.has_bias and ctx.needs_input_grad[2]
-        COUT, C, KH, KW = weight.shape
-        ext = hip_ext()
-        use_own_wrw = need_w and bool(
-            ext.conv_wrw_supported(x.shape[2], x.shape[3], C, KH, KW, stride,
-                                   COUT, x.dtype == torch.uint8)
-        )
-        gw = gb = None
-        if use_own_wrw:
-            K = KH * KW * C
-            flat_ws = torch.empty(COUT * (K + 1), dtype=torch.float32,
-                                  device=x.device)
-            ws = flat_ws[: COUT * K].view(COUT, K)
-            gb_ws = (flat_ws[COUT * K :] if need_b
-                     else torch.empty(0, device=x.device))
-            ext.conv_wrw(x, gout, ws, gb_ws, stride)
-            gw = ws.view(COUT, KH, KW, C).permute(0, 3, 1, 2).to(torch.bfloat16)
-            if need_b:
-                gb = gb_ws.to(torch.bfloat16)
-        gi = None
-        use_own_dgrad = (
-            os.environ.get("DRL_OWN_DGRAD", "0") == "1"
-            and need_x and x.dtype == torch.bfloat16
-            and hasattr(ext, "conv_dgrad_supported")
-            and bool(ext.conv_dgrad_supported(x.shape[2], x.shape[3], C, KH,
-                                              KW, stride, COUT))
-        )
-        if use_own_dgrad:
-            gi = torch.empty_like(x)
-            w_t = torch.empty(weight.numel(), dtype=torch.bfloat16,
+        gi, gw, gb = _fused_conv_backward(
+            x, weight, out, gout, ctx.stride, ctx.has_bias, ctx.chw, ctx.pq,
+            need_x, need_w, need_b)
+        return gi, gw, gb, None, None
+
+
+def _fused_conv_backward(x, weight, out, gout, stride, has_bias, chw, pq,
+                         need_x, need_w, need_b):
+    COUT = weight.shape[0]
+    if chw:
+        P, Q = pq
+        N = gout.shape[0]
+        masked = torch.empty(N, COUT, P, Q, dtype=torch.bfloat16,
+                             device=gout.device,
+                             memory_format=torch.channels_last)
+        hip_ext().relu_mask_bwd_chw(gout.contiguous(), out, masked,
+                                    COUT, P * Q)
+        gout = masked
+    else:
+        if not gout.is_contiguous(memory_format=torch.channels_last):
+            gout = gout.contiguous(memory_format=torch.channels_last)
+        masked = torch.empty_like(gout)
+        hip_ext().relu_mask_bwd(gout, out, masked)
+        gout = masked
+    COUT, C, KH, KW = weight.shape
+    ext = hip_ext()
+    use_own_wrw = need_w and bool(
+        ext.conv_wrw_supported(x.shape[2], x.shape[3], C, KH, KW, stride,
+                               COUT, x.dtype == torch.uint8)
+    )
+    gw = gb = None
+    if use_own_wrw and os.environ.get("DRL_WRW_BF16", "1") == "1":
+        gw = torch.empty(COUT, KH, KW, C, dtype=torch.bfloat16,
+                         device=x.device).permute(0, 3, 1, 2)
+        gb = (torch.empty(COUT, dtype=torch.bfloat16, device=x.device)
+              if need_b else None)
+        ext.conv_wrw(x, gout, gw,
+                     gb if need_b else torch.empty(0, device=x.device),
+                     stride)
+    elif use_own_wrw:
+        K = KH * KW * C
+        flat_ws = torch.empty(COUT * (K + 1), dtype=torch.float32,
                               device=x.device)
-            ext.conv_dgrad(gout, weight, w_t, gi, stride)
-        if (need_x and not use_own_dgrad) or (need_w and not use_own_wrw):
-            if x.dtype == torch.uint8:
-                xf = dequant_frames(x.permute(0, 2, 3, 1), torch.bfloat16)
-                xf = xf.permute(0, 3, 1, 2)
-            else:
-                xf = x
-            gi2, gw2, gb2 = torch.ops.aten.convolution_backward(
-                gout, xf, weight,
-                [COUT] if ctx.has_bias else None,
-                [stride, stride], [0, 0], [1, 1], False, [0, 0], 1,
-                [need_x and not use_own_dgrad, need_w and not use_own_wrw,
-                 need_b and not use_own_wrw],
-            )
-            if gi is None:
-                gi = gi2
-            if gw is None:
-                gw, gb = gw2, gb2
-        return (gi if need_x else None), gw, gb, None, None
+        ws = flat_ws[: COUT * K].view(COUT, K)
+        gb_ws = (flat_ws[COUT * K :] if need_b
+                 else torch.empty(0, device=x.device))
+        ext.conv_wrw(x, gout, ws, gb_ws, stride)
+        gw = ws.view(COUT, KH, KW, C).permute(0, 3, 1, 2).to(torch.bfloat16)
+        if need_b:
+            gb = gb_ws.to(torch.bfloat16)
+    gi = None
+    use_own_dgrad = (
+        os.environ.get("DRL_OWN_DGRAD", "0") == "1"
+        and need_x and x.dtype == torch.bfloat16
+        and hasattr(ext, "conv_dgrad_supported")
+        and bool(ext.conv_dgrad_supported(x.shape[2], x.shape[3], C, KH,
+                                          KW, stride, COUT))
+    )
+    if use_own_dgrad:
+        gi = torch.empty_like(x)
+        w_t = torch.empty(weight.numel(), dtype=torch.bfloat16,
+                          device=x.device)
+        ext.conv_dgrad(gout, weight, w_t, gi, stride)
+    if (need_x and not use_own_dgrad) or (need_w and not use_own_wrw):
+        if x.dtype == torch.uint8:
+            xf = dequant_frames(x.permute(0, 2, 3, 1), torch.bfloat16)
+            xf = xf.permute(0, 3, 1, 2)
+        else:
+            xf = x
+        gi2, gw2, gb2 = torch.ops.aten.convolution_backward(
+            gout, xf, weight,
+            [COUT] if has_bias else None,
+            [stride, stride], [0, 0], [1, 1], False, [0, 0], 1,
+            [need_x and not use_own_dgrad, need_w and not use_own_wrw,
+             need_b and not use_own_wrw],
+        )
+        if gi is None:
+            gi = gi2
+        if gw is None:
+            gw, gb = gw2, gb2
+    return (gi if need_x else None), gw, gb
 
 
 def fused_conv_relu(x, weight, bias, stride: int, chw_out: bool = False):
     return _FusedConvFn.apply(x, weight, bias, stride, chw_out)
+
+
+def conv_grouped_supported(H, W, C, KH, KW, S, COUT, u8: bool,
+                           chw_out: bool = False) -> bool:
+    ext = hip_ext(required=False)
+    return ext is not None and hasattr(ext, "conv_fwd_grouped_supported") and \
+        bool(ext.conv_fwd_grouped_supported(H, W, C, KH, KW, S, COUT, u8,
+                                            chw_out))
+
+
+class _FusedConvGroupedFn(torch.autograd.Function):
+
+    @staticmethod
+    def forward(ctx, stride, chw_out, njobs, *args):
+        ext = hip_ext()
+        xs = list(args[:njobs])
+        ws = list(args[njobs : 2 * njobs])
+        bs = list(args[2 * njobs :])
+        has_bias = bs[0] is not None
+        assert all((b is not None) == has_bias for b in bs), \
+            "grouped conv: biases must be all set or all None"
+        x0, w0 = xs[0], ws[0]
+        N, C, H, W = x0.shape
+        COUT, _, KH, KW = w0.shape
+        P = (H - KH) // stride + 1
+        Q = (W - KW) // stride + 1
+        if chw_out:
+            outs = [torch.empty(N, COUT * P * Q, dtype=torch.bfloat16,
+                                device=x0.device) for _ in range(njobs)]
+        else:
+            outs = [torch.empty(N, COUT, P, Q, dtype=torch.bfloat16,
+                                device=x0.device,
+                                memory_format=torch.channels_last)
+                    for _ in range(njobs)]
+        ext.conv_fwd_grouped(xs, ws, bs if has_bias else [], outs, stride,
+                             chw_out)
+        live = [any(ctx.needs_input_grad[3 + k * njobs + j] for k in range(3))
+                for j in range(njobs)]
+        saved = []
+        for j in range(njobs):
+            if live[j]:
+                saved += [xs[j], ws[j], outs[j]]
+        ctx.save_for_backward(*saved)
+        dead = [outs[j] for j in range(njobs) if not live[j]]
+        if dead:
+            ctx.mark_non_differentiable(*dead)
+        ctx.live = live
+        ctx.njobs = njobs
+        ctx.stride = stride
+        ctx.has_bias = has_bias
+        ctx.chw = chw_out
+        ctx.pq = (P, Q)
+        ctx.set_materialize_grads(False)
+        return tuple(outs)
+
+    @staticmethod
+    def backward(ctx, *gouts):
+        n = ctx.njobs
+        grads = [None] * (3 * n)
+        saved = ctx.saved_tensors
+        k = 0
+        for j in range(n):
+            if not ctx.live[j]:
+                continue
+            x, weight, out = saved[k : k + 3]
+            k += 3
+            if gouts[j] is None:
+                continue
+            need_x = ctx.needs_input_grad[3 + j]
+            need_w = ctx.needs_input_grad[3 + n + j]
+            need_b = ctx.has_bias and ctx.needs_input_grad[3 + 2 * n + j]
+            gi, gw, gb = _fused_conv_backward(
+                x, weight, out, gouts[j], ctx.stride, ctx.has_bias, ctx.chw,
+                ctx.pq, need_x, need_w, need_b)
+            grads[j], grads[n + j], grads[2 * n + j] = gi, gw, gb
+        return (None, None, None, *grads)
+
+
+def fused_conv_relu_grouped(xs, weights, biases, stride: int,
+                            chw_out: bool = False):
+    n = len(xs)
+    assert len(weights) == n and len(biases) == n
+    return _FusedConvGroupedFn.apply(stride, bool(chw_out), n, *xs, *weights,
+                                     *biases)
 
 
 
@@ -451,7 +550,8 @@
 class _DuelingQLossFn(torch.autograd.Function):
     @staticmethod
     def forward(ctx, h_s, wa, ba, wv, bv, h_on, h_tg, wa_t, ba_t, wv_t, bv_t,
-                actions, rewards, dones, weights, gamma_n, alpha):
+                actions, rewards, dones, weights, gamma_n, alpha,
+                pre_act=False):
         ext = hip_ext()
         B = h_s.shape[0]
         dev = h_s.device
@@ -465,8 +565,9 @@
             wv_t.reshape(-1).contiguous(), bv_t.contiguous(),
             actions.contiguous(), rewards.contiguous(), dones.contiguous(),
             weights.contiguous(), float(gamma_n), float(alpha),
-            acc2[0:1], prio, coef, acc2[1:2],
-        )
+            acc2[0:1], prio, coef, acc2[1:2], bool(pre_act),
+        )
+        ctx.pre_act = bool(pre_act)
         ctx.save_for_backward(coef, actions, wa, wv, h_s)
         loss_out, qmean = acc2[0], acc2[1]
         ctx.mark_non_differentiable(prio, qmean)
@@ -485,8 +586,9 @@
         dbv = torch.empty(1, dtype=torch.bfloat16, device=dev)
         ext.dueling_q_loss_bwd(coef, actions, gout.reshape(1).contiguous(),
                                wa.contiguous(), wv.reshape(-1).contiguous(),
-                               h_s.contiguous(), dh, dwa, dba, dwv, dbv)
-        return (dh, dwa, dba, dwv, dbv) + (None,) * 12
+                               h_s.contiguous(), dh, dwa, dba, dwv, dbv,
+                               ctx.pre_act)
+        return (dh, dwa, dba, dwv, dbv) + (None,) * 13
 
 
 def has_r2d2_seq_loss() -> bool:
@@ -538,14 +640,17 @@
 
 def dueling_q_head_loss(h_s, wa, ba, wv, bv, h_on, h_tg, wa_t, ba_t, wv_t,
                         bv_t, actions, rewards, dones, weights, gamma: float,
-                        n_step: int, alpha: float):
+                        n_step: int, alpha: float, pre_act: bool = False):
     if _use_hip(h_s):
         return _DuelingQLossFn.apply(
             h_s, wa, ba, wv, bv, h_on, h_tg, wa_t, ba_t, wv_t, bv_t,
             actions.long(), rewards.float(), dones.float(), weights.float(),
-            gamma ** n_step, alpha,
+            gamma ** n_step, alpha, pre_act,
         )
     import torch.nn.functional as F
+
+    if pre_act:
+        h_s, h_on, h_tg = F.relu(h_s), F.relu(h_on), F.relu(h_tg)
 
     def heads(h, wa_, ba_, wv_, bv_):
         return (F.linear(h[:, :512].float(), wa_.float(), ba_.float()),
diff --git a/distributed_rl_amd/ops/hip/conv_mfma.hip b/distributed_rl_amd/ops/hip/conv_mfma.hip
--- a/distributed_rl_amd/ops/hip/conv_mfma.hip
+++ b/distributed_rl_amd/ops/hip/conv_mfma.hip
@@ -26,15 +26,13 @@
 
 template <int H, int W, int C, int KH, int KW, int S, int COUT, bool U8IN,
           int WAVES, int RPW, bool CHW_OUT = false>
-__global__ __launch_bounds__(WAVES * 64) void conv_fwd_kernel(
+__device__ __forceinline__ void conv_fwd_block(
     const void* __restrict__ in_v,
     const __bf16* __restrict__ weight,
     const __bf16* __restrict__ bias,
     __bf16* __restrict__ out,
-    int batch) {
+    int batch, int tile, __bf16* wlds) {
   using G = ConvGeom<H, W, C, KH, KW, S, COUT, U8IN>;
-  extern __shared__ __attribute__((aligned(16))) char smem[];
-  __bf16* wlds = reinterpret_cast<__bf16*>(smem);
 
   const int tid = threadIdx.x;
   const int lane = tid & 63;
@@ -50,7 +48,7 @@
   __syncthreads();
 
   const int M = batch * G::P * G::Q;
-  const int row0 = (blockIdx.x * WAVES + wave) * RPW;
+  const int row0 = (tile * WAVES + wave) * RPW;
   if (row0 >= M) return;
   constexpr int RFRAG = RPW / 16;
   constexpr int NFRAG = COUT / 16;
@@ -135,34 +133,70 @@
     }
 }
 
+template <int H, int W, int C, int KH, int KW, int S, int COUT, bool U8IN,
+          int WAVES, int RPW, bool CHW_OUT = false>
+__global__ __launch_bounds__(WAVES * 64) void conv_fwd_kernel(
+    const void* __restrict__ in_v, const __bf16* __restrict__ weight,
+    const __bf16* __restrict__ bias, __bf16* __restrict__ out, int batch) {
+  extern __shared__ __attribute__((aligned(16))) char smem[];
+  conv_fwd_block<H, W, C, KH, KW, S, COUT, U8IN, WAVES, RPW, CHW_OUT>(
+      in_v, weight, bias, out, batch, blockIdx.x,
+      reinterpret_cast<__bf16*>(smem));
+}
+
+constexpr int kMaxConvJobs = 4;
+struct ConvJobs {
+  const void* in[kMaxConvJobs];
+  const __bf16* weight[kMaxConvJobs];
+  const __bf16* bias[kMaxConvJobs];
+  __bf16* out[kMaxConvJobs];
+};
+
+template <int H, int W, int C, int KH, int KW, int S, int COUT, bool U8IN,
+          int WAVES, int RPW, bool CHW_OUT = false>
+__global__ __launch_bounds__(WAVES * 64) void conv_fwd_grouped_kernel(
+    const ConvJobs jobs, int njobs, int batch) {
+  extern __shared__ __attribute__((aligned(16))) char smem[];
+  const int tile = blockIdx.x / njobs;
+  const int job = blockIdx.x - tile * njobs;
+  conv_fwd_block<H, W, C, KH, KW, S, COUT, U8IN, WAVES, RPW, CHW_OUT>(
+      jobs.in[job], jobs.weight[job], jobs.bias[job], jobs.out[job], batch,
+      tile, reinterpret_cast<__bf16*>(smem));
+}
+
 struct ConvLaunch {
   int H, W, C, KH, KW, S, COUT;
   bool u8;
   void (*fn)(const void*, const __bf16*, const __bf16*, __bf16*, int);
   int lds_bytes;
   int waves, rpw;
+  void (*grouped)(const ConvJobs, int, int);
 };
 
 template <int H, int W, int C, int KH, int KW, int S, int COUT, bool U8,
-          int WAVES = 4, int RPW = 16, bool CHW = false>
+          int WAVES = 4, int RPW = 16, bool CHW = false, bool GROUPED = false>
 ConvLaunch make_launch() {
   using G = ConvGeom<H, W, C, KH, KW, S, COUT, U8>;
+  void (*grouped)(const ConvJobs, int, int) = nullptr;
+  if constexpr (GROUPED)
+    grouped = conv_fwd_grouped_kernel<H, W, C, KH, KW, S, COUT, U8, WAVES, RPW,
+                                      CHW>;
   return ConvLaunch{H, W, C, KH, KW, S, COUT, U8,
                     conv_fwd_kernel<H, W, C, KH, KW, S, COUT, U8, WAVES, RPW,
                                     CHW>,
-                    (int)(G::LDS_ELEMS * sizeof(__bf16)), WAVES, RPW};
+                    (int)(G::LDS_ELEMS * sizeof(__bf16)), WAVES, RPW, grouped};
 }
 
 static const ConvLaunch kChwLaunches[] = {
-    make_launch<9, 9, 64, 3, 3, 1, 64, false, 8, 16, true>(),
+    make_launch<9, 9, 64, 3, 3, 1, 64, false, 8, 16, true, true>(),
     make_launch<20, 20, 16, 4, 4, 2, 32, false, 8, 16, true>(),
 };
 
 static const ConvLaunch kLaunches[] = {
-    make_launch<84, 84, 4, 8, 8, 4, 32, true, 8, 32>(),
-    make_launch<84, 84, 4, 8, 8, 4, 32, false, 8, 32>(),
-    make_launch<20, 20, 32, 4, 4, 2, 64, false, 8, 16>(),
-    make_launch<9, 9, 64, 3, 3, 1, 64, false, 8, 16>(),
+    make_launch<84, 84, 4, 8, 8, 4, 32, true, 8, 32, false, true>(),
+    make_launch<84, 84, 4, 8, 8, 4, 32, false, 8, 32, false, true>(),
+    make_launch<20, 20, 32, 4, 4, 2, 64, false, 8, 16, false, true>(),
+    make_launch<9, 9, 64, 3, 3, 1, 64, false, 8, 16, false, true>(),
     make_launch<84, 84, 4, 8, 8, 4, 16, true, 8, 16>(),
     make_launch<84, 84, 4, 8, 8, 4, 16, false, 8, 16>(),
     make_launch<20, 20, 16, 4, 4, 2, 32, false, 8, 16>(),
@@ -302,6 +336,14 @@
                             int64_t KW, int64_t S, int64_t COUT);
 void relu_mask_bwd_chw(torch::Tensor gout2d, torch::Tensor out2d,
                        torch::Tensor dst_nhwc, int64_t C, int64_t PQ);
+void conv_fwd_grouped(std::vector<torch::Tensor> ins,
+                      std::vector<torch::Tensor> weights,
+                      std::vector<torch::Tensor> biases,
+                      std::vector<torch::Tensor> outs, int64_t stride,
+                      bool chw_out);
+bool conv_fwd_grouped_supported(int64_t H, int64_t W, int64_t C, int64_t KH,
+                                int64_t KW, int64_t S, int64_t COUT, bool u8,
+                                bool chw_out);
 void linear_relu(torch::Tensor x, torch::Tensor w, torch::Tensor b,
                  torch::Tensor out);
 bool linear_relu_supported(int64_t K, int64_t N);
@@ -317,7 +359,11 @@
   m.def("conv_fwd_supported", &conv_fwd_supported);
   m.def("mfma_probe", &mfma_probe, "16x16x32 bf16 MFMA fragment-map probe");
   m.def("conv_fwd_variant", &conv_fwd_variant, "tuning-variant conv fwd");
-  m.def("conv_wrw", &conv_wrw, "MFMA conv weight-grad (fp32 workspace)");
+  m.def("conv_fwd_grouped", &conv_fwd_grouped,
+        "conv_fwd / conv_fwd_chw for up to 4 same-geometry jobs in one launch");
+  m.def("conv_fwd_grouped_supported", &conv_fwd_grouped_supported);
+  m.def("conv_wrw", &conv_wrw,
+        "MFMA conv weight-grad; gw/gb are fp32 workspaces or bf16 grads");
   m.def("conv_wrw_supported", &conv_wrw_supported);
   m.def("conv_dgrad", &conv_dgrad,
         "MFMA conv data-grad (masked-tap gather, pre-transposed weights)");
@@ -468,10 +514,11 @@
     }
 }
 
+template <typename OutT>
 __global__ __launch_bounds__(256) void wrw_reduce_kernel(
     const float* __restrict__ part, int planes, int n_elem,
-    float* __restrict__ out, const float* __restrict__ b_part, int b_planes,
-    int cout, float* __restrict__ b_out) {
+    OutT* __restrict__ out, const float* __restrict__ b_part, int b_planes,
+    int cout, OutT* __restrict__ b_out) {
   __shared__ __attribute__((aligned(16))) float sh4_raw[256 * 4];
   float* sh = sh4_raw;
   const int tid = threadIdx.x;
@@ -504,7 +551,12 @@
         const float4 v = sh4[k * 16 + tid];
         t.x += v.x; t.y += v.y; t.z += v.z; t.w += v.w;
       }
-      *reinterpret_cast<float4*>(out + e4) = t;
+      if constexpr (std::is_same<OutT, float>::value) {
+        *reinterpret_cast<float4*>(out + e4) = t;
+      } else {
+        v4bf_w o = {(__bf16)t.x, (__bf16)t.y, (__bf16)t.z, (__bf16)t.w};
+        *reinterpret_cast<v4bf_w*>(out + e4) = o;
+      }
     }
   } else {
     const int G = 256 / cout;
@@ -516,7 +568,7 @@
     if (tid < cout) {
       float t = 0.0f;
       for (int k = 0; k < G; ++k) t += sh[k * cout + tid];
-      b_out[tid] = t;
+      b_out[tid] = (OutT)t;
     }
   }
 }
@@ -590,7 +642,11 @@
               torch::Tensor gb_ws, int64_t stride) {
   TORCH_CHECK(in.is_contiguous(at::MemoryFormat::ChannelsLast));
   TORCH_CHECK(gout.is_contiguous(at::MemoryFormat::ChannelsLast));
-  TORCH_CHECK(gw_ws.scalar_type() == torch::kFloat32 && gw_ws.is_contiguous());
+  const bool bf16_out = gw_ws.scalar_type() == torch::kBFloat16;
+  TORCH_CHECK(bf16_out || gw_ws.scalar_type() == torch::kFloat32);
+  TORCH_CHECK(gw_ws.is_contiguous() ||
+              (gw_ws.dim() == 4 &&
+               gw_ws.is_contiguous(at::MemoryFormat::ChannelsLast)));
   const int N = (int)in.size(0), C = (int)in.size(1), H = (int)in.size(2),
             W = (int)in.size(3);
   const int COUT = (int)gout.size(1);
@@ -616,8 +672,8 @@
   auto st = (hipStream_t)at::cuda::getCurrentCUDAStream().stream();
   const int n_elem = (int)gw_ws.numel();
   TORCH_CHECK(n_elem == COUT * L->ktiles * 64, "gw_ws shape mismatch");
-  auto part = torch::empty({(int64_t)mb, (int64_t)n_elem + kPlanePad},
-                           gw_ws.options());
+  const auto f32 = gw_ws.options().dtype(torch::kFloat32);
+  auto part = torch::empty({(int64_t)mb, (int64_t)n_elem + kPlanePad}, f32);
   hipLaunchKernelGGL(L->fn, dim3(L->ktiles, mb), dim3(256), L->lds_bytes, st,
                      (const void*)in.data_ptr(), (const __bf16*)gout.data_ptr(),
                      part.data_ptr<float>(), N, mb);
@@ -625,9 +681,9 @@
   constexpr int kColsumBlocks = 256;
   torch::Tensor b_part;
   if (bias) {
-    TORCH_CHECK(gb_ws.numel() == COUT && gb_ws.scalar_type() == torch::kFloat32);
-    b_part = torch::empty({(int64_t)kColsumBlocks, (int64_t)COUT},
-                          gw_ws.options());
+    TORCH_CHECK(gb_ws.numel() == COUT && gb_ws.is_contiguous() &&
+                gb_ws.scalar_type() == gw_ws.scalar_type());
+    b_part = torch::empty({(int64_t)kColsumBlocks, (int64_t)COUT}, f32);
     const int64_t Mrows = (int64_t)N * P * Q;
     switch (COUT) {
       case 16:
@@ -650,11 +706,20 @@
     }
   }
   const int e_blocks = (n_elem + 63) / 64;
-  hipLaunchKernelGGL(wrw_reduce_kernel, dim3(e_blocks + (bias ? 1 : 0)),
-                     dim3(256), 0, st, (const float*)part.data_ptr<float>(), mb,
-                     n_elem, gw_ws.data_ptr<float>(),
-                     bias ? (const float*)b_part.data_ptr<float>() : nullptr,
-                     kColsumBlocks, COUT, bias ? gb_ws.data_ptr<float>() : nullptr);
+  const float* b_part_ptr =
+      bias ? (const float*)b_part.data_ptr<float>() : nullptr;
+  if (bf16_out)
+    hipLaunchKernelGGL(wrw_reduce_kernel<__bf16>,
+                       dim3(e_blocks + (bias ? 1 : 0)), dim3(256), 0, st,
+                       (const float*)part.data_ptr<float>(), mb, n_elem,
+                       (__bf16*)gw_ws.data_ptr(), b_part_ptr, kColsumBlocks,
+                       COUT, bias ? (__bf16*)gb_ws.data_ptr() : nullptr);
+  else
+    hipLaunchKernelGGL(wrw_reduce_kernel<float>,
+                       dim3(e_blocks + (bias ? 1 : 0)), dim3(256), 0, st,
+                       (const float*)part.data_ptr<float>(), mb, n_elem,
+                       gw_ws.data_ptr<float>(), b_part_ptr, kColsumBlocks, COUT,
+                       bias ? gb_ws.data_ptr<float>() : nullptr);
 }
 
 namespace {
@@ -885,6 +950,99 @@
                      (const void*)in.data_ptr(),
                      (const __bf16*)weight.data_ptr(), bias_ptr,
                      (__bf16*)out2d.data_ptr(), N);
+}
+
+void conv_fwd_grouped(std::vector<torch::Tensor> ins,
+                      std::vector<torch::Tensor> weights,
+                      std::vector<torch::Tensor> biases,
+                      std::vector<torch::Tensor> outs, int64_t stride,
+                      bool chw_out) {
+  const int njobs = (int)ins.size();
+  TORCH_CHECK(njobs >= 1 && njobs <= kMaxConvJobs, "1..", kMaxConvJobs,
+              " conv jobs per grouped launch");
+  TORCH_CHECK((int)weights.size() == njobs && (int)outs.size() == njobs &&
+              (biases.empty() || (int)biases.size() == njobs));
+  const auto& in0 = ins[0];
+  const auto& w0 = weights[0];
+  const int N = (int)in0.size(0), C = (int)in0.size(1), H = (int)in0.size(2),
+            W = (int)in0.size(3);
+  const int COUT = (int)w0.size(0), KH = (int)w0.size(2), KW = (int)w0.size(3);
+  const bool u8 = in0.scalar_type() == torch::kUInt8;
+  const int P = (H - KH) / (int)stride + 1, Q = (W - KW) / (int)stride + 1;
+  ConvJobs jobs{};
+  for (int j = 0; j < njobs; ++j) {
+    const auto& in = ins[j];
+    const auto& w = weights[j];
+    const auto& out = outs[j];
+    TORCH_CHECK(in.is_cuda() && w.is_cuda() && out.is_cuda());
+    TORCH_CHECK(in.dim() == 4 && in.sizes() == in0.sizes() &&
+                    in.scalar_type() == in0.scalar_type(),
+                "grouped conv jobs must share N and input geometry");
+    TORCH_CHECK(u8 || in.scalar_type() == torch::kBFloat16);
+    TORCH_CHECK(w.dim() == 4 && w.sizes() == w0.sizes() && w.size(1) == C &&
+                    w.scalar_type() == torch::kBFloat16,
+                "grouped conv jobs must share the weight geometry");
+    TORCH_CHECK(in.is_contiguous(at::MemoryFormat::ChannelsLast),
+                "conv_fwd_grouped input must be channels_last");
+    TORCH_CHECK(w.is_contiguous(at::MemoryFormat::ChannelsLast));
+    TORCH_CHECK(out.scalar_type() == torch::kBFloat16 &&
+                out.numel() == (int64_t)N * COUT * P * Q);
+    if (chw_out) {
+      TORCH_CHECK(out.dim() == 2 && out.is_contiguous());
+    } else {
+      TORCH_CHECK(out.dim() == 4 && out.size(0) == N && out.size(1) == COUT &&
+                  out.size(2) == P && out.size(3) == Q &&
+                  out.is_contiguous(at::MemoryFormat::ChannelsLast));
+    }
+    jobs.in[j] = in.data_ptr();
+    jobs.weight[j] = (const __bf16*)w.data_ptr();
+    jobs.out[j] = (__bf16*)out.data_ptr();
+    jobs.bias[j] = nullptr;
+    if (!biases.empty() && biases[j].defined() && biases[j].numel() > 0) {
+      TORCH_CHECK(biases[j].scalar_type() == torch::kBFloat16 &&
+                  biases[j].numel() == COUT && biases[j].is_cuda());
+      jobs.bias[j] = (const __bf16*)biases[j].data_ptr();
+    }
+  }
+  const ConvLaunch* L = nullptr;
+  auto match = [&](const ConvLaunch& l) {
+    return l.grouped && l.H == H && l.W == W && l.C == C && l.KH == KH &&
+           l.KW == KW && l.S == (int)stride && l.COUT == COUT && l.u8 == u8;
+  };
+  if (chw_out) {
+    for (const auto& l : kChwLaunches)
+      if (match(l)) { L = &l; break; }
+  } else {
+    for (const auto& l : kLaunches)
+      if (match(l)) { L = &l; break; }
+  }
+  TORCH_CHECK(L, "no grouped conv kernel for this geometry: ", H, "x", W, "x",
+              C, " k", KH, "x", KW, " s", stride, " -> ", COUT, " u8=", u8,
+              " chw=", chw_out);
+  const int M = N * P * Q;
+  const int rows_per_block = L->waves * L->rpw;
+  const int tiles = (M + rows_per_block - 1) / rows_per_block;
+  hipLaunchKernelGGL(L->grouped, dim3(tiles * njobs), dim3(L->waves * 64),
+                     L->lds_bytes,
+                     (hipStream_t)at::cuda::getCurrentCUDAStream().stream(),
+                     jobs, njobs, N);
+}
+
+bool conv_fwd_grouped_supported(int64_t H, int64_t W, int64_t C, int64_t KH,
+                                int64_t KW, int64_t S, int64_t COUT, bool u8,
+                                bool chw_out) {
+  auto match = [&](const ConvLaunch& l) {
+    return l.grouped && l.H == H && l.W == W && l.C == C && l.KH == KH &&
+           l.KW == KW && l.S == S && l.COUT == COUT && l.u8 == u8;
+  };
+  if (chw_out) {
+    for (const auto& l : kChwLaunches)
+      if (match(l)) return true;
+  } else {
+    for (const auto& l : kLaunches)
+      if (match(l)) return true;
+  }
+  return false;
 }
 
 namespace {
diff --git a/distributed_rl_amd/ops/hip/drl_kernels.hip b/distributed_rl_amd/ops/hip/drl_kernels.hip
--- a/distributed_rl_amd/ops/hip/drl_kernels.hip
+++ b/distributed_rl_amd/ops/hip/drl_kernels.hip
@@ -622,7 +622,9 @@
                     int64_t T, int64_t A, double er, torch::Tensor dout);
 void rmsprop_step(torch::Tensor p, torch::Tensor g, torch::Tensor sq,
                   torch::Tensor ga, torch::Tensor mom, double lr, double alpha,
-                  double eps, double wd, double mu, bool centered, bool has_mom);
+                  double eps, double wd, double mu, bool centered, bool has_mom,
+                  c10::optional<torch::Tensor> g_bf16, double grad_scale,
+                  c10::optional<torch::Tensor> p_bf16);
 void adam_step(torch::Tensor p, torch::Tensor g, torch::Tensor m,
                torch::Tensor v, torch::Tensor step, double lr, double b1,
                double b2, double eps, double wd);
@@ -676,12 +678,12 @@
                         torch::Tensor rew, torch::Tensor done, torch::Tensor w,
                         double gamma_n, double alpha, torch::Tensor loss_out,
                         torch::Tensor prio_out, torch::Tensor grad_coef,
-                        torch::Tensor qmax_out);
+                        torch::Tensor qmax_out, bool pre_act);
 void dueling_q_loss_bwd(torch::Tensor grad_coef, torch::Tensor act,
                         torch::Tensor gout, torch::Tensor wa, torch::Tensor wv,
                         torch::Tensor h_s, torch::Tensor dh, torch::Tensor dwa,
                         torch::Tensor dba, torch::Tensor dwv,
-                        torch::Tensor dbv);
+                        torch::Tensor dbv, bool pre_act);
 void r2d2_loss_fwd(torch::Tensor q_train, torch::Tensor q_tgt,
                    torch::Tensor act, torch::Tensor rew, torch::Tensor done,
                    torch::Tensor w, int64_t m, int64_t n_step, double gamma,
@@ -725,7 +727,17 @@
         "fused IMPALA total loss: pg objective + entropy + critic MSE (K9)");
   m.def("impala_out_bwd", &impala_out_bwd,
         "IMPALA whole-head backward: d loss/d out in one launch (K9)");
-  m.def("rmsprop_step", &rmsprop_step, "fused flat centered RMSprop (K12)");
+  m.def("rmsprop_step", &rmsprop_step,
+        "fused flat centered RMSprop (K12); optional bf16 grad source "
+        "(* grad_scale) and bf16 param shadow fold the mixed-precision "
+        "upcast and param sync into the same pass",
+        pybind11::arg("p"), pybind11::arg("g"), pybind11::arg("sq"),
+        pybind11::arg("ga"), pybind11::arg("mom"), pybind11::arg("lr"),
+        pybind11::arg("alpha"), pybind11::arg("eps"), pybind11::arg("wd"),
+        pybind11::arg("mu"), pybind11::arg("centered"),
+        pybind11::arg("has_mom"), pybind11::arg("g_bf16") = pybind11::none(),
+        pybind11::arg("grad_scale") = 1.0,
+        pybind11::arg("p_bf16") = pybind11::none());
   m.def("adam_step", &adam_step, "fused flat Adam (K12)");
   m.def("lstm_step_fused", &lstm_step_fused,
         "one-kernel LSTM timestep: fp32-MFMA hh GEMM + cell (K5)");
@@ -1118,15 +1130,27 @@
 }
 
 namespace {
+template <bool FUSED_TAIL, bool SCALE>
 __global__ void rmsprop_step_kernel(
     float* __restrict__ p, const float* __restrict__ g,
     float* __restrict__ sq, float* __restrict__ ga, float* __restrict__ mom,
     int64_t n, float lr, float alpha, float eps, float wd, float mu,
-    bool centered, bool has_mom) {
+    bool centered, bool has_mom, const __bf16* __restrict__ g_bf16,
+    float grad_scale, __bf16* __restrict__ p_bf16) {
   int64_t stride = (int64_t)gridDim.x * blockDim.x;
   for (int64_t i = (int64_t)blockIdx.x * blockDim.x + threadIdx.x; i < n;
        i += stride) {
-    float grad = g[i] + wd * p[i];
+    float gi;
+    if constexpr (FUSED_TAIL) {
+      gi = (float)g_bf16[i];
+      if constexpr (SCALE) {
+        gi = gi * grad_scale;
+        asm volatile("" : "+v"(gi));
+      }
+    } else {
+      gi = g[i];
+    }
+    float grad = gi + wd * p[i];
     float s = alpha * sq[i] + (1.0f - alpha) * grad * grad;
     sq[i] = s;
     float avg;
@@ -1143,7 +1167,9 @@
       mom[i] = m;
       upd = m;
     }
-    p[i] -= lr * upd;
+    const float pn = p[i] - lr * upd;
+    p[i] = pn;
+    if constexpr (FUSED_TAIL) p_bf16[i] = (__bf16)pn;
   }
 }
 
@@ -1175,15 +1201,46 @@
 void rmsprop_step(torch::Tensor p, torch::Tensor g, torch::Tensor sq,
                   torch::Tensor ga, torch::Tensor mom, double lr, double alpha,
                   double eps, double wd, double mu, bool centered,
-                  bool has_mom) {
+                  bool has_mom, c10::optional<torch::Tensor> g_bf16,
+                  double grad_scale, c10::optional<torch::Tensor> p_bf16) {
   int64_t n = p.numel();
-  hipLaunchKernelGGL(rmsprop_step_kernel, dim3(grid_for(n, 4)), dim3(kBlock), 0,
-                     cur_stream(), p.data_ptr<float>(), g.data_ptr<float>(),
-                     sq.data_ptr<float>(),
-                     centered ? ga.data_ptr<float>() : sq.data_ptr<float>(),
-                     has_mom ? mom.data_ptr<float>() : sq.data_ptr<float>(),
-                     n, (float)lr, (float)alpha, (float)eps, (float)wd,
-                     (float)mu, centered, has_mom);
+  float* ga_ptr = centered ? ga.data_ptr<float>() : sq.data_ptr<float>();
+  float* mom_ptr = has_mom ? mom.data_ptr<float>() : sq.data_ptr<float>();
+  const bool fused = g_bf16.has_value() || p_bf16.has_value();
+  if (!fused) {
+    TORCH_CHECK(g.numel() == n, "rmsprop_step: grad size mismatch");
+    hipLaunchKernelGGL((rmsprop_step_kernel<false, false>),
+                       dim3(grid_for(n, 4)), dim3(kBlock), 0, cur_stream(),
+                       p.data_ptr<float>(), g.data_ptr<float>(),
+                       sq.data_ptr<float>(), ga_ptr, mom_ptr, n, (float)lr,
+                       (float)alpha, (float)eps, (float)wd, (float)mu, centered,
+                       has_mom, (const __bf16*)nullptr, 1.0f,
+                       (__bf16*)nullptr);
+    return;
+  }
+  TORCH_CHECK(g_bf16.has_value() && p_bf16.has_value(),
+              "rmsprop_step: the fused tail takes g_bf16 AND p_bf16");
+  TORCH_CHECK(g_bf16->scalar_type() == torch::kBFloat16 &&
+              p_bf16->scalar_type() == torch::kBFloat16 &&
+              g_bf16->numel() == n && p_bf16->numel() == n &&
+              g_bf16->is_contiguous() && p_bf16->is_contiguous() &&
+              p.is_contiguous() && sq.numel() == n);
+  const __bf16* gb = (const __bf16*)g_bf16->data_ptr();
+  __bf16* pb = (__bf16*)p_bf16->data_ptr();
+  if (grad_scale != 1.0)
+    hipLaunchKernelGGL((rmsprop_step_kernel<true, true>),
+                       dim3(grid_for(n, 4)), dim3(kBlock), 0, cur_stream(),
+                       p.data_ptr<float>(), (const float*)nullptr,
+                       sq.data_ptr<float>(), ga_ptr, mom_ptr, n, (float)lr,
+                       (float)alpha, (float)eps, (float)wd, (float)mu, centered,
+                       has_mom, gb, (float)grad_scale, pb);
+  else
+    hipLaunchKernelGGL((rmsprop_step_kernel<true, false>),
+                       dim3(grid_for(n, 4)), dim3(kBlock), 0, cur_stream(),
+                       p.data_ptr<float>(), (const float*)nullptr,
+                       sq.data_ptr<float>(), ga_ptr, mom_ptr, n, (float)lr,
+                       (float)alpha, (float)eps, (float)wd, (float)mu, centered,
+                       has_mom, gb, 1.0f, pb);
 }
 
 void adam_step(torch::Tensor p, torch::Tensor g, torch::Tensor m,
@@ -2102,7 +2159,11 @@
   return v;
 }
 
-template <int HH, int A>
+__device__ __forceinline__ float relu_if(bool pre, float x) {
+  return pre ? (x > 0.0f ? x : 0.0f) : x;
+}
+
+template <int HH, int A, bool PRE>
 __global__ __launch_bounds__(256) void dueling_q_loss_fwd_kernel(
     const __bf16* __restrict__ h_s,
     const __bf16* __restrict__ h_on,
@@ -2124,12 +2185,15 @@
   float ha_s[8], hv_s[8], ha_on[8], hv_on[8], ha_tg[8], hv_tg[8];
 #pragma unroll
   for (int j = 0; j < 8; ++j) {
-    ha_s[j] = (float)h_s[(int64_t)b * 2 * HH + k8 + j];
-    hv_s[j] = (float)h_s[(int64_t)b * 2 * HH + HH + k8 + j];
-    ha_on[j] = (float)h_on[(int64_t)b * 2 * HH + k8 + j];
-    hv_on[j] = (float)h_on[(int64_t)b * 2 * HH + HH + k8 + j];
-    ha_tg[j] = (float)h_tg[(int64_t)b * 2 * HH + k8 + j];
-    hv_tg[j] = (float)h_tg[(int64_t)b * 2 * HH + HH + k8 + j];
+    ha_s[j] = relu_if(PRE, (float)h_s[(int64_t)b * 2 * HH + k8 + j]);
+    hv_s[j] =
+        relu_if(PRE, (float)h_s[(int64_t)b * 2 * HH + HH + k8 + j]);
+    ha_on[j] = relu_if(PRE, (float)h_on[(int64_t)b * 2 * HH + k8 + j]);
+    hv_on[j] =
+        relu_if(PRE, (float)h_on[(int64_t)b * 2 * HH + HH + k8 + j]);
+    ha_tg[j] = relu_if(PRE, (float)h_tg[(int64_t)b * 2 * HH + k8 + j]);
+    hv_tg[j] =
+        relu_if(PRE, (float)h_tg[(int64_t)b * 2 * HH + HH + k8 + j]);
   }
   float q_s[A], q_on[A], q_tg[A];
 #pragma unroll
@@ -2193,11 +2257,12 @@
   }
 }
 
-template <int HH, int A>
+template <int HH, int A, bool PRE>
 __global__ void dueling_q_loss_bwd_dh_kernel(
     const float* __restrict__ grad_coef, const int64_t* __restrict__ act,
     const float* __restrict__ gout, const __bf16* __restrict__ wa,
-    const __bf16* __restrict__ wv, int B, __bf16* __restrict__ dh) {
+    const __bf16* __restrict__ wv, const __bf16* __restrict__ h_s, int B,
+    __bf16* __restrict__ dh) {
   const int i = blockIdx.x * blockDim.x + threadIdx.x;
   if (i >= B * 2 * HH) return;
   const int b = i / (2 * HH);
@@ -2212,10 +2277,13 @@
   } else {
     v = c * (float)wv[k - HH];
   }
+  if constexpr (PRE) {
+    if (!((float)h_s[i] > 0.0f)) v = 0.0f;
+  }
   dh[i] = (__bf16)v;
 }
 
-template <int HH, int A, int BS>
+template <int HH, int A, int BS, bool PRE>
 __global__ __launch_bounds__(256) void dueling_q_loss_bwd_dw_kernel(
     const float* __restrict__ grad_coef, const int64_t* __restrict__ act,
     const float* __restrict__ gout, const __bf16* __restrict__ h_s, int B,
@@ -2243,7 +2311,7 @@
 #pragma unroll
     for (int u = 0; u < HH / 256; ++u) {
       const int k = u * 256 + tid;
-      accw[u] += alpha_jb * (float)h_s[hoff + k];
+      accw[u] += alpha_jb * relu_if(PRE, (float)h_s[hoff + k]);
     }
   }
   float* row = ws + ((int64_t)sl * (A + 1) + j) * (HH + 1);
@@ -2287,10 +2355,11 @@
                         torch::Tensor rew, torch::Tensor done, torch::Tensor w,
                         double gamma_n, double alpha, torch::Tensor loss_out,
                         torch::Tensor prio_out, torch::Tensor grad_coef,
-                        torch::Tensor qmax_out) {
+                        torch::Tensor qmax_out, bool pre_act) {
   int B = (int)h_s.size(0);
   TORCH_CHECK(h_s.size(1) == 1024 && wa.size(0) == 6, "geometry: HH=512 A=6");
-  hipLaunchKernelGGL((dueling_q_loss_fwd_kernel<512, 6>),
+  hipLaunchKernelGGL((pre_act ? dueling_q_loss_fwd_kernel<512, 6, true>
+                              : dueling_q_loss_fwd_kernel<512, 6, false>),
                      dim3((B + 3) / 4), dim3(256), 0, cur_stream(),
                      (const __bf16*)h_s.data_ptr(),
                      (const __bf16*)h_on.data_ptr(),
@@ -2311,18 +2380,21 @@
                         torch::Tensor gout, torch::Tensor wa, torch::Tensor wv,
                         torch::Tensor h_s, torch::Tensor dh, torch::Tensor dwa,
                         torch::Tensor dba, torch::Tensor dwv,
-                        torch::Tensor dbv) {
+                        torch::Tensor dbv, bool pre_act) {
   int B = (int)h_s.size(0);
-  hipLaunchKernelGGL((dueling_q_loss_bwd_dh_kernel<512, 6>),
+  TORCH_CHECK(h_s.numel() == (int64_t)B * 1024 && dh.numel() == h_s.numel());
+  hipLaunchKernelGGL((pre_act ? dueling_q_loss_bwd_dh_kernel<512, 6, true>
+                              : dueling_q_loss_bwd_dh_kernel<512, 6, false>),
                      dim3(ceil_div((int64_t)B * 1024, kBlock)), dim3(kBlock),
                      0, cur_stream(), grad_coef.data_ptr<float>(),
                      act.data_ptr<int64_t>(), gout.data_ptr<float>(),
                      (const __bf16*)wa.data_ptr(), (const __bf16*)wv.data_ptr(),
-                     B, (__bf16*)dh.data_ptr());
+                     (const __bf16*)h_s.data_ptr(), B, (__bf16*)dh.data_ptr());
   constexpr int BS = 32;
   auto ws = torch::empty({BS * 7 * 513}, torch::dtype(torch::kFloat32)
                                              .device(h_s.device()));
-  hipLaunchKernelGGL((dueling_q_loss_bwd_dw_kernel<512, 6, BS>),
+  hipLaunchKernelGGL((pre_act ? dueling_q_loss_bwd_dw_kernel<512, 6, BS, true>
+                              : dueling_q_loss_bwd_dw_kernel<512, 6, BS, false>),
                      dim3(7, BS), dim3(256), 0, cur_stream(),
                      grad_coef.data_ptr<float>(), act.data_ptr<int64_t>(),
                      gout.data_ptr<float>(), (const __bf16*)h_s.data_ptr(), B,
diff --git a/distributed_rl_amd/parallel/flat_optim.py b/distributed_rl_amd/parallel/flat_optim.py
--- a/distributed_rl_amd/parallel/flat_optim.py
+++ b/distributed_rl_amd/parallel/flat_optim.py
@@ -38,6 +38,15 @@
                                      self.ga, self.mom):
             ext.rmsprop_step(p, g, sq, ga, mom, self.lr, self.alpha, self.eps,
                              self.wd, self.mu, self.centered, self.mu > 0)
+
+    def step_mixed(self, grads_bf16, params_bf16, grad_scale: float = 1.0):
+        ext = hip_ext()
+        for p, sq, ga, mom, gb, pb in zip(self.params, self.sq, self.ga,
+                                          self.mom, grads_bf16, params_bf16):
+            ext.rmsprop_step(p, p, sq, ga, mom, self.lr, self.alpha, self.eps,
+                             self.wd, self.mu, self.centered, self.mu > 0,
+                             g_bf16=gb, grad_scale=float(grad_scale),
+                             p_bf16=pb)
 
     def state_dict(self):
         return {"kind": "flat_rmsprop", "sq": self.sq, "ga": self.ga,
diff --git a/distributed_rl_amd/parallel/precision.py b/distributed_rl_amd/parallel/precision.py
--- a/distributed_rl_amd/parallel/precision.py
+++ b/distributed_rl_amd/parallel/precision.py
@@ -182,6 +182,19 @@
         for g in self.groups:
             g.flat_cparam.copy_(g.flat_mparam)
 
+    def fused_step(self, optim) -> bool:
+        from .flat_optim import FlatRMSprop
+
+        if not (isinstance(optim, FlatRMSprop) and len(self.groups) == 1
+                and self.groups[0].dtype == torch.bfloat16
+                and len(optim.params) == 1
+                and optim.params[0] is self.groups[0].flat_mparam):
+            return False
+        g = self.groups[0]
+        optim.step_mixed([g.flat_cgrad], [g.flat_cparam],
+                         1.0 / self.world if self.world > 1 else 1.0)
+        return True
+
     def broadcast_master(self):
         if self.world > 1:
             for g in self.groups:
```

New measurement: 1.030 million frames/s, median of 6. 1.13x the previous value.
